# aws/sagemaker-xgboost-container

Hardware: NVIDIA H100
Metric: boosting rounds/sec (higher is better)
Workload: dtype int64

## Files before the change

### microbench/hist_modes.py

```python
#!/usr/bin/env python
import argparse
import json
import os
import sys

import numpy as np

ROOT = os.path.dirname(os.path.dirname(os.path.abspath(__file__)))
sys.path.insert(0, ROOT)


def main():
    ap = argparse.ArgumentParser()
    ap.add_argument("--rows", type=int, default=50_000_000)
    ap.add_argument("--cols", type=int, default=100)
    ap.add_argument("--repeats", type=int, default=5)
    ap.add_argument("--out", default="")
    a = ap.parse_args()
    import torch
    import bench
    import sagemaker_xgboost_container_b200 as xgb
    be = xgb.get_backend()
    dev = torch.device("cuda", 0)
    ba = argparse.Namespace(rows=a.rows, cols=a.cols, seed=43, objective="reg:squarederror", num_class=0)
    X, y = bench.gen_shard(ba, 0, a.rows, dev)
    d = xgb.DMatrix(X, label=y.cpu().numpy())
    del X
    torch.cuda.empty_cache()
    b = xgb.Booster({"max_bin": 256}, [d])
    rng = np.random.default_rng(1)
    n, F = a.rows, a.cols
    gpair = np.empty((n, 2), np.float32)
    gpair[:, 0] = rng.standard_normal(n, dtype=np.float32)
    gpair[:, 1] = 1.0
    peak = bench.hbm_peak()[0]
    res = []

    def run(label, mode, rows=None):
        m = n if rows is None else len(rows)
        gp = gpair if rows is None else gpair[:m]
        be.build_histogram_ex(b.handle, d.handle, gp, mode=mode, row_ids=rows, repeats=2)
        hist, scales, ms, kernel = be.build_histogram_ex(b.handle, d.handle, gp, mode=mode, row_ids=rows, repeats=a.repeats)
        bytes_ = m * (F + 8 + (0 if rows is None else 4))
        r = {"case": label, "kernel": kernel, "rows": m, "ms": ms, "gbs": bytes_ / ms / 1e6, "frac_of_peak": bytes_ / ms / 1e6 / peak,
             "checksum": int(hist[:, :, 0].sum()), "checksum_h": int(hist[:, :, 1].sum())}
        res.append(r)
        print(json.dumps(r), flush=True)

    run("root TMA G+H", 0)
    run("root TMA G-only", 2)
    run("root gather-kernel", 1)
    run("every 2nd row", 0, np.arange(0, n, 2, dtype=np.uint32))
    run("every 4th row", 0, np.arange(0, n, 4, dtype=np.uint32))
    sub = np.sort(rng.choice(n, size=n // 4, replace=False).astype(np.uint32))
    run("random 25% sorted", 0, sub)
    sub = np.sort(rng.choice(n, size=n // 16, replace=False).astype(np.uint32))
    run("random 6% sorted", 0, sub)
    if a.out:
        json.dump({"rows": n, "cols": F, "peak_gbs": peak, "results": res}, open(a.out, "w"), indent=1)


if __name__ == "__main__":
    main()
```

### sagemaker-xgboost-container_b200/csrc/booster.cu

```cuda
#include "booster.h"
#include <algorithm>
#include <atomic>
#include <cctype>
#include <cmath>
#include <cstring>
#include "comm.h"
#include "rng.h"

namespace b200 {

long long g_kernel_launches = 0;

namespace {
struct DeviceCtx {
  cudaStream_t stream = nullptr; int num_sms = 0; bool ok = false; std::string why;
  DeviceCtx() {
    int count = 0;
    cudaError_t e = cudaGetDeviceCount(&count);
    if (e != cudaSuccess || count == 0) { why = std::string("no CUDA device available (") + cudaGetErrorString(e) + ")"; cudaGetLastError(); return; }
    int dev = 0;
    if (const char* lr = getenv("LOCAL_RANK")) { dev = atoi(lr) % count; }
    if (const char* d = getenv("B200XGB_DEVICE")) { dev = atoi(d) % count; }
    if (cudaSetDevice(dev) != cudaSuccess) { why = "cudaSetDevice failed"; return; }
    if (cudaStreamCreateWithFlags(&stream, cudaStreamNonBlocking) != cudaSuccess) { why = "cudaStreamCreate failed"; return; }
// ... 462 lines not shown
    c.n = dm->n; c.margin.alloc((size_t)dm->n * K); c.trees_applied = -1;
  }
  return c;
}

void Booster::bring_cache_up_to_date(DMatrix* dm, PredCache& c) {
  cudaStream_t s = engine_stream();
  const int K = param_.num_class;
  const int nt = (int)trees_.size();
  if (c.trees_applied < 0) {
    if (!dm->base_margin.empty()) {
      B200_CHECK(dm->base_margin.size() == (size_t)dm->n * K, "base_margin size does not match rows x groups");
      CUDA_OK(cudaMemcpyAsync(c.margin.p, dm->d_base_margin.p, sizeof(float) * dm->n * K, cudaMemcpyDeviceToDevice, s));
    } else launch_fill(c.margin.p, dm->n * K, base_margin(), s);
    c.trees_applied = 0; c.weights.clear();
  }
  if (dart_.on) {
    std::vector<int> ids; std::vector<float> coef;
    for (int t = 0; t < c.trees_applied; ++t)
      if (c.weights[t] != weight_drop_[t]) { ids.push_back(t); coef.push_back(weight_drop_[t] - c.weights[t]); }
    for (int t = c.trees_applied; t < nt; ++t) { ids.push_back(t); coef.push_back(weight_drop_[t]); }
    if (!ids.empty()) dart_margin(dm, ids, coef, {}, c.margin.p, nullptr);
  } else if (c.trees_applied < nt) {
    upload_model();
    PredictArgs pa = predict_args(dm, c.trees_applied, nt);
    pa.margin = c.margin.p;
    launch_predict(pa, s);
  }
  c.trees_applied = nt;
  c.weights.assign(weight_drop_.begin(), weight_drop_.begin() + nt);
}

std::vector<int> Booster::dart_drop_set(int round) const {
  std::vector<int> D;
  const int T = (int)weight_drop_.size();
  const unsigned seed = param_.seed;
  if (T == 0) return D;
  if (dart_.skip_drop > 0.0f && rng_uniform(seed, kDartSkipStream, (uint64_t)round) < dart_.skip_drop) return D;
  const uint64_t tree_stream = kDartTreeStream + (uint64_t)round;
  float sum_w = 0.0f;
  for (float w : weight_drop_) sum_w += w;
  for (int i = 0; i < T; ++i) {
    const float u = rng_uniform(seed, tree_stream, (uint64_t)i);
    const float thr = dart_.sample_type == 1 ? dart_.rate_drop * (float)T * weight_drop_[i] / sum_w : dart_.rate_drop;
    if (u < thr) D.push_back(i);
  }
  if (dart_.one_drop && D.empty()) {
    const double u = (double)rng_uniform(seed, kDartOneStream, (uint64_t)round);
    int pick = std::min(T - 1, (int)(u * (double)T));
    if (dart_.sample_type == 1) {
      double tot = 0.0; for (float w : weight_drop_) tot += (double)w;
      const double target = u * tot; double acc = 0.0; pick = T - 1;
      for (int i = 0; i < T; ++i) { acc += (double)weight_drop_[i]; if (acc > target) { pick = i; break; } }
    }
    D.push_back(pick);
  }
  return D;
}

float* Booster::dart_begin_round(DMatrix* dtrain, PredCache& c, int round) {
  const std::vector<int> D = dart_drop_set(round);
  const int K = param_.num_class;
  const float lr = (float)((double)param_.eta / (double)K);
  float factor = 1.0f; dart_new_weight_ = 1.0f;
  if (!D.empty()) {
    if (dart_.normalize_type == 1) { factor = (float)(1.0 / (1.0 + (double)lr)); dart_new_weight_ = factor; }
    else { const float denom = (float)D.size() + lr; factor = (float)((double)D.size() / (double)denom); dart_new_weight_ = (float)(1.0 / (double)denom); }
  }
  builder_->set_leaf_scale(dart_new_weight_);
  if (D.empty()) return c.margin.p;
  std::vector<float> coef_full, coef_drop;
  for (int j : D) {
    const float w = weight_drop_[j], w2 = w * factor;
    coef_drop.push_back(w); coef_full.push_back(w2 - w);
    weight_drop_[j] = w2; c.weights[j] = w2;
  }
  dart_drop_margin_.ensure((size_t)dtrain->n * K);
  dart_margin(dtrain, D, coef_full, coef_drop, c.margin.p, dart_drop_margin_.p);
  return dart_drop_margin_.p;
}

void Booster::dart_margin(DMatrix* dm, const std::vector<int>& ids, const std::vector<float>& coef_full, const std::vector<float>& coef_drop,
                          float* m_full, float* m_drop) {
  cudaStream_t s = engine_stream();
  upload_model();
  const size_t m = ids.size();
  dart_ids_.ensure(m); dart_coef_.ensure(2 * m);
  CUDA_OK(cudaMemcpyAsync(dart_ids_.p, ids.data(), sizeof(int) * m, cudaMemcpyHostToDevice, s));
  CUDA_OK(cudaMemcpyAsync(dart_coef_.p, coef_full.data(), sizeof(float) * m, cudaMemcpyHostToDevice, s));
  if (m_drop) CUDA_OK(cudaMemcpyAsync(dart_coef_.p + m, coef_drop.data(), sizeof(float) * m, cudaMemcpyHostToDevice, s));
  DartArgs a{}; a.X = dm->X.p; a.n = dm->n; a.F = dm->F; a.nodes = d_nodes.p; a.tree_offset = d_tree_offset.p; a.tree_info = d_tree_info.p;
  a.trees = dart_ids_.p; a.ntrees = (int)m; a.K = param_.num_class; a.coef_full = dart_coef_.p; a.coef_drop = dart_coef_.p + m;
  a.m_full = m_full; a.m_drop = m_drop;
  launch_dart_margin(a, s);
  Comm::get().sync_stream(s);
}

static void check_labels(const DMatrix* dm) {
  B200_CHECK(dm->labels.size() == (size_t)dm->n, "Check failed: preds.size() == info.labels_.size() (" + std::to_string(dm->n) + " vs. " +
             std::to_string(dm->labels.size()) + ") : labels are not correctly provided");
}
static void check_aft_bounds(const DMatrix* dm) {
  B200_CHECK(dm->label_lower.size() == (size_t)dm->n && dm->label_upper.size() == (size_t)dm->n,
             "survival:aft needs label_lower_bound and label_upper_bound with one entry per row (" + std::to_string(dm->n) + " rows, " +
             std::to_string(dm->label_lower.size()) + " lower and " + std::to_string(dm->label_upper.size()) + " upper bounds)");
}
static void check_train_width(const DMatrix* dm) {
  B200_CHECK(dm->F <= kMaxTrainFeatures, "the CUDA hist builder trains on at most " + std::to_string(kMaxTrainFeatures) + " features (the data has " +
             std::to_string(dm->F) + ")");
}

void Booster::update_one_iter(int iter, DMatrix* dtrain) {
  configure();
  (void)iter;
  cudaStream_t s = engine_stream();
  if (param_.objective == kAft) check_aft_bounds(dtrain); else check_labels(dtrain);
  B200_CHECK(param_.objective != kCox || !Comm::get().distributed(), "survival:cox is not supported with more than one GPU (world_size > 1): its risk sets span the rows of every rank");
  if (num_feature_ == 0) num_feature_ = dtrain->F;
  B200_CHECK(num_feature_ == dtrain->F, "Check failed: learner_model_param_.num_feature == p_fmat->Info().num_col_ (" + std::to_string(num_feature_) +
             " vs. " + std::to_string(dtrain->F) + ") : Number of columns does not match number of features in booster.");
  B200_CHECK(dtrain->n > 0 || Comm::get().distributed(), "Empty dataset at worker: 0");
  check_train_width(dtrain);
  dtrain->ensure_binned(param_.max_bin);
  const int K = param_.num_class;
  TreeBuilder& b = builder_for(dtrain);
  if (!labels_checked_) {
    const std::vector<float>& y = dtrain->labels;
    if (param_.objective == kBinaryLogistic || param_.objective == kRegLogistic || param_.objective == kLogitRaw)
      for (float v : y) B200_CHECK(v >= 0.0f && v <= 1.0f, "Check failed: label must be in [0,1] for logistic regression");
    if (param_.objective == kSoftprob || param_.objective == kSoftmax)
      for (float v : y) B200_CHECK(v >= 0.0f && (int)v < K, "SoftmaxMultiClassObj: label must be in [0, num_class).");
    if (param_.objective == kSquaredLogError) for (float v : y) B200_CHECK(v > -1.0f, "Check failed: label must be greater than -1 for rmsle so that log(label + 1) can be valid.");
    if (param_.objective == kPoisson) for (float v : y) B200_CHECK(v >= 0.0f, "PoissonRegression: label must be nonnegative");
    if (param_.objective == kGamma) for (float v : y) B200_CHECK(v > 0.0f, "GammaRegression: label must be positive.");
    if (param_.objective == kTweedie) for (float v : y) B200_CHECK(v >= 0.0f, "TweedieRegression: label must be nonnegative");
    if (param_.objective == kAft)
      for (int64_t i = 0; i < dtrain->n; ++i) {
        const float lo = dtrain->label_lower[i], hi = dtrain->label_upper[i];
        B200_CHECK(lo >= 0.0f, "survival:aft: label_lower_bound must be >= 0 (row " + std::to_string(i) + ": " + std::to_string(lo) + ")");
        B200_CHECK(hi >= lo, "survival:aft: label_upper_bound must be >= label_lower_bound (row " + std::to_string(i) + ": " + std::to_string(lo) + " > " + std::to_string(hi) + ")");
      }
    labels_checked_ = true;
  }
  estimate_base_score(dtrain);
  PredCache& cache = cache_for(dtrain);
  bring_cache_up_to_date(dtrain, cache);

  const int round = layers();
  const int P = param_.num_parallel_tree;
  const bool per_tree_sample = P > 1 && param_.subsample < 1.0f;
  B200_CHECK(!dart_.on || P == 1, "booster=dart with num_parallel_tree > 1 is not implemented on the CUDA hist path");
  if (!per_tree_sample) forest_gpair_.release();
  const float* grad_margin = dart_.on ? dart_begin_round(dtrain, cache, round) : cache.margin.p;
  CUDA_OK(cudaMemsetAsync(b.gs.absmax, 0, 8, s));
  if (per_tree_sample) {
    forest_gpair_.ensure((size_t)b.gp_stride * K);
    launch_objective(dtrain, grad_margin, round, forest_gpair_.p, b.gp_stride, nullptr, 1.0f);
  } else launch_objective(dtrain, grad_margin, round, b.gpair.p, b.gp_stride, b.gs.absmax, param_.subsample);
  if (!per_tree_sample) {
    Comm::get().allreduce_max_u32(b.gs.absmax, 2, s);
    launch_scales(b.gs, grad_bits_for(b.global_n), s);
  }

  for (int k = 0; k < K; ++k)
    for (int j = 0; j < P; ++j) {
      if (per_tree_sample) {
        CUDA_OK(cudaMemsetAsync(b.gs.absmax, 0, 8, s));
        SampleArgs sa{}; sa.src = forest_gpair_.p; sa.dst = b.gpair.p; sa.absmax = b.gs.absmax; sa.gp_stride = b.gp_stride; sa.n = dtrain->n;
        sa.row_offset = (int64_t)Comm::get().rank() << 40; sa.K = K; sa.subsample = param_.subsample; sa.seed = param_.seed;
        sa.stream = j == 0 ? 0x2000ull + (uint64_t)round : kForestRowStream + ((uint64_t)round << 20) + (uint64_t)j;
        launch_sample_gpair(sa, s);
        Comm::get().allreduce_max_u32(b.gs.absmax, 2, s);
        launch_scales(b.gs, grad_bits_for(b.global_n), s);
      }
      grow_one_tree(dtrain, cache, k, iteration_indptr_[round] + k * P + j);
    }
  iteration_indptr_.push_back((int)trees_.size());
}

void Booster::launch_objective(DMatrix* dm, const float* margin, int round, float2* gpair, int64_t gp_stride, unsigned* absmax, float subsample) {
  cudaStream_t s = engine_stream();
  const int64_t row_offset = (int64_t)Comm::get().rank() << 40;
  if (objective_is_survival(param_.objective)) {
    SurvivalGradArgs sa{}; sa.margin = margin; sa.label = dm->d_labels.p; sa.lower = dm->d_label_lower.p; sa.upper = dm->d_label_upper.p;
    sa.weight = dm->weights.empty() ? nullptr : dm->d_weights.p; sa.gpair = gpair; sa.absmax = absmax; sa.n = dm->n; sa.row_offset = row_offset;
    sa.subsample = subsample; sa.seed = param_.seed; sa.iter = (unsigned long long)round; sa.dist = param_.aft_dist; sa.sigma = param_.aft_sigma;
    if (param_.objective == kAft) { launch_aft_gradient(sa, s); return; }
    if (!dm->cox_order.valid) cox_sort(dm->d_labels.p, dm->n, &dm->cox_order, &cox_scratch_, s);
    launch_cox_gradient(sa, dm->cox_order, &cox_scratch_, s);
    return;
  }
  GradArgs ga{}; ga.margin = margin; ga.label = dm->d_labels.p; ga.weight = dm->weights.empty() ? nullptr : dm->d_weights.p;
  ga.gpair = gpair; ga.gp_stride = gp_stride; ga.absmax = absmax; ga.err = builder_->err.p; ga.n = dm->n; ga.row_offset = row_offset; ga.K = param_.num_class;
  ga.objective = param_.objective; ga.scale_pos_weight = param_.scale_pos_weight; ga.subsample = subsample; ga.seed = param_.seed;
  ga.iter = (unsigned long long)round; ga.aux = objective_aux(param_);
  launch_gradient(ga, s);
}

void Booster::debug_gradient(DMatrix* dm, const float* margin, int round, float* out) {
  configure();
  cudaStream_t s = engine_stream();
  if (param_.objective == kAft) check_aft_bounds(dm); else check_labels(dm);
  dm->ensure_binned(param_.max_bin); builder_for(dm);
  const int K = param_.num_class;
  const int64_t n = dm->n;
  DevBuf<float> d_margin; DevBuf<float2> d_gp; d_margin.alloc((size_t)n * K); d_gp.alloc((size_t)n * K);
  if (n) CUDA_OK(cudaMemcpyAsync(d_margin.p, margin, sizeof(float) * n * K, cudaMemcpyHostToDevice, s));
  launch_objective(dm, d_margin.p, round, d_gp.p, n, nullptr, param_.subsample);
  std::vector<float2> h((size_t)n * K);
  if (n) CUDA_OK(cudaMemcpyAsync(h.data(), d_gp.p, sizeof(float2) * h.size(), cudaMemcpyDeviceToHost, s));
  Comm::get().sync_stream(s);
  for (int64_t r = 0; r < n; ++r)
    for (int k = 0; k < K; ++k) { out[(r * K + k) * 2] = h[(size_t)k * n + r].x; out[(r * K + k) * 2 + 1] = h[(size_t)k * n + r].y; }
}

static int lossguide_iters(const TrainParam& p) {
  if (!p.lossguide) return 0;
  if (p.max_leaves > 0) return std::max(1, p.max_leaves - 1);
  return (1 << p.max_depth) - 1;
}

static TrainParamDev to_dev(const TrainParam& p) {
  TrainParamDev d; d.eta = p.eta / (float)p.num_parallel_tree; d.lambda = p.lambda; d.alpha = p.alpha; d.gamma = p.gamma; d.min_child_weight = p.min_child_weight;
  d.max_delta_step = p.max_delta_step; d.max_depth = p.max_depth; d.max_leaves = p.max_leaves; return d;
}

TreeBuilder& Booster::builder_for(DMatrix* dm) {
  builder_->ensure(dm->binned_view(), param_.max_depth, param_.num_class, lossguide_iters(param_), (int)interaction_.size());
  return *builder_;
}

TreeInputs Booster::tree_inputs(const DMatrix& dm, const std::string& mask, int tree_index, float* margin, int k) {
  TreeBuilder& b = *builder_;
  TreeInputs in{};
  in.bm = dm.binned_view(); in.cut_ptrs = dm.d_cut_ptrs.p; in.cut_vals = dm.d_cut_vals.p; in.min_vals = dm.d_min_vals.p;
  in.margin = margin; in.K = param_.num_class; in.k = k;
  in.p = to_dev(param_); in.colsample_bynode = param_.colsample_bynode; in.seed = param_.seed; in.lg_iters = lossguide_iters(param_);
  in.mask = mask.empty() ? nullptr : b.upload_mask(mask, tree_index);
  in.monotone = b.upload_monotone(monotone_, dm.F);
  b.upload_interaction(interaction_, dm.F); in.n_ic = (int)interaction_.size();
  static const bool no_consth = getenv("B200XGB_NO_CONSTH") != nullptr;
  const bool consth = !no_consth && param_.objective == kSquaredError && param_.num_class == 1 && dm.weights.empty() &&
                      param_.subsample >= 1.0f && param_.scale_pos_weight == 1.0f;
  in.root_mode = !consth ? 0 : b.root_h_valid && b.root_h_uid == dm.uid && b.root_h_version == dm.binned_version ? 2 : 1;
  in.world = Comm::get().world();
  return in;
}

void Booster::grow_one_tree(DMatrix* dtrain, PredCache& cache, int k, int tree_index) {
  cudaStream_t s = engine_stream();
  TreeBuilder& b = *builder_;
  std::string mask;
  if (param_.colsample_bytree < 1.0f || param_.colsample_bylevel < 1.0f || param_.colsample_bynode < 1.0f) {
    const std::string tm = colsample_mask(param_.seed, tree_index, dtrain->F, param_.colsample_bytree);
    for (int d = 0; d < param_.max_depth; ++d) mask += subset_mask(tm, param_.colsample_bylevel, param_.seed, 0x300000ull + 64ull * (uint64_t)tree_index + (uint64_t)d);
  }
  const TreeInputs in = tree_inputs(*dtrain, mask, tree_index, cache.margin.p, k);
  b.grow(in);
  if (in.root_mode == 1) { b.root_h_valid = true; b.root_h_uid = dtrain->uid; b.root_h_version = dtrain->binned_version; }

  reserve_nodes((size_t)b.cap_nodes, 64 * (size_t)b.cap_nodes);
  CUDA_OK(cudaMemcpyAsync(d_nodes.p + d_nodes_used, b.packed.p, sizeof(DevNode) * (size_t)b.cap_nodes, cudaMemcpyDeviceToDevice, s));
  if (pending_.size() - (size_t)std::count_if(pending_.begin(), pending_.end(), [](const PendingTree& p) { return p.staging == nullptr; }) >= 512) sync_model();
  const float weight = dart_.on ? dart_new_weight_ : 1.0f;
  append_device_tree(k, d_nodes_used, b.cap_nodes, b.stage_tree(), weight);
  d_nodes_used += (size_t)b.cap_nodes;
  d_trees_uploaded = 0;
  cache.trees_applied = (int)trees_.size();
  cache.weights.push_back(weight);
}

void Booster::boost_one_iter(DMatrix*, const float*, const float*, size_t) {
  throw Error("custom objective (BoostOneIter) is not implemented on the CUDA hist path");
}

int Booster::boosted_rounds() { configure(); return layers(); }

static std::string default_metric(const TrainParam& p) {
  switch (p.objective) {
    case kSquaredError: case kRegLogistic: return "rmse";
    case kBinaryLogistic: case kLogitRaw: return "logloss";
    case kSquaredLogError: return "rmsle";
    case kPseudoHuber: return "mphe";
    case kPoisson: return "poisson-nloglik";
    case kGamma: return "gamma-nloglik";
    case kTweedie: { char buf[64]; snprintf(buf, sizeof buf, "tweedie-nloglik@%g", (double)p.tweedie_variance_power); return buf; }
    case kHinge: return "error";
    case kAft: return "aft-nloglik";
    case kCox: return "cox-nloglik";
    default: return "mlogloss";
  }
}

std::string Booster::eval_one_iter(int iter, const std::vector<DMatrix*>& dms, const std::vector<std::string>& names) {
  configure();
  cudaStream_t s = engine_stream();
  std::vector<std::string> metrics = eval_metrics_;
  if (metrics.empty()) metrics.push_back(default_metric(param_));
  dsum_.ensure(4);
  std::string out = "[" + std::to_string(iter) + "]";
  for (size_t i = 0; i < dms.size(); ++i) {
    DMatrix* dm = dms[i];
    if (param_.objective != kAft) check_labels(dm);
    PredCache& c = cache_for(dm);
    bring_cache_up_to_date(dm, c);
    for (const std::string& mname : metrics) {
      MetricArgs ma{}; ma.margin = c.margin.p; ma.label = dm->d_labels.p; ma.weight = dm->weights.empty() ? nullptr : dm->d_weights.p;
      ma.out = dsum_.p; ma.n = dm->n; ma.K = param_.num_class; ma.threshold = 0.5f;
      ma.is_logistic = (param_.objective == kBinaryLogistic || param_.objective == kRegLogistic) ? 1 : 0;
      ma.transform = objective_transform(param_.objective); ma.aux = 0.0f;
      std::string base = mname;
      if (mname.rfind("tweedie-nloglik@", 0) == 0) { base = "tweedie-nloglik"; ma.aux = std::stof(mname.substr(16)); B200_CHECK(ma.aux >= 1.0f && ma.aux < 2.0f, "tweedie variance power must be in interval [1, 2)"); }
      if (mname.rfind("error@", 0) == 0) { base = "error"; ma.threshold = std::stof(mname.substr(6)); }
      if (base == "auc") {
        B200_CHECK(param_.num_class <= 1, "auc is implemented for binary / regression-style predictions only");
        const int logistic = (param_.objective == kBinaryLogistic || param_.objective == kRegLogistic) ? 1 : 0;
        compute_auc_device(c.margin.p, dm->d_labels.p, dm->weights.empty() ? nullptr : dm->d_weights.p, dm->n, logistic, dsum_.p, s);
        double h3[3];
        CUDA_OK(cudaMemcpyAsync(h3, dsum_.p, 3 * sizeof(double), cudaMemcpyDeviceToHost, s));
        Comm::get().sync_stream(s);
        double pair[2] = {h3[0], h3[1] * h3[2]};
        if (Comm::get().distributed()) {
          CUDA_OK(cudaMemcpyAsync(dsum_.p, pair, 2 * sizeof(double), cudaMemcpyHostToDevice, s));
          Comm::get().allreduce_sum_f64(dsum_.p, 2, s);
          CUDA_OK(cudaMemcpyAsync(pair, dsum_.p, 2 * sizeof(double), cudaMemcpyDeviceToHost, s));
          Comm::get().sync_stream(s);
        }
        B200_CHECK(pair[1] > 0.0, "Check failed: !auc_error AUC: the dataset only contains pos or neg samples");
        char buf[64]; snprintf(buf, sizeof buf, "%.17g", pair[0] / pair[1]);
        out += "\t" + names[i] + "-" + mname + ":" + buf;
        continue;
      }
      if (mname == "aft-nloglik" || mname == "interval-regression-accuracy") {
        check_aft_bounds(dm);
        CUDA_OK(cudaMemsetAsync(dsum_.p, 0, 2 * sizeof(double), s));
        launch_aft_metric(c.margin.p, dm->d_label_lower.p, dm->d_label_upper.p, ma.weight, dm->n, param_.aft_dist, param_.aft_sigma,
                          mname == "aft-nloglik" ? 0 : 1, dsum_.p, s);
      } else if (mname == "cox-nloglik") {
        B200_CHECK(!Comm::get().distributed(), "cox-nloglik is not supported with more than one GPU (world_size > 1)");
        check_labels(dm);
        if (!dm->cox_order.valid) cox_sort(dm->d_labels.p, dm->n, &dm->cox_order, &cox_scratch_, s);
        cox_nloglik(c.margin.p, dm->n, dm->cox_order, &cox_scratch_, dsum_.p, s);
      } else {
        if (param_.objective == kAft) check_labels(dm);
        if (base == "rmse") ma.metric = kMetricRmse; else if (base == "mse") ma.metric = kMetricRmse; else if (base == "mae") ma.metric = kMetricMae;
        else if (base == "logloss") ma.metric = kMetricLogloss; else if (base == "error") ma.metric = kMetricError;
        else if (base == "merror") ma.metric = kMetricMerror; else if (base == "mlogloss") ma.metric = kMetricMlogloss;
        else if (base == "rmsle") ma.metric = kMetricRmsle; else if (base == "mape") ma.metric = kMetricMape;
        else if (base == "mphe") { ma.metric = kMetricMphe; ma.aux = param_.huber_slope; }
        else if (base == "poisson-nloglik") ma.metric = kMetricPoissonNll; else if (base == "gamma-nloglik") ma.metric = kMetricGammaNll;
        else if (base == "gamma-deviance") ma.metric = kMetricGammaDeviance;
        else if (base == "tweedie-nloglik") { ma.metric = kMetricTweedieNll; if (ma.aux == 0.0f) throw Error("tweedie-nloglik needs its variance power: tweedie-nloglik@rho"); }
        else throw Error("Unknown metric function " + mname + " (the CUDA hist path implements rmse, mse, rmsle, mae, mape, mphe, logloss, error, error@t, merror, mlogloss, auc, poisson-nloglik, gamma-nloglik, gamma-deviance, tweedie-nloglik@rho, aft-nloglik, interval-regression-accuracy, cox-nloglik)");
        if (param_.objective == kLogitRaw && (ma.metric == kMetricLogloss || ma.metric == kMetricError)) ma.is_logistic = 1;
        if ((ma.metric == kMetricMerror || ma.metric == kMetricMlogloss)) B200_CHECK(param_.num_class > 1, "Check failed: preds.size() == info.labels_.size() : label and prediction size not match, hint: use merror or mlogloss for multi-class classification");
        CUDA_OK(cudaMemsetAsync(dsum_.p, 0, 2 * sizeof(double), s));
        launch_metric(ma, s);
      }
      Comm::get().allreduce_sum_f64(dsum_.p, 2, s);
      double h[2];
      CUDA_OK(cudaMemcpyAsync(h, dsum_.p, 2 * sizeof(double), cudaMemcpyDeviceToHost, s));
      Comm::get().sync_stream(s);
      double v = h[1] == 0.0 ? h[0] : h[0] / h[1];
      if (mname == "rmse" || mname == "rmsle") v = std::sqrt(v);
      if (mname == "gamma-deviance") v *= 2.0;
      char buf[64]; snprintf(buf, sizeof buf, "%.17g", v);
      out += "\t" + names[i] + "-" + mname + ":" + buf;
    }
  }
  return out;
}

void Booster::predict(DMatrix* dm, int type, bool training, int iter_begin, int iter_end, bool strict_shape,
                      std::vector<float>* out, std::vector<uint64_t>* shape) {
  configure();
  (void)training;
  cudaStream_t s = engine_stream();
  const int K = param_.num_class;
  const int rounds = layers();
  if (iter_end == 0) iter_end = rounds;
  B200_CHECK(iter_begin >= 0 && iter_begin <= iter_end && iter_end <= rounds, "Invalid iteration range: [" + std::to_string(iter_begin) + ", " + std::to_string(iter_end) + ") for a model with " + std::to_string(rounds) + " rounds");
  if (num_feature_ > 0 && !trees_.empty())
    B200_CHECK(dm->F <= num_feature_ || true, "feature count mismatch");
  B200_CHECK(type == 0 || type == 1 || type == 2 || type == 6, "predict type " + std::to_string(type) + " (approximate contributions / interactions) is not implemented on the CUDA path");
  const int tb = iteration_indptr_[iter_begin], te = iteration_indptr_[iter_end];
  if (type == 2) { predict_contribs(dm, tb, te, out, shape); return; }
  upload_model();
  const int64_t n = dm->n;
  PredictArgs pa = predict_args(dm, tb, te);
  if (type == 6) {
    const int nt = te - tb;
    DevBuf<int>& leaf = pred_leaf_; leaf.ensure((size_t)n * std::max(nt, 1));
    pa.margin = nullptr; pa.leaf = leaf.p;
    launch_predict(pa, s);
    std::vector<int> h((size_t)n * nt);
    if (!h.empty()) CUDA_OK(cudaMemcpyAsync(h.data(), leaf.p, sizeof(int) * h.size(), cudaMemcpyDeviceToHost, s));
    Comm::get().sync_stream(s);
// ... 153 lines not shown
```

### sagemaker-xgboost-container_b200/csrc/booster.h

```cpp
#pragma once
#include <map>
#include <memory>
#include <string>
#include <vector>
#include "engine.h"
#include "grow.h"
#include "json.h"
#include "misc.h"
#include "survival.h"
#include "tree.h"

namespace b200 {

class DMatrix {
 public:
  int64_t n = 0; int F = 0;
  bool has_missing = false;
  DevBuf<float> X;
  std::vector<float> labels, weights, base_margin;
  DevBuf<float> d_labels, d_weights, d_base_margin;
  std::vector<float> label_lower, label_upper;
  DevBuf<float> d_label_lower, d_label_upper;
  CoxOrder cox_order;
  std::vector<std::string> feature_names, feature_types;
  bool binned = false; int binned_max_bin = 0;
  HostCuts cuts; DevBuf<int> d_cut_ptrs; DevBuf<float> d_cut_vals, d_min_vals;
  DevBuf<uint8_t> bins, bins_tail, bins_col, bins_gather; int ngroups = 0, tw = 0, ntail = 0, gather_stride = 0;
  uint64_t binned_version = 0;
  uint64_t uid;

  DMatrix();
  static std::unique_ptr<DMatrix> from_dense(const float* data, int64_t nrow, int ncol, float missing);
  static std::unique_ptr<DMatrix> from_device(const float* dptr, int64_t nrow, int ncol, float missing);
  static std::unique_ptr<DMatrix> from_csv_text(const char* text, int64_t len, char delim, int* status);
  static std::unique_ptr<DMatrix> from_libsvm_text(const char* text, int64_t len, int whitespace_mode, float absent, int* status);
  static std::unique_ptr<DMatrix> from_csv_text_labeled(const char* text, int64_t len, char delim, int label_col, int weight_col, int* status);
  static std::unique_ptr<DMatrix> from_columns(const void* const* cols, const int* types, int ncols, int64_t nrow, int label_col, int weight_col);
  static std::unique_ptr<DMatrix> from_csr(const size_t* indptr, const unsigned* indices, const float* data, size_t nindptr, size_t nelem, size_t ncol);
  std::unique_ptr<DMatrix> slice(const int* idx, int64_t len) const;
  void set_float_info(const std::string& field, const float* v, size_t len);
  const std::vector<float>& get_float_info(const std::string& field) const;
  void ensure_binned(int max_bin);
  void set_cuts(const HostCuts& c);
  BinnedMatrix binned_view() const { BinnedMatrix b; b.bins = bins.p; b.bins_tail = tw ? bins_tail.p : nullptr; b.bins_col = bins_col.p; b.n = n; b.F = F;
    b.bins_gather = bins_gather.p ? bins_gather.p : bins.p; b.gather_stride = gather_stride; b.tail_in_gather = bins_gather.p && tw == 8 ? 1 : 0;
    b.ngroups = ngroups; b.tw = tw; b.ntail = ntail; b.has_missing = has_missing; return b; }
  void finish_upload(float missing);
 private:
  void bin_with_cuts();
};

struct HostTree {
  std::vector<int> left, right, parent, split_index, split_bin;
  std::vector<uint8_t> default_left;
  std::vector<float> split_cond, base_weight, loss_chg, sum_hess;
  int num_nodes() const { return (int)left.size(); }
};

struct PredCache {
  DevBuf<float> margin; int trees_applied = 0; int64_t n = 0; uint64_t model_version = 0;
  std::vector<float> weights;
};

struct DartParam { bool on = false; float rate_drop = 0.0f, skip_drop = 0.0f; int one_drop = 0, sample_type = 0, normalize_type = 0; };

bool looks_like_legacy_binary(const char* buf, size_t len);
JPtr legacy_binary_to_doc(const char* buf, size_t len);
std::pair<const char*, size_t> legacy_serialized_model_section(const char* buf, size_t len);

class Booster {
 public:
  Booster();
  ~Booster();
  void set_param(const std::string& k, const std::string& v);
  std::string save_config();
  void load_config(const std::string& json);
  void update_one_iter(int iter, DMatrix* dtrain);
  void boost_one_iter(DMatrix* dtrain, const float* grad, const float* hess, size_t len);
  std::string eval_one_iter(int iter, const std::vector<DMatrix*>& dms, const std::vector<std::string>& names);
  void predict(DMatrix* dm, int type, bool training, int iter_begin, int iter_end, bool strict_shape,
               std::vector<float>* out, std::vector<uint64_t>* shape);
  void predict_contribs(DMatrix* dm, int tree_begin, int tree_end, std::vector<float>* out, std::vector<uint64_t>* shape);
  std::string save_model_buffer(const std::string& format);
  void load_model_buffer(const char* buf, size_t len);
  std::string serialize();
  void unserialize(const char* buf, size_t len);
  std::unique_ptr<Booster> slice(int begin, int end, int step);
  int boosted_rounds();
  int num_features() const { return num_feature_; }
  std::map<std::string, std::string> attrs;
  std::vector<std::string> feature_names, feature_types;

  void sync_model();
  void cached_margin(DMatrix* dm, std::vector<float>* out);
  float debug_predict_kernel_ms(DMatrix* dm, int repeats);
  std::string debug_predict_plan(DMatrix* dm, int iter_begin, int iter_end);
  const std::vector<HostTree>& trees() { sync_model(); return trees_; }
  const std::vector<int>& tree_info() const { return tree_info_; }
  const std::vector<float>& tree_weights() const { return weight_drop_; }
  float base_score() const { return base_score_; }
  int num_class() const { return param_.num_class; }
  const TrainParam& param() { configure(); return param_; }
  void set_profile(bool on);
  void debug_gradient(DMatrix* dm, const float* margin, int round, float* out);
  std::string get_profile();
  void debug_build_root_hist(DMatrix* dm, const float* gpair_host, std::vector<long long>* hist_out, float* scales_out,
                             int repeats, float* ms_out, int mode = 0, const unsigned* row_ids = nullptr, int64_t n_ids = 0);
  std::string debug_eval_root(DMatrix* dm, const long long* hist_fm, long long G, long long H, float max_g, float max_h,
                              float lower, float upper, const unsigned char* feat_mask);

 private:
  PredictArgs predict_args(DMatrix* dm, int tree_begin, int tree_end);
  std::map<std::string, std::string> raw_params_;
  std::vector<std::string> eval_metrics_;
  std::vector<int> monotone_;
  std::vector<std::vector<int>> interaction_;
  bool configured_ = false;
  TrainParam param_;
  std::string objective_name_ = "reg:squarederror";
  bool base_score_set_ = false; float base_score_ = 0.5f; bool base_score_estimated_ = false;
  int num_feature_ = 0;
  std::vector<HostTree> trees_; std::vector<int> tree_info_;
  std::vector<int> iteration_indptr_{0};
  DevBuf<float2> forest_gpair_;
  std::vector<float> weight_drop_;
  DartParam dart_;
  float dart_new_weight_ = 1.0f;
  DevBuf<float> dart_drop_margin_;
  DevBuf<int> dart_ids_; DevBuf<float> dart_coef_;
  std::vector<PendingTree> pending_;
  std::vector<char> on_device_;
  uint64_t model_version_ = 0;
  DevBuf<DevNode> d_nodes; std::vector<int64_t> h_tree_offset; DevBuf<int64_t> d_tree_offset; DevBuf<int> d_tree_info;
  size_t d_nodes_used = 0; int d_trees_uploaded = 0;
  std::map<uint64_t, PredCache> caches_;
  std::unique_ptr<TreeBuilder> builder_ = std::make_unique<TreeBuilder>();
  DevBuf<double> dsum_;
  CoxScratch cox_scratch_;
  bool labels_checked_ = false;
  DevBuf<float> pred_margin_, pred_cls_; DevBuf<int> pred_leaf_;
  bool children_adjacent_ = true;

  void configure();
  int layers() const { return (int)iteration_indptr_.size() - 1; }
  float base_margin() const;
  void estimate_base_score(DMatrix* dtrain);
  void upload_model();
  PredCache& cache_for(DMatrix* dm);
  void bring_cache_up_to_date(DMatrix* dm, PredCache& c);
  void append_device_tree(int class_id, size_t device_offset, int max_nodes, PendingTree pt, float weight);
  std::vector<int> dart_drop_set(int round) const;
  float* dart_begin_round(DMatrix* dtrain, PredCache& c, int round);
  void dart_margin(DMatrix* dm, const std::vector<int>& ids, const std::vector<float>& coef_full, const std::vector<float>& coef_drop,
                   float* m_full, float* m_drop);
  void reserve_nodes(size_t count, size_t slack);
  TreeBuilder& builder_for(DMatrix* dm);
  TreeInputs tree_inputs(const DMatrix& dm, const std::string& mask, int tree_index, float* margin, int k);
  void grow_one_tree(DMatrix* dtrain, PredCache& cache, int k, int tree_index);
  void launch_objective(DMatrix* dm, const float* margin, int round, float2* gpair, int64_t gp_stride, unsigned* absmax, float subsample);
  JPtr model_to_json();
  void model_from_json(const JValue& doc);
  JPtr config_to_json();
  void config_from_json(const JValue& doc);
  void reset_model();
};

std::string colsample_mask(unsigned seed, int tree_index, int F, float frac);
std::string subset_mask(const std::string& parent, float frac, unsigned seed, uint64_t stream);

}
```

### sagemaker-xgboost-container_b200/csrc/grow.cu

```cuda
#include "grow.h"
#include <algorithm>
#include <cmath>
#include <cstdlib>
#include <cstring>
#include "comm.h"

namespace b200 {

__global__ void pack_tree_kernel(TreeArrays t, const int* n_nodes, DevNode* out, int cap) {
  const int nn = *n_nodes;
  for (int i = blockIdx.x * blockDim.x + threadIdx.x; i < cap; i += gridDim.x * blockDim.x) {
    DevNode d;
    if (i < nn) { d.cond = t.split_cond[i]; d.left = t.left[i]; d.right = t.right[i]; d.fidx_dl = (unsigned)t.split_index[i] | ((unsigned)t.default_left[i] << 31); }
    else { d.cond = 0.f; d.left = -1; d.right = -1; d.fidx_dl = 0; }
    out[i] = d;
  }
}
__global__ void snapshot_h_kernel(const GH64* slot, long long* cache, size_t entries) {
  for (size_t e = (size_t)blockIdx.x * blockDim.x + threadIdx.x; e < entries; e += (size_t)gridDim.x * blockDim.x) cache[e] = slot[e].h;
}
__global__ void slot_from_cache_kernel(GH64* slot, const long long* cache, size_t entries) {
  for (size_t e = (size_t)blockIdx.x * blockDim.x + threadIdx.x; e < entries; e += (size_t)gridDim.x * blockDim.x) { GH64 v; v.g = 0; v.h = cache[e]; slot[e] = v; }
}
__global__ void gather_u32_kernel(const unsigned* src, const unsigned* idx, unsigned* dst, int64_t n) {
// ... 15 lines not shown
  auto take = [&](auto*& p, size_t bytes) { p = reinterpret_cast<std::remove_reference_t<decltype(p)>>(base + off); off += (bytes + 255) & ~(size_t)255; };
  take(gs.seg_begin, 4 * N); take(gs.seg_count, 4 * N); take(gs.hist_slot, 4 * N); take(gs.node_sum, 16 * N); take(gs.root_gain, 4 * N); take(gs.weight, 4 * N);
  take(gs.best, sizeof(SplitCand) * N); take(gs.best_group, sizeof(SplitCand) * N * nblocks);
  take(gs.level_nodes, 4 * (size_t)(kMaxDepth + 1) * L); take(gs.level_count, 4 * (kMaxDepth + 2));
  take(gs.build_nid, 4 * L); take(gs.build_sub_nid, 4 * L); take(gs.build_parent_slot, 4 * L); take(gs.build_count, 4); take(gs.build_prefix, 4 * (L + 1));
  take(gs.part_action, 4 * L); take(gs.tile_prefix, 4 * (L + 1));
  take(gs.tile_desc, 8 * ((size_t)max_tiles + 1)); gs.part_ctl = (unsigned*)(gs.tile_desc + max_tiles);
  take(gs.n_leaves, 4); take(gs.scales, 16); take(gs.absmax, 8);
  take(gs.depth, 4 * N); take(gs.open, N); take(gs.n_slots, 4); take(gs.lg_done, 4); take(gs.lower, 4 * N); take(gs.upper, 4 * N);
  return off;
}

void TreeBuilder::ensure(const BinnedMatrix& bm, int max_depth_, int K, int lg_iters_, int n_ic_) {
  const bool tail_pos_ = tail_by_position(bm);
  const int64_t stride_ = (bm.n + 63) & ~(int64_t)63;
  if (n == bm.n && F == bm.F && ngroups == bm.ngroups && tw == bm.tw && tail_pos == tail_pos_ && max_depth == max_depth_ && lg_iters == lg_iters_ &&
      n_ic == n_ic_ && gpair.n >= (size_t)stride_ * K + 512) return;
  if (lg_iters_ == 0) B200_CHECK(max_depth_ >= 1 && max_depth_ <= kMaxDepth, "max_depth must be in [1, 16] for the B200 depth-wise hist builder");
  n = bm.n; F = bm.F; ngroups = bm.ngroups; tw = bm.tw; tail_pos = tail_pos_; max_depth = max_depth_; lg_iters = lg_iters_; n_ic = n_ic_;
  gp_stride = stride_; root_h_valid = false;
  cudaStream_t s = engine_stream();
  if (peer_reduce_active()) {
    peer_reduce_close();
    DevBuf<unsigned> bar; bar.alloc(1); bar.zero(s);
    Comm::get().allreduce_max_u32(bar.p, 1, s);
    Comm::get().sync_stream(s);
  }
  for (auto& tg : graphs) tg.destroy();
  size_t pool_slots; int max_nodes;
  if (lg_iters > 0) {
    max_nodes = 2 * lg_iters + 1; max_level_nodes = 2; region = 0;
    pool_slots = (size_t)lg_iters + kLgFirstFreeSlot;
  } else {
    max_nodes = (1 << (max_depth + 1)) - 1; max_level_nodes = 1 << (max_depth - 1); region = max_level_nodes;
    pool_slots = 2 * (size_t)region;
  }
  cap_nodes = (max_nodes + 15) & ~15;
  slot_stride = hist_slot_entries(ngroups, tw);
  const size_t pool_bytes = pool_slots * slot_stride * sizeof(GH64);
  size_t free_b = 0, total_b = 0; cudaMemGetInfo(&free_b, &total_b);
  B200_CHECK(pool_bytes < free_b / 2 + hist_pool.n * sizeof(GH64), "histogram pool for this max_depth / max_leaves / feature count does not fit in device memory");
  hist_pool.alloc(pool_slots * slot_stride);
  gpair.alloc((size_t)gp_stride * K + 512); gpair.zero(s); err.alloc(1); tree_index_dev.alloc(1);
  if (!leaf_scale.p) { leaf_scale.alloc(1); set_leaf_scale(1.0f); }
  root_h_cache.alloc(slot_stride);
  const bool routed = routes(lg_iters, max_depth);
  for (int i = 0; i < 2; ++i) { const size_t m = i == 0 || !routed ? (size_t)n : 0; ridx[i].alloc(m); gp[i].alloc(m); tl[i].alloc(tail_pos ? m : 0); }
  route_tiles = routed ? (unsigned)((n + kRouteTile - 1) / kRouteTile) : 0u;
  node_of_row.alloc(routed ? (size_t)n : 0);
  route_counts.alloc(routed && max_depth >= 2 ? ((size_t)1 << (max_depth - 2)) * route_tiles : 0);
  max_tiles = (unsigned)((n + kPartTile - 1) / kPartTile) + max_level_nodes + 1;
  scratch.alloc(3 * (size_t)max_level_nodes + 8);
  state_block.alloc(carve(gs, 0)); state_block.zero(s);
  carve(gs, (uintptr_t)state_block.p);
  tree_block.alloc(tree_block_bytes(cap_nodes));
  const TreeBlock tb = tree_block_layout(tree_block.p, cap_nodes);
  gs.n_nodes = tb.n_nodes; ta = tb.t; packed.alloc(cap_nodes);
  ic_path.alloc(n_ic ? (size_t)cap_nodes * F : 0); ic_allowed.alloc(n_ic ? (size_t)cap_nodes * F : 0);
  ic_sets.alloc((size_t)n_ic * F); ic_sets_host.clear();
  hist_configure();
  global_n = n;
  if (Comm::get().distributed()) {
    peer_reduce_setup({{hist_pool.p, hist_pool.n * sizeof(GH64)}, {state_block.p, state_block.n}}, s);
    DevBuf<double> dsum; dsum.alloc(1); double v = (double)n;
    CUDA_OK(cudaMemcpyAsync(dsum.p, &v, sizeof v, cudaMemcpyHostToDevice, s));
    Comm::get().allreduce_sum_f64(dsum.p, 1, s);
    CUDA_OK(cudaMemcpyAsync(&v, dsum.p, sizeof v, cudaMemcpyDeviceToHost, s));
    Comm::get().sync_stream(s);
    global_n = (int64_t)v;
  }
}

void TreeBuilder::set_leaf_scale(float v) {
  cudaStream_t s = engine_stream();
  CUDA_OK(cudaMemcpyAsync(leaf_scale.p, &v, sizeof v, cudaMemcpyHostToDevice, s));
  Comm::get().sync_stream(s);
}

const unsigned char* TreeBuilder::upload_mask(const std::string& mask, int tree_index) {
  cudaStream_t s = engine_stream(); feat_mask.ensure(mask.size());
  CUDA_OK(cudaMemcpyAsync(feat_mask.p, mask.data(), mask.size(), cudaMemcpyHostToDevice, s));
  CUDA_OK(cudaMemcpyAsync(tree_index_dev.p, &tree_index, sizeof(int), cudaMemcpyHostToDevice, s));
  Comm::get().sync_stream(s); return feat_mask.p;
}
template <typename T> static T* upload_changed(DevBuf<T>& d, std::vector<T>& host, const std::vector<T>& v) {
  if (v == host && d.n >= v.size()) return d.p;
  cudaStream_t s = engine_stream(); d.ensure(v.size());
  CUDA_OK(cudaMemcpyAsync(d.p, v.data(), sizeof(T) * v.size(), cudaMemcpyHostToDevice, s));
  Comm::get().sync_stream(s); host = v; return d.p;
}

const int* TreeBuilder::upload_monotone(const std::vector<int>& mono, int F_) {
  if (mono.empty()) return nullptr;
  B200_CHECK((int)mono.size() <= F_, "monotone_constraints has more entries than the data has features");
  std::vector<int> mh(mono); mh.resize((size_t)F_, 0);
  return upload_changed(monotone_dev, monotone_host, mh);
}
void TreeBuilder::upload_interaction(const std::vector<std::vector<int>>& ic, int F_) {
  if (ic.empty()) return;
  std::vector<unsigned char> sets(ic.size() * (size_t)F_, 0);
  for (size_t si = 0; si < ic.size(); ++si)
    for (int f : ic[si]) { B200_CHECK(f < F_, "interaction_constraints names feature " + std::to_string(f) + " but the data has " + std::to_string(F_) + " features"); sets[si * F_ + f] = 1; }
  upload_changed(ic_sets, ic_sets_host, sets);
}
HistArgs TreeBuilder::hist_args(const BinnedMatrix& bm, int k) const {
  HistArgs ha{}; ha.bins = bm.bins; ha.bins_tail = bm.bins_tail; ha.n = bm.n; ha.row_stride = bm.ngroups * kSlots; ha.tw = bm.tw;
  ha.bins_gather = bm.bins_gather; ha.gather_stride = bm.gather_stride;
  ha.tail_in_gather = bm.tail_in_gather;
  ha.gpair = gpair.p + (size_t)k * gp_stride;
  ha.build_count = gs.build_count; ha.build_nid = gs.build_nid; ha.build_prefix = gs.build_prefix; ha.seg_begin = gs.seg_begin;
  ha.hist_slot = gs.hist_slot; ha.scales = gs.scales; ha.hist_pool = hist_pool.p; ha.node_sum = gs.node_sum; ha.ngroups = bm.ngroups;
  ha.accumulate_sum = 1; ha.window_rows = window_rows_for(global_n);
  return ha;
}

EvalArgs TreeBuilder::eval_args(const TreeInputs& in, int level, const unsigned char* feat_mask) const {
  const BinnedMatrix& bm = in.bm;
  EvalArgs ea{}; ea.hist_pool = hist_pool.p; ea.gs = gs; ea.cut_ptrs = in.cut_ptrs; ea.feat_mask = feat_mask; ea.p = in.p; ea.F = bm.F;
  ea.ngroups = bm.ngroups; ea.tw = bm.tw; ea.ntail = bm.ntail; ea.has_missing = bm.has_missing; ea.level = level; ea.max_level_nodes = max_level_nodes;
  ea.colsample_bynode = in.mask ? in.colsample_bynode : 1.0f; ea.seed = in.seed; ea.tree_index = tree_index_dev.p; ea.monotone = in.monotone;
  ea.node_allowed = in.n_ic > 0 ? ic_allowed.p : nullptr;
  return ea;
}
ApplyArgs TreeBuilder::apply_args(const TreeInputs& in, int level, int next_base, int next_half) const {
  const BinnedMatrix& bm = in.bm;
  ApplyArgs aa{}; aa.gs = gs; aa.tree = ta; aa.cut_ptrs = in.cut_ptrs; aa.cut_vals = in.cut_vals; aa.min_vals = in.min_vals;
  aa.p = in.p; aa.scratch = scratch.p; aa.nblocks = bm.ngroups + (bm.tw > 0 ? 1 : 0); aa.level = level; aa.max_level_nodes = max_level_nodes;
  aa.next_base = next_base; aa.next_half = next_half; aa.monotone = in.monotone;
  if (in.n_ic > 0) { aa.node_path = ic_path.p; aa.node_allowed = ic_allowed.p; aa.ic_sets = ic_sets.p; aa.n_ic_sets = in.n_ic; aa.F = bm.F; }
  return aa;
}
template <class Launch> void TreeBuilder::timed(ProfKind kind, Launch launch) {
  if (!profile) { launch(); return; }
  ProfEvent e; e.kind = kind; e.launches = g_kernel_launches;
  CUDA_OK(cudaEventCreate(&e.a)); CUDA_OK(cudaEventCreate(&e.b));
  CUDA_OK(cudaEventRecord(e.a, engine_stream()));
  launch();
  e.launches = g_kernel_launches - e.launches;
  CUDA_OK(cudaEventRecord(e.b, engine_stream()));
  prof_events.push_back(e);
}

constexpr int kRootRows = -1;
void TreeBuilder::enqueue(const TreeInputs& in) {
  cudaStream_t s = engine_stream();
  const BinnedMatrix& bm = in.bm;
  const int k = in.k, D = in.p.max_depth;
  const bool dist = in.world > 1;
  const int num_sms = engine_num_sms();
  launch_init_tree(gs, ta, (unsigned)bm.n, s);
  if (in.root_mode == 2) { slot_from_cache_kernel<<<num_sms, 256, 0, s>>>(hist_pool.p, root_h_cache.p, slot_stride); ++g_kernel_launches; CUDA_OK(cudaGetLastError()); }
  else CUDA_OK(cudaMemsetAsync(hist_pool.p, 0, slot_stride * sizeof(GH64), s));
  const bool g_only = in.root_mode != 0;
  const bool carry_tail = tail_by_position(bm);
  const bool routed = routes(in.lg_iters, D);
  if (profile && routed) {
    prof_part_row_bytes[0] = 3;
    prof_part_row_bytes[1] = 4;
    prof_part_row_bytes[2] = 8 + 4 + (g_only ? 4 : 8) + (carry_tail ? 8 : 0);
  } else if (profile) {
    prof_part_row_bytes[0] = 8 + (carry_tail ? 4 : 0) + 1;
    prof_part_row_bytes[2] = 4 + (g_only ? 4 : 8) + (carry_tail ? 4 : 0);
    prof_part_row_bytes[1] = prof_part_row_bytes[2] + 1;
  }
  HistArgs root = hist_args(bm, k);
  root.g_only = in.root_mode == 2 ? 1 : 0; root.rows_counter = profile ? prof_rows.p : nullptr;
  timed(kProfRootHist, [&] { launch_hist_build(root, num_sms, s); });
  if (in.root_mode == 1) { snapshot_h_kernel<<<num_sms, 256, 0, s>>>(hist_pool.p, root_h_cache.p, slot_stride); ++g_kernel_launches; CUDA_OK(cudaGetLastError()); }
  auto collective = [&](std::function<void()> f) {
    if (!dist) return;
    if (!capturing) { f(); return; }
    end_segment(); capturing->colls.push_back(f);
    CUDA_OK(cudaStreamBeginCapture(s, cudaStreamCaptureModeThreadLocal));
  };
  auto allreduce_hist = [&](GH64* p, size_t cnt) {
    if (!dist) return;
    if (peer_allreduce_i64(reinterpret_cast<long long*>(p), cnt, s)) return;
    collective([p, cnt, s]() { Comm::get().allreduce_sum_i64(p, cnt, s); });
  };
  allreduce_hist(hist_pool.p, slot_stride * 2);
  allreduce_hist(gs.node_sum, 2);
  if (in.n_ic > 0) {
    CUDA_OK(cudaMemsetAsync(ic_path.p, 0, (size_t)bm.F, s));
    CUDA_OK(cudaMemsetAsync(ic_allowed.p, 1, (size_t)bm.F, s));
  }
  auto part_args = [&](int level, int cur, int next) {
    const bool root = cur == kRootRows;
    PartArgs pa{}; pa.gs = gs; pa.tree = ta; pa.bins_col = bm.bins_col; pa.n = bm.n;
    pa.ridx_cur = root ? nullptr : ridx[cur].p; pa.ridx_next = ridx[next].p;
    pa.gp_cur = root ? static_cast<const void*>(gpair.p + (size_t)k * gp_stride) : gp[cur].p; pa.gp_next = gp[next].p;
    pa.gp_cur_stride = root ? 2 : 1; pa.g_only = g_only ? 1 : 0;
    pa.tl_cur = !carry_tail ? nullptr : (root ? reinterpret_cast<const unsigned*>(bm.bins_tail) : tl[cur].p); pa.tl_next = carry_tail ? tl[next].p : nullptr;
    pa.has_missing = bm.has_missing; pa.level = level; pa.max_level_nodes = max_level_nodes; pa.rows_counter = profile ? prof_rows.p + 2 : nullptr;
    return pa;
  };
  auto level_hist_args = [&](int set) {
    HistArgs ha = hist_args(bm, k);
    ha.ridx = ridx[set].p; ha.tail_pos = carry_tail ? tl[set].p : nullptr; ha.accumulate_sum = 0;
    ha.gpair = g_only ? nullptr : gp[set].p; ha.gpos = g_only ? reinterpret_cast<const float*>(gp[set].p) : nullptr;
    ha.rows_counter = profile ? prof_rows.p + 1 : nullptr;
    return ha;
  };
  launch_eval(eval_args(in, 0, in.mask), 1, s);
  for (int it = 0; it < in.lg_iters; ++it) {
    launch_apply_lossguide(apply_args(in, 0, 0, 0), it, s);
    const PartArgs pa = part_args(0, it == 0 ? kRootRows : 0, 1);
    timed(kProfPartition, [&] { launch_partition(pa, max_tiles, s); });
    launch_lg_copy_back(pa, ridx[0].p, gp[0].p, tl[0].p, max_tiles, s);
    launch_zero_build_slots(gs, hist_pool.p, slot_stride, 1, s);
    timed(kProfDeepHist, [&] { launch_hist_build(level_hist_args(0), num_sms, s); });
    if (dist) {
      launch_lg_stage(gs, hist_pool.p, slot_stride, 1, s);
      allreduce_hist(hist_pool.p + (size_t)kLgStageSlot * slot_stride, slot_stride * 2);
      launch_lg_stage(gs, hist_pool.p, slot_stride, 0, s);
    }
    launch_subtract(gs, hist_pool.p, slot_stride, 1, s);
    launch_eval(eval_args(in, 1, nullptr), 2, s);
  }
  for (int L = 0; L < D && in.lg_iters == 0; ++L) {
    const bool final_level = (L == D - 1);
    const int next_base = ((L + 1) & 1) * region, next_half = 1 << L;
    launch_apply(apply_args(in, L, next_base, next_half), s);
    if (final_level) break;
    if (routed) {
      RouteArgs ra{}; ra.gs = gs; ra.tree = ta; ra.bins_col = bm.bins_col; ra.n = bm.n; ra.node_of_row = node_of_row.p;
      ra.tile_counts = route_counts.p; ra.ntiles = route_tiles; ra.has_missing = bm.has_missing; ra.level = L;
      ra.gpair = gpair.p + (size_t)k * gp_stride; ra.g_only = g_only ? 1 : 0;
      ra.tail_row = carry_tail ? reinterpret_cast<const unsigned*>(bm.bins_tail) : nullptr;
      ra.ridx = ridx[0].p; ra.gp = gp[0].p; ra.tl = carry_tail ? tl[0].p : nullptr; ra.rows_counter = profile ? prof_rows.p + 2 : nullptr;
      timed(kProfPartition, [&] { launch_route(ra, s); });
    } else {
      PartArgs pa = part_args(L, L == 0 ? kRootRows : (L & 1) ^ 1, L & 1);
      pa.build_only = L == D - 2 ? 1 : 0;
      timed(kProfPartition, [&] { launch_partition(pa, max_tiles, s); });
    }
    CUDA_OK(cudaMemsetAsync(hist_pool.p + (size_t)next_base * slot_stride, 0, (size_t)next_half * slot_stride * sizeof(GH64), s));
    timed(kProfDeepHist, [&] { launch_hist_build(level_hist_args(routed ? 0 : L & 1), num_sms, s); });
    allreduce_hist(hist_pool.p + (size_t)next_base * slot_stride, (size_t)next_half * slot_stride * 2);
    launch_subtract(gs, hist_pool.p, slot_stride, next_half, s);
    launch_eval(eval_args(in, L + 1, in.mask ? in.mask + (size_t)(L + 1) * bm.F : nullptr), 1 << (L + 1), s);
  }
  const uint8_t* start = routed && D >= 2 ? node_of_row.p : nullptr;
  timed(kProfMargin, [&] { launch_update_margin(ta, gs.n_nodes, bm.bins_col, bm.n, bm.has_missing, start, in.margin, in.K, k, leaf_scale.p, s); });
  if (profile) prof_margin_rows += bm.n;
  pack_tree_kernel<<<(cap_nodes + 255) / 256, 256, 0, s>>>(ta, gs.n_nodes, packed.p, cap_nodes); ++g_kernel_launches;
  CUDA_OK(cudaGetLastError());
}
void TreeBuilder::end_segment() {
  cudaGraph_t graph = nullptr; cudaGraphExec_t exec = nullptr;
  CUDA_OK(cudaStreamEndCapture(engine_stream(), &graph));
  cudaError_t e = cudaGraphInstantiate(&exec, graph, 0);
  cudaGraphDestroy(graph);
  CUDA_OK(e);
  capturing->segs.push_back(exec);
}

void TreeBuilder::grow(const TreeInputs& in) {
  cudaStream_t s = engine_stream();
  static const bool no_graph = getenv("B200XGB_NO_GRAPH") != nullptr;
  if ((int)graphs.size() <= in.k) graphs.resize(in.k + 1);
  TreeGraph& tg = graphs[in.k];
  if (profile || no_graph || (in.world > 1 && !tg.eager_done) || in.root_mode == 1) { tg.eager_done = true; enqueue(in); return; }
  if (tg.segs.empty() || memcmp(&tg.key, &in, sizeof in) != 0) {
    tg.destroy();
    const long long launches_before = g_kernel_launches;
    CUDA_OK(cudaStreamBeginCapture(s, cudaStreamCaptureModeThreadLocal));
    capturing = &tg;
    try { enqueue(in); end_segment(); }
    catch (...) { capturing = nullptr; cudaGraph_t graph = nullptr; cudaStreamEndCapture(s, &graph); if (graph) cudaGraphDestroy(graph); tg.destroy(); throw; }
    capturing = nullptr;
    tg.key = in; tg.launches = g_kernel_launches - launches_before;
    g_kernel_launches = launches_before;
  }
  for (size_t i = 0; i < tg.segs.size(); ++i) {
    CUDA_OK(cudaGraphLaunch(tg.segs[i], s));
    if (i < tg.colls.size()) tg.colls[i]();
  }
  g_kernel_launches += tg.launches;
}
PendingTree TreeBuilder::stage_tree() {
  cudaStream_t s = engine_stream();
  PendingTree pt; pt.cap_nodes = (size_t)cap_nodes; pt.staging = pinned.take(tree_block.n);
  if (!free_events.empty()) { pt.ready = free_events.back(); free_events.pop_back(); }
  else CUDA_OK(cudaEventCreateWithFlags(&pt.ready, cudaEventDisableTiming));
  CUDA_OK(cudaMemcpyAsync(pt.staging, tree_block.p, tree_block.n, cudaMemcpyDeviceToHost, s));
  CUDA_OK(cudaEventRecord(pt.ready, s));
  return pt;
}

void TreeBuilder::debug_build_root_hist(const BinnedMatrix& bm, const float* gpair_host, std::vector<long long>* hist_out, float* scales_out,
                                        int repeats, float* ms_out, int mode, const unsigned* row_ids, int64_t n_ids) {
  cudaStream_t s = engine_stream();
  const int64_t rows = row_ids ? n_ids : bm.n;
  B200_CHECK(rows <= bm.n, "debug_build_root_hist: more row ids than rows");
  CUDA_OK(cudaMemcpyAsync(gpair.p, gpair_host, sizeof(float2) * rows, cudaMemcpyHostToDevice, s));
  if (row_ids) CUDA_OK(cudaMemcpyAsync(ridx[0].p, row_ids, sizeof(unsigned) * rows, cudaMemcpyHostToDevice, s));
  float mg = 0.f, mh = 0.f;
  for (int64_t i = 0; i < rows; ++i) { mg = std::max(mg, std::fabs(gpair_host[2 * i])); mh = std::max(mh, gpair_host[2 * i + 1]); }
  unsigned am[2]; memcpy(&am[0], &mg, 4); memcpy(&am[1], &mh, 4);
  CUDA_OK(cudaMemcpyAsync(gs.absmax, am, 8, cudaMemcpyHostToDevice, s));
  launch_scales(gs, grad_bits_for(global_n), s);
  HistArgs ha = hist_args(bm, 0);
  ha.ridx = row_ids ? ridx[0].p : nullptr;
  ha.force_gather = (mode & 3) == 1 ? 1 : 0; ha.g_only = (mode & 3) == 2 ? 1 : 0;
  if (mode & 8) {
    std::vector<float> gh((size_t)rows);
    for (int64_t i = 0; i < rows; ++i) gh[i] = gpair_host[2 * i];
    float* gpos = reinterpret_cast<float*>(gp[0].p);
    if (rows) CUDA_OK(cudaMemcpyAsync(gpos, gh.data(), sizeof(float) * rows, cudaMemcpyHostToDevice, s));
    Comm::get().sync_stream(s);
    ha.gpos = gpos; ha.gpair = nullptr;
  }
  if ((mode & 4) && row_ids && tail_by_position(bm)) {
    gather_u32_kernel<<<(unsigned)((rows + 255) / 256), 256, 0, s>>>(reinterpret_cast<const unsigned*>(bm.bins_tail), ridx[0].p, tl[0].p, rows); ++g_kernel_launches;
    CUDA_OK(cudaGetLastError());
    ha.tail_pos = tl[0].p;
  }
  root_h_valid = false;
  cudaEvent_t e0, e1; CUDA_OK(cudaEventCreate(&e0)); CUDA_OK(cudaEventCreate(&e1));
  float total = 0.f;
  for (int r = 0; r < std::max(1, repeats); ++r) {
    launch_init_tree(gs, ta, (unsigned)rows, s);
    CUDA_OK(cudaMemsetAsync(hist_pool.p, 0, slot_stride * sizeof(GH64), s));
    CUDA_OK(cudaEventRecord(e0, s));
    launch_hist_build(ha, engine_num_sms(), s);
    CUDA_OK(cudaEventRecord(e1, s));
    CUDA_OK(cudaEventSynchronize(e1));
    float ms = 0; CUDA_OK(cudaEventElapsedTime(&ms, e0, e1)); total += ms;
  }
  if (ms_out) *ms_out = total / std::max(1, repeats);
  hist_out->resize(slot_stride * 2);
  CUDA_OK(cudaMemcpyAsync(hist_out->data(), hist_pool.p, sizeof(GH64) * slot_stride, cudaMemcpyDeviceToHost, s));
  CUDA_OK(cudaMemcpyAsync(scales_out, gs.scales, 4 * sizeof(float), cudaMemcpyDeviceToHost, s));
  Comm::get().sync_stream(s);
  cudaEventDestroy(e0); cudaEventDestroy(e1);
}

std::string TreeBuilder::debug_eval_root(const TreeInputs& in, const long long* hist_fm, long long G, long long H, float max_g, float max_h,
                                         float lower, float upper) {
  cudaStream_t s = engine_stream();
  root_h_valid = false;
  const BinnedMatrix& bm = in.bm;
  const int F_ = bm.F;
  std::vector<GH64> slot(slot_stride, GH64{0, 0});
  const size_t W = (size_t)bm.ngroups * kSlots, tail0 = (size_t)bm.ngroups * kGroupEntries;
  for (int f = 0; f < F_; ++f)
    for (int b = 0; b < kBins; ++b) {
      const size_t e = (size_t)f < W ? ((size_t)(f / kSlots) * kBins + b) * kSlots + f % kSlots : tail0 + (size_t)b * bm.tw + (f - W);
      slot[e].g = hist_fm[((size_t)f * kBins + b) * 2]; slot[e].h = hist_fm[((size_t)f * kBins + b) * 2 + 1];
    }
  launch_init_tree(gs, ta, (unsigned)bm.n, s);
  CUDA_OK(cudaMemcpyAsync(hist_pool.p, slot.data(), sizeof(GH64) * slot_stride, cudaMemcpyHostToDevice, s));
  const GH64 tot{G, H};
  CUDA_OK(cudaMemcpyAsync(gs.node_sum, &tot, sizeof tot, cudaMemcpyHostToDevice, s));
  CUDA_OK(cudaMemcpyAsync(gs.lower, &lower, 4, cudaMemcpyHostToDevice, s));
  CUDA_OK(cudaMemcpyAsync(gs.upper, &upper, 4, cudaMemcpyHostToDevice, s));
  unsigned am[2]; memcpy(&am[0], &max_g, 4); memcpy(&am[1], &max_h, 4);
  CUDA_OK(cudaMemcpyAsync(gs.absmax, am, 8, cudaMemcpyHostToDevice, s));
  launch_scales(gs, grad_bits_for(global_n), s);
  launch_eval(eval_args(in, 0, in.mask), 1, s);
  const ApplyArgs aa = apply_args(in, 0, region, 1);
  if (in.lg_iters > 0) launch_apply_lossguide(aa, 0, s); else launch_apply(aa, s);
  const int nblocks = bm.ngroups + (bm.tw > 0 ? 1 : 0);
  std::vector<unsigned char> sb(state_block.n), tb(tree_block.n);
  CUDA_OK(cudaMemcpyAsync(sb.data(), state_block.p, sb.size(), cudaMemcpyDeviceToHost, s));
  CUDA_OK(cudaMemcpyAsync(tb.data(), tree_block.p, tb.size(), cudaMemcpyDeviceToHost, s));
  Comm::get().sync_stream(s);
  GrowState h; carve(h, (uintptr_t)sb.data());
  auto bits = [](float v) { unsigned u; memcpy(&u, &v, 4); return std::to_string(u); };
  auto cand = [&](const SplitCand& c) {
    return "{\"loss_chg\":" + bits(c.loss_chg) + ",\"feature\":" + std::to_string(c.feature) + ",\"bin\":" + std::to_string(c.bin) + ",\"dleft\":" +
           std::to_string(c.dleft) + ",\"ord\":" + std::to_string(c.ord) + ",\"GL\":" + std::to_string(c.GL) + ",\"HL\":" + std::to_string(c.HL) + "}";
  };
  const TreeBlock t = tree_block_layout(tb.data(), cap_nodes);
  const int nn = *t.n_nodes;
  std::string o = "{\"scales\":[";
  for (int i = 0; i < 4; ++i) o += (i ? "," : "") + bits(h.scales[i]);
  o += "],\"root_gain\":" + bits(h.root_gain[0]) + ",\"weight\":" + bits(h.weight[0]) + ",\"best_group\":[";
  for (int i = 0; i < nblocks; ++i) o += (i ? "," : "") + cand(h.best_group[i]);
  o += "],\"best\":" + cand(h.best[0]) + ",\"n_nodes\":" + std::to_string(nn) + ",\"expanded\":" + (nn == 3 ? "true" : "false") + ",\"tree\":{";
  const char* iname[5] = {"left", "right", "parent", "split_index", "split_bin"};
  const int* iarr[5] = {t.t.left, t.t.right, t.t.parent, t.t.split_index, t.t.split_bin};
  const char* fname[4] = {"split_cond", "base_weight", "loss_chg", "sum_hess"};
  const float* farr[4] = {t.t.split_cond, t.t.base_weight, t.t.loss_chg, t.t.sum_hess};
  for (int a = 0; a < 5; ++a) { o += std::string(a ? "," : "") + "\"" + iname[a] + "\":["; for (int i = 0; i < nn; ++i) o += (i ? "," : "") + std::to_string(iarr[a][i]); o += "]"; }
  for (int a = 0; a < 4; ++a) { o += std::string(",\"") + fname[a] + "\":["; for (int i = 0; i < nn; ++i) o += (i ? "," : "") + bits(farr[a][i]); o += "]"; }
  o += ",\"default_left\":["; for (int i = 0; i < nn; ++i) o += (i ? "," : "") + std::to_string((int)t.t.default_left[i]); o += "]}";
  o += ",\"children\":[";
  for (int c = 1; c < nn && c < 3; ++c)
    o += std::string(c > 1 ? "," : "") + "{\"G\":" + std::to_string(h.node_sum[c].g) + ",\"H\":" + std::to_string(h.node_sum[c].h) + ",\"lower\":" + bits(h.lower[c]) + ",\"upper\":" + bits(h.upper[c]) + "}";
  o += "]}";
  return o;
}

void TreeBuilder::set_profile(bool on) {
  profile = on;
  if (on) { prof_rows.alloc(4); prof_rows.zero(engine_stream()); prof_margin_rows = 0; }
  for (auto& e : prof_events) { cudaEventDestroy(e.a); cudaEventDestroy(e.b); }
  prof_events.clear();
}
std::string TreeBuilder::profile_json() {
  cudaStream_t s = engine_stream();
  Comm::get().sync_stream(s);
  double ms[kProfKinds] = {}; long long launches[kProfKinds] = {};
  for (auto& e : prof_events) { float t = 0; CUDA_OK(cudaEventElapsedTime(&t, e.a, e.b)); ms[e.kind] += t; launches[e.kind] += e.launches; }
  unsigned long long rows[4] = {0, 0, 0, 0};
  if (prof_rows.p) CUDA_OK(cudaMemcpy(rows, prof_rows.p, sizeof rows, cudaMemcpyDeviceToHost));
  char buf[1024];
  snprintf(buf, sizeof buf, "{\"root_hist_ms\":%.6f,\"root_hist_launches\":%lld,\"root_hist_rows\":%llu,\"deep_hist_ms\":%.6f,\"deep_hist_launches\":%lld,\"deep_hist_rows\":%llu,"
           "\"part_ms\":%.6f,\"part_launches\":%lld,\"part_rows\":%llu,\"part_rows_written\":%llu,"
           "\"part_row_bytes_in_root\":%d,\"part_row_bytes_in\":%d,\"part_row_bytes_out\":%d,\"margin_ms\":%.6f,\"margin_launches\":%lld,\"margin_rows\":%lld}",
           ms[kProfRootHist], launches[kProfRootHist], rows[0], ms[kProfDeepHist], launches[kProfDeepHist], rows[1],
           ms[kProfPartition], launches[kProfPartition], rows[2], rows[3], prof_part_row_bytes[0], prof_part_row_bytes[1], prof_part_row_bytes[2],
           ms[kProfMargin], launches[kProfMargin], prof_margin_rows);
  return buf;
}

}
```

### sagemaker-xgboost-container_b200/csrc/grow.h

```cpp
#pragma once
#include <functional>
#include <string>
#include <type_traits>
#include <vector>
#include "engine.h"
#include "misc.h"
#include "tree.h"

namespace b200 {

struct TreeInputs {
  BinnedMatrix bm;
  const int* cut_ptrs; const float* cut_vals; const float* min_vals;
  float* margin;
  const unsigned char* mask;
  const int* monotone;
  TrainParamDev p;
  float colsample_bynode; unsigned seed;
  int lg_iters, n_ic;
  int K, k, world;
  int root_mode;
};
static_assert(std::is_trivially_copyable<TreeInputs>::value, "TreeInputs is compared as bytes");
static_assert(sizeof(BinnedMatrix) == 4 * sizeof(void*) + sizeof(int64_t) + 8 * sizeof(int), "BinnedMatrix has padding bytes");
static_assert(sizeof(TrainParamDev) == 8 * 4, "TrainParamDev has padding bytes");
static_assert(sizeof(TreeInputs) == sizeof(BinnedMatrix) + 6 * sizeof(void*) + sizeof(TrainParamDev) + 8 * 4, "TreeInputs has padding bytes");

inline size_t tree_block_bytes(size_t cap) { return 64 + 9 * 4 * cap + cap; }
struct TreeBlock { int* n_nodes; TreeArrays t; };
inline TreeBlock tree_block_layout(void* base, size_t cap) {
  int* ip = (int*)((unsigned char*)base + 64); float* fp = (float*)(ip + 5 * cap);
  return {(int*)base, {ip, ip + cap, ip + 2 * cap, ip + 3 * cap, ip + 4 * cap, (unsigned char*)(fp + 4 * cap), fp, fp + cap, fp + 2 * cap, fp + 3 * cap}};
}

struct PendingTree {
  void* staging = nullptr; size_t cap_nodes = 0; cudaEvent_t ready = nullptr;
};
struct PinnedPool {
  std::vector<std::pair<char*, size_t>> chunks; size_t cur = 0, off = 0;
  ~PinnedPool() { for (auto& c : chunks) cudaFreeHost(c.first); }
  void* take(size_t bytes);
  void reset() { cur = 0; off = 0; }
};

struct TreeGraph {
  std::vector<cudaGraphExec_t> segs; std::vector<std::function<void()>> colls;
  TreeInputs key{}; long long launches = 0;
  bool eager_done = false;
  TreeGraph() = default; TreeGraph(TreeGraph&&) = default;
  ~TreeGraph() { destroy(); }
  void destroy() { for (auto e : segs) if (e) cudaGraphExecDestroy(e); segs.clear(); colls.clear(); }
};

struct TreeBuilder {
  int64_t n = 0; int F = 0, ngroups = 0, tw = 0, max_depth = 0, cap_nodes = 0, max_level_nodes = 0, region = 0; bool tail_pos = false;
  int lg_iters = 0, n_ic = 0;
  size_t slot_stride = 0;
  int64_t gp_stride = 0;
  unsigned max_tiles = 0;
  int64_t global_n = 0;
  DevBuf<long long> root_h_cache; uint64_t root_h_uid = 0, root_h_version = 0; bool root_h_valid = false;
  GrowState gs{}; TreeArrays ta{};
  DevBuf<unsigned char> state_block;
  DevBuf<unsigned char> tree_block;
  DevBuf<GH64> hist_pool; DevBuf<unsigned> ridx[2], scratch;
  DevBuf<float2> gpair, gp[2]; DevBuf<unsigned> tl[2]; DevBuf<int> err, tree_index_dev; DevBuf<unsigned char> ic_path, ic_allowed, ic_sets;
  DevBuf<uint8_t> node_of_row; DevBuf<unsigned> route_counts; unsigned route_tiles = 0;
  DevBuf<DevNode> packed;
  DevBuf<float> leaf_scale;
  DevBuf<unsigned char> feat_mask; DevBuf<int> monotone_dev;
  std::vector<unsigned char> ic_sets_host;
  std::vector<int> monotone_host;
  PinnedPool pinned; std::vector<cudaEvent_t> free_events;
  std::vector<TreeGraph> graphs;
  TreeGraph* capturing = nullptr;
  enum ProfKind { kProfRootHist, kProfDeepHist, kProfPartition, kProfMargin, kProfKinds };
  struct ProfEvent { cudaEvent_t a, b; int kind; long long launches; };
  bool profile = false; std::vector<ProfEvent> prof_events;
  DevBuf<unsigned long long> prof_rows;
  long long prof_margin_rows = 0;
  int prof_part_row_bytes[3] = {0, 0, 0};

  ~TreeBuilder() { for (auto e : free_events) cudaEventDestroy(e); for (auto& e : prof_events) { cudaEventDestroy(e.a); cudaEventDestroy(e.b); } }
  void ensure(const BinnedMatrix& bm, int max_depth, int K, int lg_iters, int n_ic);
  static bool routes(int lg_iters, int max_depth) { return lg_iters == 0 && max_depth <= kRouteMaxDepth; }
  const unsigned char* upload_mask(const std::string& mask, int tree_index);
  const int* upload_monotone(const std::vector<int>& mono, int F);
  void upload_interaction(const std::vector<std::vector<int>>& sets, int F);
  void set_leaf_scale(float v);
  void grow(const TreeInputs& in);
  PendingTree stage_tree();
  void set_profile(bool on); std::string profile_json();
  void debug_build_root_hist(const BinnedMatrix& bm, const float* gpair_host, std::vector<long long>* hist_out, float* scales_out,
                             int repeats, float* ms_out, int mode, const unsigned* row_ids, int64_t n_ids);
  std::string debug_eval_root(const TreeInputs& in, const long long* hist_fm, long long G, long long H, float max_g, float max_h,
                              float lower, float upper);

 private:
  size_t carve(GrowState& g, uintptr_t base) const;
  void enqueue(const TreeInputs& in);
  void end_segment();
  HistArgs hist_args(const BinnedMatrix& bm, int k) const;
  EvalArgs eval_args(const TreeInputs& in, int level, const unsigned char* feat_mask) const;
  ApplyArgs apply_args(const TreeInputs& in, int level, int next_base, int next_half) const;
  template <class Launch> void timed(ProfKind kind, Launch launch);
};

}
```

### sagemaker-xgboost-container_b200/csrc/hist.cu

```cuda
#include <cuda.h>
#include <cstdlib>
#include <cstring>
#include <map>
#include <mutex>
#include <tuple>
#include <type_traits>
#include "engine.h"
#include "tree.h"

namespace b200 {

constexpr int kSuperRows = 32;
constexpr int kMinRowsPerCta = 4096;
constexpr int kSpillThreshold = 1 << 24;
constexpr int kPlaneBytes = kGroupEntries * 4;
constexpr int kMaxSmem = 232448;
constexpr int kTeamWarps = 4, kTeams = 6, kRootRows = 16 * kTeamWarps;
constexpr int kRootConsumerWarps = kTeamWarps * kTeams;
constexpr int kRootProducerWarps = 3;
constexpr int kRootThreads = (kRootConsumerWarps + kRootProducerWarps) * 32;

template <int K, int N, typename F> __device__ __forceinline__ void static_for(F&& f) {
  if constexpr (K < N) { f(std::integral_constant<int, K>{}); static_for<K + 1, N>(f); }
}
// ... 118 lines not shown
  ww[0] = __funnelshift_r(w0, w0, qb8); ww[1] = __funnelshift_r(w1, w1, qb8); ww[2] = __funnelshift_r(w2, w2, qb8); ww[3] = __funnelshift_r(w3, w3, qb8);
}
template <int GOFF>
__device__ __forceinline__ void accumulate16_pairs_prerotated(const unsigned (&A)[16], const unsigned (&ww)[4], int gq, unsigned hq) {
#pragma unroll
  for (int jw = 0; jw < 4; ++jw) {
#pragma unroll
    for (int jb = 0; jb < 4; ++jb) {
      const unsigned bin = (ww[jw] >> (8 * jb)) & 0xffu;
      const unsigned addr = (bin << 7) + A[4 * jw + jb];
      red_shared_s32_off<GOFF>(addr, gq);
      red_shared_u32_off<GOFF + 32768>(addr, hq);
    }
  }
}

template <bool GONLY, int GOFF>
__device__ __forceinline__ void accumulate16(const LaneConst& lc, const unsigned (&ww)[4], int gq, unsigned hq) {
#pragma unroll
  for (int jw = 0; jw < 4; ++jw) {
#pragma unroll
    for (int jb = 0; jb < 4; ++jb) {
      const unsigned bin = __byte_perm(ww[jw], 0u, lc.S[jb]);
      const unsigned addr = (bin << 7) + lc.A[4 * jw + jb];
      red_shared_s32_off<GOFF>(addr, gq);
      if (!GONLY) red_shared_u32_off<GOFF + 32768>(addr, hq);
    }
  }
}

struct TailConst { unsigned base_g, hplane_bytes, bin_stride, rep_off; int tw; };

template <bool GONLY>
__device__ __forceinline__ void tail_accumulate(const TailConst& tc, int lane, unsigned w0, unsigned w1, int gq, unsigned hq) {
#pragma unroll
  for (int j = 0; j < 8; ++j) {
    if (j < tc.tw) {
      const unsigned slot = (unsigned)(j + lane) & (unsigned)(tc.tw - 1);
      const unsigned bin = __byte_perm(w0, w1, slot) & 0xffu;
      const unsigned addr = tc.base_g + bin * tc.bin_stride + tc.rep_off + slot * 4u;
      red_shared_s32(addr, gq);
      if (!GONLY) red_shared_u32(addr + tc.hplane_bytes, hq);
    }
  }
}

template <int TW, int TREP>
__device__ __forceinline__ void tail_accumulate_ct(unsigned base_rep, int lane, unsigned w0, unsigned w1, int gq, unsigned hq) {
  constexpr unsigned kBinStride = (unsigned)(TW * TREP) * 4u, kHPlane = 256u * kBinStride;
#pragma unroll
  for (int j = 0; j < TW; ++j) {
    const unsigned slot = (unsigned)(j + lane) & (unsigned)(TW - 1);
    const unsigned bin = __byte_perm(w0, w1, slot) & 0xffu;
    const unsigned addr = base_rep + bin * kBinStride + slot * 4u;
    red_shared_s32(addr, gq);
    red_shared_u32(addr + kHPlane, hq);
  }
}

__device__ __forceinline__ void flush_node_sum(GH64* dst, int g, unsigned h, int lane) {
  long long G = g, H = h;
#pragma unroll
  for (int o = 16; o > 0; o >>= 1) { G += __shfl_xor_sync(0xffffffffu, G, o); H += __shfl_xor_sync(0xffffffffu, H, o); }
  if (lane == 0 && (G != 0 || H != 0)) { red_global_s64(&dst->g, G); red_global_s64(&dst->h, H); }
}

template <int PL>
__device__ __forceinline__ void spill_main(int* smem, int ng_here, GH64* out, bool last, int tid, int nthr) {
  const int vecs = ng_here * PL * (kGroupEntries / 4);
  const int start = (int)(((long long)blockIdx.x * vecs) / gridDim.x);
  for (int i = tid; i < vecs; i += nthr) {
    int v = i + start; if (v >= vecs) v -= vecs;
    int4 x = reinterpret_cast<int4*>(smem)[v];
    if ((x.x | x.y | x.z | x.w) == 0) continue;
    const int plane = v >> 11;
    const int e0 = (v & 2047) << 2;
    const bool is_h = PL == 2 && (plane & 1);
    GH64* o = out + (size_t)(plane / PL) * kGroupEntries + e0;
    int vals[4] = {x.x, x.y, x.z, x.w};
    bool any = false;
#pragma unroll
    for (int k = 0; k < 4; ++k) {
      const int val = vals[k];
      const bool sp = last ? (val != 0) : (is_h ? ((unsigned)val >= (unsigned)kSpillThreshold) : (val >= kSpillThreshold || val <= -kSpillThreshold));
      if (sp) {
        red_global_s64(is_h ? &o[k].h : &o[k].g, is_h ? (long long)(unsigned)val : (long long)val);
        vals[k] = 0; any = true;
      }
    }
    if (any) reinterpret_cast<int4*>(smem)[v] = make_int4(vals[0], vals[1], vals[2], vals[3]);
  }
}

template <int PL>
__device__ __forceinline__ void spill_tail(int* tsm, int tw, int trep, GH64* out_tail, bool last, int tid, int nthr) {
  const int per_plane = 256 * tw * trep;
  const int per_bin = tw * trep;
  for (int idx = tid; idx < PL * per_plane; idx += nthr) {
    const int val = tsm[idx];
    if (val == 0) continue;
    const bool is_h = idx >= per_plane;
    const int e = is_h ? idx - per_plane : idx;
    const int bin = e / per_bin, slot = e & (tw - 1);
    const bool sp = last ? true : (is_h ? ((unsigned)val >= (unsigned)kSpillThreshold) : (val >= kSpillThreshold || val <= -kSpillThreshold));
    if (sp) {
      GH64* o = out_tail + bin * tw + slot;
      red_global_s64(is_h ? &o->h : &o->g, is_h ? (long long)(unsigned)val : (long long)val);
      tsm[idx] = 0;
    }
  }
}

struct RootCfg {
  int S;
  int trep;
  int box_groups;
  unsigned tail_off;
  unsigned ring_off;
  unsigned stage_bytes;
  unsigned total;
  int flags;
};

template <bool GONLY, int G>
__device__ __forceinline__ void root_unit(const LaneConst& lc, const unsigned (&ldsoff)[4], unsigned rowaddr, int gq, unsigned hq) {
  constexpr int PL = GONLY ? 1 : 2;
  unsigned ww[4];
#pragma unroll
  for (int j = 0; j < 4; ++j) ww[j] = lds_u32(rowaddr + (unsigned)(G * 32) + ldsoff[j]);
  accumulate16<GONLY, G * PL * kPlaneBytes>(lc, ww, gq, hq);
}

template <bool GONLY>
__global__ void __launch_bounds__(kRootThreads, 1)
hist_root_kernel(const __grid_constant__ CUtensorMap tm, HistArgs a, RootCfg c) {
  constexpr int PL = GONLY ? 1 : 2;
  constexpr int NCW = kRootConsumerWarps, R = kRootRows;
  extern __shared__ __align__(128) unsigned char smem_raw[];
  const int nb = *a.build_count;
  if (nb <= 0) return;
  const unsigned T = a.build_prefix[nb];
  if (T == 0) return;
  const int lane = threadIdx.x & 31, warp = threadIdx.x >> 5;
  const int g0 = blockIdx.y * a.ng_chunk;
  const int ng_here = min(a.ng_chunk, a.ngroups - g0);
  const bool has_tail = a.tw > 0 && blockIdx.y == gridDim.y - 1;
  if (a.rows_counter && blockIdx.x == 0 && blockIdx.y == 0 && threadIdx.x == 0) atomicAdd(a.rows_counter, (unsigned long long)T);

  const unsigned smem_base = (unsigned)__cvta_generic_to_shared(smem_raw);
  const unsigned ring = (smem_base + c.ring_off + 127u) & ~127u;
  const unsigned bars = ring + (unsigned)c.S * c.stage_bytes;
  const unsigned row_bytes = 32u * (unsigned)c.box_groups;
  const unsigned main_tile_bytes = (unsigned)R * row_bytes;
  const unsigned gp_off = main_tile_bytes, tail_tile_off = main_tile_bytes + (unsigned)R * 8u;
  const unsigned ntiles = (T + R - 1) / R;
  const unsigned my_ntiles = ntiles > blockIdx.x ? (ntiles - blockIdx.x + gridDim.x - 1) / gridDim.x : 0u;

  {
    const int main4 = ng_here * PL * kPlaneBytes / 16;
    int4* z = reinterpret_cast<int4*>(smem_raw);
    for (int i = threadIdx.x; i < main4; i += blockDim.x) z[i] = make_int4(0, 0, 0, 0);
    if (has_tail) {
      const int tail4 = PL * 256 * a.tw * c.trep * 4 / 16;
      int4* zt = reinterpret_cast<int4*>(smem_raw + c.tail_off);
      for (int i = threadIdx.x; i < tail4; i += blockDim.x) zt[i] = make_int4(0, 0, 0, 0);
    }
    if (threadIdx.x == 0) {
      for (int s = 0; s < c.S; ++s) { mbar_init(bars + 8u * s, 1); mbar_init(bars + 8u * (c.S + s), kTeamWarps); }
      asm volatile("fence.mbarrier_init.release.cluster;" ::: "memory");
    }
  }
  __syncthreads();

  const int nid = a.build_nid[0];
  const size_t slot_entries = (size_t)a.ngroups * kGroupEntries + (size_t)256 * a.tw;
  GH64* out_slot = a.hist_pool + (size_t)a.hist_slot[nid] * slot_entries;
  GH64* out_main = out_slot + (size_t)g0 * kGroupEntries;
  GH64* out_tail = out_slot + (size_t)a.ngroups * kGroupEntries;

  if (warp >= NCW) {
    if (lane == 0) {
      const unsigned P = (c.flags & 8) ? 1u : (unsigned)kRootProducerWarps, pw = (unsigned)(warp - NCW);
      if (pw < P) {
        const unsigned tx = main_tile_bytes + (unsigned)R * 8u + (has_tail ? (unsigned)R * (unsigned)a.tw : 0u);
        unsigned s = pw % (unsigned)c.S, round = pw / (unsigned)c.S;
        for (unsigned i = pw; i < my_ntiles; i += P) {
          if (round > 0) mbar_wait(bars + 8u * (c.S + s), (round - 1u) & 1u);
          const unsigned full = bars + 8u * s, dst = ring + s * c.stage_bytes;
          const unsigned t = blockIdx.x + i * gridDim.x;
          const unsigned row0 = t * (unsigned)R;
          mbar_expect_tx(full, tx);
          if ((c.flags & 1) && gridDim.y == 1) bulk_load_1d(dst, a.bins + (size_t)row0 * a.row_stride, main_tile_bytes, full);
          else tma_load_2d(dst, &tm, g0 * 32, (int)row0, full);
          bulk_load_1d(dst + gp_off, a.gpair + row0, (unsigned)R * 8u, full);
          if (has_tail) bulk_load_1d(dst + tail_tile_off, a.bins_tail + (size_t)row0 * a.tw, (unsigned)R * (unsigned)a.tw, full);
          const unsigned tp = t + 8u * gridDim.x;
          if (tp < ntiles && !(c.flags & 4)) tma_prefetch_2d(&tm, g0 * 32, (int)(tp * (unsigned)R));
          s += P; if (s >= (unsigned)c.S) { s -= (unsigned)c.S; ++round; }
        }
      }
    }
    return;
  }

  const int team = warp / kTeamWarps, wit = warp % kTeamWarps;
  const float sg = a.scales[0], sh = a.scales[1];
  const LaneConst lc = make_lane_const(lane, smem_base);
  unsigned ldsoff[4];
#pragma unroll
  for (int j = 0; j < 4; ++j) { ldsoff[j] = 16u * (unsigned)(lane & 1) + 4u * (unsigned)((j + lc.qw) & 3); asm volatile("" : "+r"(ldsoff[j])); }
  TailConst tc;
  tc.tw = a.tw; tc.base_g = smem_base + c.tail_off; tc.hplane_bytes = 256u * (unsigned)a.tw * (unsigned)c.trep * 4u;
  tc.bin_stride = (unsigned)a.tw * (unsigned)c.trep * 4u;
  tc.rep_off = has_tail ? (unsigned)((lane / a.tw) % c.trep) * (unsigned)a.tw * 4u : 0u;
  const unsigned rowl = (unsigned)(wit << 4) + (unsigned)(lane >> 1);
  const unsigned tiles_per_window = (unsigned)a.window_rows / R;
  long long accG = 0, accH = 0;
  unsigned i = (unsigned)team, s = (unsigned)team, ph = 0;
  for (unsigned wstart = 0;; wstart += tiles_per_window) {
    const unsigned wend = wstart + tiles_per_window < my_ntiles ? wstart + tiles_per_window : my_ntiles;
    while (i < wend) {
      mbar_wait(bars + 8u * s, ph);
      const unsigned tile = ring + s * c.stage_bytes;
      const unsigned row0 = (blockIdx.x + i * gridDim.x) * (unsigned)R;
      if (!(c.flags & 2)) {
        const uint2 ghb = lds_v2(tile + gp_off + rowl * 8u);
        int gq = 0; unsigned hq = 0;
        if (row0 + rowl < T) { gq = __float2int_rn(__uint_as_float(ghb.x) * sg); hq = (unsigned)__float2int_rn(__uint_as_float(ghb.y) * sh); }
        if ((lane & 1) == 0) { accG += gq; accH += hq; }
        const unsigned rowaddr = tile + rowl * row_bytes;
        root_unit<GONLY, 0>(lc, ldsoff, rowaddr, gq, hq);
        if (ng_here > 1) root_unit<GONLY, 1>(lc, ldsoff, rowaddr, gq, hq);
        if (ng_here > 2) root_unit<GONLY, 2>(lc, ldsoff, rowaddr, gq, hq);
        if (has_tail) {
          const unsigned tu = ((unsigned)wit + i) & (unsigned)(kTeamWarps - 1);
          if (tu < (unsigned)(R >> 5)) {
            const unsigned trow = (tu << 5) + (unsigned)lane;
            unsigned w0, w1 = 0;
            if (a.tw == 4) w0 = lds_u32(tile + tail_tile_off + trow * 4u);
            else { const uint2 ww = lds_v2(tile + tail_tile_off + trow * 8u); w0 = ww.x; w1 = ww.y; }
            const uint2 gt = lds_v2(tile + gp_off + trow * 8u);
            int gqt = 0; unsigned hqt = 0;
            if (row0 + trow < T) { gqt = __float2int_rn(__uint_as_float(gt.x) * sg); hqt = (unsigned)__float2int_rn(__uint_as_float(gt.y) * sh); }
            else { w0 = 0; w1 = 0; }
            tail_accumulate<GONLY>(tc, lane, w0, w1, gqt, hqt);
          }
        }
      }
      __syncwarp();
      if (lane == 0) mbar_arrive(bars + 8u * (c.S + s));
      i += kTeams; s += kTeams;
      if (s >= (unsigned)c.S) { s -= (unsigned)c.S; ph ^= 1u; }
    }
    if (wend == my_ntiles) break;
    named_bar_sync(1, NCW * 32);
    spill_main<PL>(reinterpret_cast<int*>(smem_raw), ng_here, out_main, false, threadIdx.x, NCW * 32);
    if (has_tail) spill_tail<PL>(reinterpret_cast<int*>(smem_raw + c.tail_off), a.tw, c.trep, out_tail, false, threadIdx.x, NCW * 32);
    named_bar_sync(1, NCW * 32);
  }
  named_bar_sync(1, NCW * 32);
  spill_main<PL>(reinterpret_cast<int*>(smem_raw), ng_here, out_main, true, threadIdx.x, NCW * 32);
  if (has_tail) spill_tail<PL>(reinterpret_cast<int*>(smem_raw + c.tail_off), a.tw, c.trep, out_tail, true, threadIdx.x, NCW * 32);
  if (a.accumulate_sum && blockIdx.y == 0) {
#pragma unroll
    for (int o = 16; o > 0; o >>= 1) { accG += __shfl_xor_sync(0xffffffffu, accG, o); accH += __shfl_xor_sync(0xffffffffu, accH, o); }
    if (lane == 0 && (accG != 0 || accH != 0)) { red_global_s64(&a.node_sum[nid].g, accG); red_global_s64(&a.node_sum[nid].h, accH); }
  }
}

template <int TW, bool GPAY> struct Stage { unsigned id; typename std::conditional<GPAY, float, float2>::type gr; unsigned t0; };
template <bool GPAY> struct Stage<8, GPAY> { unsigned id; typename std::conditional<GPAY, float, float2>::type gr; unsigned t0, t1; };

__host__ __device__ constexpr int gather_tail_replicas(int ng) { return ng >= 3 ? 4 : 8; }
__host__ __device__ constexpr int gather_tail_bytes(int ng) { return ng >= 3 ? 32768 : 65536; }

template <int NG, int TW, int NTHREADS, bool GPAY>
__global__ void __launch_bounds__(NTHREADS, NG == 1 ? (TW ? 1 : 3) : 1) hist_gather_kernel(HistArgs a) {
  constexpr bool TAIL = TW != 0;
  constexpr int NWARPS = NTHREADS / 32;
  constexpr int LPR = 2 * NG, RPI = 32 / LPR, U = 2 * NG;
  constexpr int SUP = RPI * U;
  static_assert(kWindowRowsSmall / (SUP * NWARPS) >= 1, "window too small");
  const unsigned iters_per_window = (unsigned)a.window_rows / (SUP * NWARPS);
  extern __shared__ __align__(16) int smem[];
  const int nb = *a.build_count;
  if (nb <= 0) return;
  const unsigned T = a.build_prefix[nb];
  if (T == 0) return;
  if (a.rows_counter && blockIdx.x == 0 && blockIdx.y == 0 && threadIdx.x == 0) atomicAdd(a.rows_counter, (unsigned long long)T);
  const unsigned C = gridDim.x;
  unsigned ceff = (T + kMinRowsPerCta - 1) / kMinRowsPerCta;
  ceff = ceff < 1 ? 1 : (ceff > C ? C : ceff);
  if (blockIdx.x >= ceff) return;
  unsigned chunk = (T + ceff - 1) / ceff;
  chunk = (chunk + SUP - 1) / SUP * SUP;
  unsigned long long r0l = (unsigned long long)blockIdx.x * chunk;
  if (r0l >= T) return;
  unsigned r0 = (unsigned)r0l;
  unsigned r1 = (unsigned long long)r0 + chunk > T ? T : r0 + chunk;
  const int g0 = blockIdx.y * a.ng_chunk;
  const int ng_here = min(min(a.ng_chunk, NG), a.ngroups - g0);
  const bool has_tail = TAIL && a.tw > 0 && blockIdx.y == gridDim.y - 1;
  const float sg = a.scales[0], sh = a.scales[1];
  const unsigned smem_g = (unsigned)__cvta_generic_to_shared(smem);
  const bool aligned = a.ridx != nullptr && a.bins_gather != nullptr;
  constexpr bool kLineTail = NG == 3 && TW == 8;
  const bool tail_line = kLineTail && aligned && a.tail_in_gather;
  const int64_t row_stride = aligned ? (int64_t)a.gather_stride : (int64_t)a.row_stride;
  const int lane = threadIdx.x & 31, warp = threadIdx.x >> 5;
  const int q = lane / LPR, c = lane - q * LPR;
  const bool lane_on = q < RPI && (c >> 1) < ng_here;
  const int rot = q < RPI ? NG * q + (c >> 1) : 15;
  const LaneConst lc = make_lane_const_rot(rot, c & 1, smem_g + (unsigned)((q < RPI ? (c >> 1) : 0) * 2 * kPlaneBytes));
  const int rot_qw = rot >> 2, rot_qb8 = (rot & 3) * 8;
  const uint8_t* gbins = (aligned ? a.bins_gather : a.bins) + (int64_t)g0 * kSlots + c * 16;
  constexpr int TWC = TAIL ? TW : 4;
  constexpr int trep = gather_tail_replicas(NG) < gather_tail_bytes(NG) / (2 * 256 * 4 * TWC) ? gather_tail_replicas(NG) : gather_tail_bytes(NG) / (2 * 256 * 4 * TWC);
  const unsigned tail_base_rep = smem_g + (unsigned)(NG * 2 * kPlaneBytes) + (unsigned)((lane / TWC) % trep) * (unsigned)TWC * 4u;

  {
    const int words4 = (NG * 2 * kPlaneBytes + (TAIL ? 2 * 256 * TWC * trep * 4 : 0)) / 16;
    for (int i = threadIdx.x; i < words4; i += NTHREADS) reinterpret_cast<int4*>(smem)[i] = make_int4(0, 0, 0, 0);
  }
  __syncthreads();

  int b = 0;
  { int lo = 0, hi = nb; while (lo < hi) { int mid = (lo + hi) >> 1; if (a.build_prefix[mid + 1] > r0) hi = mid; else lo = mid + 1; } b = lo; }

  const size_t slot_entries = (size_t)a.ngroups * kGroupEntries + (size_t)256 * a.tw;
  typedef Stage<TW, GPAY> StageT;
  const unsigned hq_one = (unsigned)__float2int_rn(1.0f * sh);
  while (r0 < r1) {
    const unsigned nbeg = a.build_prefix[b], nend_node = a.build_prefix[b + 1];
    const unsigned nend = nend_node < r1 ? nend_node : r1;
    const int nid = a.build_nid[b];
    const unsigned seg = a.seg_begin[nid];
    GH64* out_slot = a.hist_pool + (size_t)a.hist_slot[nid] * slot_entries;
    GH64* out_main = out_slot + (size_t)g0 * kGroupEntries;
    GH64* out_tail = out_slot + (size_t)a.ngroups * kGroupEntries;
    int accG = 0; unsigned accH = 0;
    const unsigned pa = seg + (r0 - nbeg), pb = seg + (nend - nbeg);
    const unsigned nsuper = (pb - pa + SUP - 1) / SUP;
    const unsigned iters = (nsuper + NWARPS - 1) / NWARPS;

    auto load_ids = [&](unsigned st) -> StageT {
      StageT s_; s_.id = 0xffffffffu; s_.gr = {}; s_.t0 = 0u;
      if constexpr (TW == 8) s_.t1 = 0u;
      unsigned p = pa + st * SUP + lane;
      if (lane < SUP && st < nsuper && p < pb) {
        s_.id = a.ridx ? __ldg(a.ridx + p) : p;
        if constexpr (GPAY) s_.gr = __uint_as_float(ldg_nc_u32(a.gpos + p)); else s_.gr = ldg_nc_f2(a.gpair + p);
        if (TAIL && has_tail && !tail_line) {
          if constexpr (TW == 8) { const uint2 v = ldg_nc_v2(a.bins_tail + (int64_t)s_.id * 8); s_.t0 = v.x; s_.t1 = v.y; }
          else if (a.tail_pos) s_.t0 = ldg_nc_u32(a.tail_pos + p);
          else s_.t0 = ldg_nc_u32(a.bins_tail + (int64_t)s_.id * 4);
        }
      }
      return s_;
    };
    auto load_unit = [&](unsigned ids, int k) -> uint4 {
      const unsigned rid = __shfl_sync(0xffffffffu, ids, q < RPI ? k * RPI + q : 0);
      return (lane_on && rid != 0xffffffffu) ? ldg_nc_v4(gbins + (int64_t)rid * row_stride) : make_uint4(0, 0, 0, 0);
    };
    auto load_line_tail = [&](StageT& s_) {
      if constexpr (TAIL) {
        if (tail_line && has_tail && s_.id != 0xffffffffu) {
          const uint8_t* t = a.bins_gather + (int64_t)s_.id * row_stride + a.ngroups * kSlots;
          if constexpr (TW == 8) { const uint2 v = ldg_nc_v2(t); s_.t0 = v.x; s_.t1 = v.y; } else s_.t0 = ldg_nc_u32(t);
        }
      }
    };
    StageT cur = load_ids(warp);
    StageT nxt = load_ids(warp + NWARPS);
    uint4 w[U];
#pragma unroll
    for (int k = 0; k < U; ++k) w[k] = load_unit(cur.id, k);
    load_line_tail(cur);
    for (unsigned it = 0; it < iters; ++it) {
      const unsigned s = warp + it * NWARPS;
      StageT nn = load_ids(s + 2 * NWARPS);
      const bool active = s < nsuper;
      int gq_l; unsigned hq_l;
      if constexpr (GPAY) { gq_l = __float2int_rn(cur.gr * sg); hq_l = cur.id != 0xffffffffu ? hq_one : 0u; }
      else { gq_l = __float2int_rn(cur.gr.x * sg); hq_l = (unsigned)__float2int_rn(cur.gr.y * sh); }
      accG += gq_l; accH += hq_l;
#pragma unroll
      for (int k = 0; k < U; ++k) {
        if (active) {
          int gq = __shfl_sync(0xffffffffu, gq_l, q < RPI ? k * RPI + q : 0);
          unsigned hq = __shfl_sync(0xffffffffu, hq_l, q < RPI ? k * RPI + q : 0);
          if (!lane_on) { gq = 0; hq = 0; }
          unsigned ww[4];
          rotate_words_bytes(rot_qw, rot_qb8, w[k], ww);
          accumulate16_pairs_prerotated<0>(lc.A, ww, gq, hq);
        }
        w[k] = load_unit(nxt.id, k);
      }
      if constexpr (TAIL) { if (active && has_tail) { unsigned t1 = 0; if constexpr (TW == 8) t1 = cur.t1; tail_accumulate_ct<TWC, trep>(tail_base_rep, lane, cur.t0, t1, gq_l, hq_l); } }
      load_line_tail(nxt);
      cur = nxt; nxt = nn;
      if ((it + 1) % iters_per_window == 0 && it + 1 < iters) {
        if (a.accumulate_sum && blockIdx.y == 0) { flush_node_sum(a.node_sum + nid, accG, accH, lane); accG = 0; accH = 0; }
        __syncthreads();
        spill_main<2>(smem, ng_here, out_main, false, threadIdx.x, NTHREADS);
        if (has_tail) spill_tail<2>(smem + NG * 2 * kGroupEntries, TWC, trep, out_tail, false, threadIdx.x, NTHREADS);
        __syncthreads();
      }
    }
    __syncthreads();
    spill_main<2>(smem, ng_here, out_main, true, threadIdx.x, NTHREADS);
    if (has_tail) spill_tail<2>(smem + NG * 2 * kGroupEntries, TWC, trep, out_tail, true, threadIdx.x, NTHREADS);
    __syncthreads();
    if (a.accumulate_sum && blockIdx.y == 0) flush_node_sum(a.node_sum + nid, accG, accH, lane);
    r0 = nend; ++b;
  }
}

static thread_local const char* g_last_kernel = "none";
const char* hist_last_kernel() { return g_last_kernel; }

static int chunks_for(int ngroups) { return (ngroups + 2) / 3; }
static int groups_per_chunk(int ngroups) { const int nc = chunks_for(ngroups); return (ngroups + nc - 1) / nc; }

static bool root_plan(int ngc, int tw, bool gonly, RootCfg* c) {
  const int PL = gonly ? 1 : 2;
  const unsigned main_b = (unsigned)ngc * PL * kPlaneBytes;
  const unsigned avail = kMaxSmem - 128  - 2 * 8 * 16 ;
  const unsigned stage = (unsigned)kRootRows * (32u * ngc + 8u + tw);
  int trep = tw ? 32 / tw : 0;
  unsigned tail_b = (unsigned)PL * 256u * tw * trep * 4u;
  if (tw && main_b + tail_b + kTeams * stage > avail) { trep = 1; tail_b = (unsigned)PL * 256u * tw * 4u; }
  if (main_b + tail_b + kTeams * stage > avail) return false;
  int S = (int)((avail - main_b - tail_b) / stage);
  int smax = 16;
  if (const char* e = getenv("B200XGB_ROOT_S")) smax = atoi(e);
  if (S > smax) S = smax;
  constexpr int kStageQuantum = kTeams % kRootProducerWarps == 0 ? kTeams : kTeams * kRootProducerWarps;
  S -= S % kStageQuantum;
  if (S < kTeams) return false;
  c->S = S; c->trep = trep; c->box_groups = ngc; c->tail_off = main_b; c->ring_off = main_b + tail_b; c->stage_bytes = stage;
  c->total = main_b + tail_b + 128 + (unsigned)S * stage + 2 * 8 * (unsigned)S;
  c->flags = 0;
  if (const char* f = getenv("B200XGB_ROOT_FLAGS")) c->flags = atoi(f);
  return true;
}

typedef CUresult (*EncodeTiledFn)(CUtensorMap*, CUtensorMapDataType, cuuint32_t, void*, const cuuint64_t*, const cuuint64_t*, const cuuint32_t*,
                                  const cuuint32_t*, CUtensorMapInterleave, CUtensorMapSwizzle, CUtensorMapL2promotion, CUtensorMapFloatOOBfill);
static EncodeTiledFn encode_fn() {
  static EncodeTiledFn fn = [] {
    void* p = nullptr; cudaDriverEntryPointQueryResult q;
    if (cudaGetDriverEntryPoint("cuTensorMapEncodeTiled", &p, cudaEnableDefault, &q) != cudaSuccess || q != cudaDriverEntryPointSuccess) { cudaGetLastError(); p = nullptr; }
    return reinterpret_cast<EncodeTiledFn>(p);
  }();
  return fn;
}

static bool get_tensor_map(const uint8_t* bins, int64_t n, int row_stride, int box_groups, int R, CUtensorMap* out) {
  typedef std::tuple<const void*, int64_t, int, int, int> Key;
  static std::map<Key, CUtensorMap> cache; static std::mutex mu;
  std::lock_guard<std::mutex> lk(mu);
  const Key key(bins, n, row_stride, box_groups, R);
  auto it = cache.find(key);
  if (it != cache.end()) { *out = it->second; return true; }
  EncodeTiledFn fn = encode_fn();
  if (!fn) return false;
  CUtensorMap tm;
  const cuuint64_t dims[2] = {(cuuint64_t)row_stride, (cuuint64_t)n};
  const cuuint64_t strides[1] = {(cuuint64_t)row_stride};
  const cuuint32_t box[2] = {(cuuint32_t)(32 * box_groups), (cuuint32_t)R};
  const cuuint32_t estr[2] = {1, 1};
  CUresult r = fn(&tm, CU_TENSOR_MAP_DATA_TYPE_UINT8, 2, const_cast<uint8_t*>(bins), dims, strides, box, estr, CU_TENSOR_MAP_INTERLEAVE_NONE,
                  CU_TENSOR_MAP_SWIZZLE_NONE, CU_TENSOR_MAP_L2_PROMOTION_L2_128B, CU_TENSOR_MAP_FLOAT_OOB_FILL_NONE);
  if (r != CUDA_SUCCESS) return false;
  if (cache.size() > 64) cache.clear();
  cache[key] = tm; *out = tm;
  return true;
}

template <int NG, int TW, int NT> static void set_gather_attr() {
  const int smem = NG * 2 * kPlaneBytes + (TW ? gather_tail_bytes(NG) : 0);
  CUDA_OK(cudaFuncSetAttribute(hist_gather_kernel<NG, TW, NT, false>, cudaFuncAttributeMaxDynamicSharedMemorySize, smem));
  CUDA_OK(cudaFuncSetAttribute(hist_gather_kernel<NG, TW, NT, true>, cudaFuncAttributeMaxDynamicSharedMemorySize, smem));
}

void hist_configure() {
  static bool configured = false;
  if (configured) return;
  set_gather_attr<1, 0, 256>(); set_gather_attr<1, 4, 256>(); set_gather_attr<1, 8, 256>();
  set_gather_attr<2, 0, 768>(); set_gather_attr<2, 4, 768>(); set_gather_attr<2, 8, 768>();
  set_gather_attr<3, 0, 768>(); set_gather_attr<3, 4, 768>(); set_gather_attr<3, 8, 768>();
  CUDA_OK(cudaFuncSetAttribute(hist_root_kernel<false>, cudaFuncAttributeMaxDynamicSharedMemorySize, kMaxSmem));
  CUDA_OK(cudaFuncSetAttribute(hist_root_kernel<true>, cudaFuncAttributeMaxDynamicSharedMemorySize, kMaxSmem));
  configured = true;
}

template <int NG, int NT, bool GPAY>
static void launch_gather_tw(const HistArgs& a, int gx, int nchunks, cudaStream_t stream) {
  const int smem = NG * 2 * kPlaneBytes + (a.tw ? gather_tail_bytes(NG) : 0);
  if (a.tw == 0) hist_gather_kernel<NG, 0, NT, GPAY><<<dim3(gx, nchunks), NT, smem, stream>>>(a);
  else if (a.tw == 4) hist_gather_kernel<NG, 4, NT, GPAY><<<dim3(gx, nchunks), NT, smem, stream>>>(a);
  else hist_gather_kernel<NG, 8, NT, GPAY><<<dim3(gx, nchunks), NT, smem, stream>>>(a);
}
template <int NG, int NT>
static void launch_gather(const HistArgs& a, int gx, int nchunks, cudaStream_t stream) {
  if (a.gpos) launch_gather_tw<NG, NT, true>(a, gx, nchunks, stream); else launch_gather_tw<NG, NT, false>(a, gx, nchunks, stream);
}

void launch_hist_build(const HistArgs& a_in, int num_sms, cudaStream_t stream) {
  HistArgs a = a_in;
  const int nchunks = chunks_for(a.ngroups);
  a.ng_chunk = groups_per_chunk(a.ngroups);
  static const bool no_tma = getenv("B200XGB_NO_TMA") != nullptr;
  if (a.ridx == nullptr && !no_tma && !a.force_gather && a.gpos == nullptr) {
    RootCfg c; CUtensorMap tm;
    const bool gonly = a.g_only != 0;
    if (root_plan(a.ng_chunk, a.tw, gonly, &c) && get_tensor_map(a.bins, a.n, a.row_stride, c.box_groups, kRootRows, &tm)) {
      const int gx = num_sms / nchunks > 0 ? num_sms / nchunks : 1;
      if (gonly) hist_root_kernel<true><<<dim3(gx, nchunks), kRootThreads, c.total, stream>>>(tm, a, c);
      else hist_root_kernel<false><<<dim3(gx, nchunks), kRootThreads, c.total, stream>>>(tm, a, c);
      g_last_kernel = gonly ? "hist_root_kernel<GONLY>" : "hist_root_kernel<GH>";
      ++g_kernel_launches;
      CUDA_OK(cudaGetLastError());
      return;
    }
  }
  B200_CHECK(!a.g_only || a.ridx == nullptr, "hist: G-only accumulation is a root-pass mode");
  B200_CHECK(!a.g_only, "hist: the G-only root pass needs the TMA kernel (tensor-map creation failed or B200XGB_NO_TMA is set)");
  const bool tail = a.tw > 0;
  const int ng = a.ng_chunk;
  if (ng == 1) {
    const int per_sm = tail ? 1 : 3;
    const int gx = (num_sms * per_sm + nchunks - 1) / nchunks;
    launch_gather<1, 256>(a, gx, nchunks, stream);
  } else {
    const int gx = (num_sms + nchunks - 1) / nchunks;
    if (ng == 2) launch_gather<2, 768>(a, gx, nchunks, stream); else launch_gather<3, 768>(a, gx, nchunks, stream);
  }
  g_last_kernel = "hist_gather_kernel";
  ++g_kernel_launches;
  CUDA_OK(cudaGetLastError());
}

}
```

### sagemaker-xgboost-container_b200/csrc/misc.cu

```cuda
#include <algorithm>
#include <cstdlib>
#include <utility>
#include "engine.h"
#include "misc.h"
#include "rng.h"

namespace b200 {

__device__ __forceinline__ float sigmoidf_xgb(float x) {
  const float kEps = 1e-16f;
  x = fminf(-x, 88.7f);
  float denom = expf(x) + 1.0f + kEps;
  return 1.0f / denom;
}

__global__ void __launch_bounds__(256) gradient_kernel(GradArgs a) {
  float mg = 0.f, mh = 0.f;
  for (int64_t r = (int64_t)blockIdx.x * blockDim.x + threadIdx.x; r < a.n; r += (int64_t)gridDim.x * blockDim.x) {
    const float y = a.label[r];
    float w = a.weight ? a.weight[r] : 1.0f;
    bool dropped = false;
    if (a.subsample < 1.0f) dropped = !(rng_uniform(a.seed, 0x2000ull + a.iter, (unsigned long long)(r + a.row_offset)) < a.subsample);
    if (a.objective == kSoftprob || a.objective == kSoftmax) {
      const int K = a.K;
      const float* m = a.margin ? a.margin + r * K : nullptr;
      float wmax = m ? m[0] : 0.f;
      for (int k = 1; k < K; ++k) wmax = fmaxf(wmax, m ? m[k] : 0.f);
      float wsum = 0.f;
      for (int k = 0; k < K; ++k) wsum += expf((m ? m[k] : 0.f) - wmax);
      int label = (int)y;
      if (label < 0 || label >= K) { *a.err = 2; label = 0; }
      for (int k = 0; k < K; ++k) {
        float pk = expf((m ? m[k] : 0.f) - wmax) / wsum;
        float h = fmaxf(2.0f * pk * (1.0f - pk) * w, 1e-16f);
        float g = (label == k ? pk - 1.0f : pk) * w;
        if (dropped) { g = 0.f; h = 0.f; }
        a.gpair[(int64_t)k * a.gp_stride + r] = make_float2(g, h);
        mg = fmaxf(mg, fabsf(g)); mh = fmaxf(mh, h);
      }
    } else {
      const bool reg_loss = a.objective <= kLogitRaw || a.objective == kSquaredLogError || a.objective == kPseudoHuber;
      if (reg_loss && y == 1.0f) w *= a.scale_pos_weight;
      float p = a.margin ? a.margin[r] : 0.f, g, h;
      switch (a.objective) {
        case kSquaredError: g = p - y; h = 1.0f; break;
        case kSquaredLogError: {
          if (!(y > -1.0f)) *a.err = 3;
          p = fmaxf(p, -1.0f + 1e-6f);
          g = (log1pf(p) - log1pf(y)) / (p + 1.0f);
          h = fmaxf((-log1pf(p) + log1pf(y) + 1.0f) / ((p + 1.0f) * (p + 1.0f)), 1e-6f);
          break; }
        case kPseudoHuber: {
          const float z = p - y, s2 = a.aux * a.aux, scale_sqrt = sqrtf(1.0f + z * z / s2);
          g = z / scale_sqrt; h = s2 / ((s2 + z * z) * scale_sqrt);
          break; }
        case kPoisson: {
          if (y < 0.0f) *a.err = 4;
          g = expf(p) - y; h = expf(p + a.aux);
          break; }
        case kGamma: {
          if (!(y > 0.0f)) *a.err = 5;
          const float ep = expf(p);
          g = 1.0f - y / ep; h = y / ep;
          break; }
        case kTweedie: {
          if (y < 0.0f) *a.err = 6;
          const float rho = a.aux, e1 = expf((1.0f - rho) * p), e2 = expf((2.0f - rho) * p);
          g = -y * e1 + e2; h = -y * (1.0f - rho) * e1 + (2.0f - rho) * e2;
          break; }
        case kHinge: {
          const float yy = y * 2.0f - 1.0f;
          if (p * yy < 1.0f) { g = -yy; h = 1.0f; } else { g = 0.0f; h = 1.17549435e-38f; }
          break; }
        default: {
          if (y < 0.0f || y > 1.0f) *a.err = 1;
          p = sigmoidf_xgb(p); g = p - y; h = fmaxf(p * (1.0f - p), 1e-16f);
          break; }
      }
      g *= w; h *= w;
      if (dropped) { g = 0.f; h = 0.f; }
      a.gpair[r] = make_float2(g, h);
      mg = fmaxf(mg, fabsf(g)); mh = fmaxf(mh, h);
    }
  }
#pragma unroll
  for (int o = 16; o > 0; o >>= 1) { mg = fmaxf(mg, __shfl_xor_sync(0xffffffffu, mg, o)); mh = fmaxf(mh, __shfl_xor_sync(0xffffffffu, mh, o)); }
  __shared__ float sg[8], sh[8];
  if ((threadIdx.x & 31) == 0) { sg[threadIdx.x >> 5] = mg; sh[threadIdx.x >> 5] = mh; }
  __syncthreads();
  if (threadIdx.x == 0) {
    for (int w = 1; w < 8; ++w) { mg = fmaxf(mg, sg[w]); mh = fmaxf(mh, sh[w]); }
    if (a.absmax) { atomicMax(a.absmax, __float_as_uint(mg)); atomicMax(a.absmax + 1, __float_as_uint(mh)); }
  }
}

__global__ void __launch_bounds__(256) sample_gpair_kernel(SampleArgs a) {
  float mg = 0.f, mh = 0.f;
  for (int64_t r = (int64_t)blockIdx.x * blockDim.x + threadIdx.x; r < a.n; r += (int64_t)gridDim.x * blockDim.x) {
    const bool keep = rng_uniform(a.seed, a.stream, (unsigned long long)(r + a.row_offset)) < a.subsample;
    for (int k = 0; k < a.K; ++k) {
      const float2 v = keep ? a.src[(int64_t)k * a.gp_stride + r] : make_float2(0.f, 0.f);
      a.dst[(int64_t)k * a.gp_stride + r] = v;
      mg = fmaxf(mg, fabsf(v.x)); mh = fmaxf(mh, v.y);
    }
  }
#pragma unroll
  for (int o = 16; o > 0; o >>= 1) { mg = fmaxf(mg, __shfl_xor_sync(0xffffffffu, mg, o)); mh = fmaxf(mh, __shfl_xor_sync(0xffffffffu, mh, o)); }
  __shared__ float sg[8], sh[8];
  if ((threadIdx.x & 31) == 0) { sg[threadIdx.x >> 5] = mg; sh[threadIdx.x >> 5] = mh; }
  __syncthreads();
  if (threadIdx.x == 0) {
    for (int w = 1; w < 8; ++w) { mg = fmaxf(mg, sg[w]); mh = fmaxf(mh, sh[w]); }
    atomicMax(a.absmax, __float_as_uint(mg)); atomicMax(a.absmax + 1, __float_as_uint(mh));
  }
}

__global__ void __launch_bounds__(256) sum_gpair_kernel(const float2* gp, int64_t n, double* out) {
  double g = 0, h = 0;
  for (int64_t r = (int64_t)blockIdx.x * blockDim.x + threadIdx.x; r < n; r += (int64_t)gridDim.x * blockDim.x) { float2 v = gp[r]; g += v.x; h += v.y; }
#pragma unroll
  for (int o = 16; o > 0; o >>= 1) { g += __shfl_xor_sync(0xffffffffu, g, o); h += __shfl_xor_sync(0xffffffffu, h, o); }
  if ((threadIdx.x & 31) == 0) { atomicAdd(out, g); atomicAdd(out + 1, h); }
}

__device__ __forceinline__ uint8_t bin_of(float v, const float* c, int nc) {
  if (isnan(v)) return (uint8_t)kMissingBin;
  int lo = 0, hi = nc;
  while (lo < hi) { int mid = (lo + hi) >> 1; if (c[mid] > v) hi = mid; else lo = mid + 1; }
  if (lo >= nc) lo = nc - 1;
  return (uint8_t)lo;
}

__global__ void __launch_bounds__(256) bin_kernel(const float* X, int64_t n, int F, int ngroups, int tw, const int* cut_ptrs, const float* cut_vals,
                                                  uint8_t* bins, uint8_t* bins_tail) {
  const int W = ngroups * kSlots + tw;
  const int64_t total = n * W;
  for (int64_t idx = (int64_t)blockIdx.x * blockDim.x + threadIdx.x; idx < total; idx += (int64_t)gridDim.x * blockDim.x) {
    const int c = (int)(idx % W);
    const int64_t r = idx / W;
    uint8_t b = 0;
    if (c < F) b = bin_of(X[r * F + c], cut_vals + cut_ptrs[c], cut_ptrs[c + 1] - cut_ptrs[c]);
    if (c < ngroups * kSlots) bins[r * (ngroups * kSlots) + c] = b;
    else bins_tail[r * tw + (c - ngroups * kSlots)] = b;
  }
}

__global__ void __launch_bounds__(256) pad_rows_kernel(const uint8_t* src, const uint8_t* tail, int tw, int64_t n, int src_stride, uint8_t* dst, int dst_stride) {
  const int cpr = dst_stride / 16, spr = src_stride / 16;
  for (int64_t i = (int64_t)blockIdx.x * blockDim.x + threadIdx.x; i < n * cpr; i += (int64_t)gridDim.x * blockDim.x) {
    const int64_t r = i / cpr; const int c = (int)(i - r * cpr);
    uint4 v = make_uint4(0, 0, 0, 0);
    if (c < spr) v = reinterpret_cast<const uint4*>(src + r * src_stride)[c];
    else if (c == spr && tw > 0) {
      v.x = reinterpret_cast<const unsigned*>(tail + r * tw)[0];
      if (tw == 8) v.y = reinterpret_cast<const unsigned*>(tail + r * tw)[1];
    }
    reinterpret_cast<uint4*>(dst + r * dst_stride)[c] = v;
  }
}
void launch_pad_rows(const uint8_t* src, const uint8_t* tail, int tw, int64_t n, int src_stride, uint8_t* dst, int dst_stride, cudaStream_t s) {
  if (n == 0) return;
  B200_CHECK(tw == 0 || (tw <= dst_stride - src_stride && src_stride % 16 == 0), "pad_rows: the tail does not fit in the row's pad");
  pad_rows_kernel<<<engine_num_sms() * 16, 256, 0, s>>>(src, tail, tw, n, src_stride, dst, dst_stride); ++g_kernel_launches; CUDA_OK(cudaGetLastError());
}

__global__ void __launch_bounds__(256) transpose_bins_kernel(const uint8_t* bins, const uint8_t* bins_tail, int64_t n, int F, int ngroups, int tw, uint8_t* bins_col) {
  __shared__ uint8_t tile[256][kSlots + 1];
  const int g = blockIdx.y;
  const bool is_tail = g == ngroups;
  const int width = is_tail ? tw : kSlots;
  const int64_t r0 = (int64_t)blockIdx.x * 256;
  for (int i = threadIdx.x; i < 256 * width; i += 256) {
    int rr = i / width, s = i % width;
    int64_t r = r0 + rr;
    tile[rr][s] = r < n ? (is_tail ? bins_tail[r * tw + s] : bins[r * (ngroups * kSlots) + g * kSlots + s]) : 0;
  }
  __syncthreads();
  const int64_t r = r0 + threadIdx.x;
  if (r < n) for (int s = 0; s < width; ++s) { int f = g * kSlots + s; if (f < F) bins_col[(int64_t)f * n + r] = tile[threadIdx.x][s]; }
}

__global__ void __launch_bounds__(256) count_nan_kernel(const float* X, int64_t count, float missing, int use_missing, unsigned long long* out) {
  unsigned long long c = 0;
  for (int64_t i = (int64_t)blockIdx.x * blockDim.x + threadIdx.x; i < count; i += (int64_t)gridDim.x * blockDim.x) {
    float v = X[i];
    c += (isnan(v) || (use_missing && v == missing)) ? 1ull : 0ull;
  }
#pragma unroll
  for (int o = 16; o > 0; o >>= 1) c += __shfl_xor_sync(0xffffffffu, c, o);
  if ((threadIdx.x & 31) == 0 && c) atomicAdd(out, c);
}

__global__ void __launch_bounds__(256) replace_missing_kernel(float* X, int64_t count, float missing) {
  for (int64_t i = (int64_t)blockIdx.x * blockDim.x + threadIdx.x; i < count; i += (int64_t)gridDim.x * blockDim.x)
    if (X[i] == missing) X[i] = __int_as_float(0x7fc00000);
}

__global__ void __launch_bounds__(256) predict_kernel(PredictArgs a) {
  const int64_t r = (int64_t)blockIdx.x * blockDim.x + threadIdx.x;
  if (r >= a.n) return;
  const float* x = a.X + r * a.F;
  const int nt = a.tree_end - a.tree_begin;
  float acc = (a.K == 1 && a.margin) ? a.margin[r] : 0.f;
  for (int t = a.tree_begin; t < a.tree_end; ++t) {
    const DevNode* nodes = a.nodes + a.tree_offset[t];
    int nid = 0;
    DevNode nd = nodes[0];
    while (nd.left != -1) {
      const unsigned f = nd.fidx_dl & 0x7fffffffu;
      const float v = f < (unsigned)a.F ? __ldg(x + f) : __int_as_float(0x7fc00000);
      if (isnan(v)) nid = (nd.fidx_dl >> 31) ? nd.left : nd.right;
      else nid = v < nd.cond ? nd.left : nd.right;
      nd = nodes[nid];
    }
    if (a.margin) { if (a.K == 1) acc += nd.cond; else a.margin[r * a.K + a.tree_info[t]] += nd.cond; }
    if (a.leaf) a.leaf[r * nt + (t - a.tree_begin)] = nid;
  }
  if (a.K == 1 && a.margin) a.margin[r] = acc;
}

struct PNode { float cond; unsigned w; };

static_assert(kPredictMaxPitch <= 0x7fff + 1, "the tiled predictor's feature field has 15 bits");

template <bool HAS_NAN, bool LEAF_OUT>
__global__ void __launch_bounds__(1024) predict_tiled_kernel(PredictArgs a, int tree_lo, int tree_hi, int pitch, int rows_per_tile, int64_t num_tiles) {
  extern __shared__ __align__(16) unsigned char psm[];
  const int nt_chunk = tree_hi - tree_lo;
  int* s_toff = reinterpret_cast<int*>(psm);
  PNode* s_nodes = reinterpret_cast<PNode*>(psm + (((size_t)(nt_chunk + 1) * 4 + 15) & ~(size_t)15));
  __shared__ int s_total;
  if (threadIdx.x == 0) {
    int off = 0;
    for (int t = 0; t < nt_chunk; ++t) { s_toff[t] = off; off += (int)(a.tree_offset[tree_lo + t + 1] - a.tree_offset[tree_lo + t]); }
    s_toff[nt_chunk] = off; s_total = off;
  }
  __syncthreads();
  for (int t = 0; t < nt_chunk; ++t) {
    const DevNode* src = a.nodes + a.tree_offset[tree_lo + t];
    const int cnt = s_toff[t + 1] - s_toff[t];
    for (int i = threadIdx.x; i < cnt; i += blockDim.x) {
      const DevNode d = src[i];
      PNode p; p.cond = d.cond;
      p.w = (d.left < 0 ? 0xffffu : (unsigned)d.left) | ((d.fidx_dl & 0x7fffu) << 16) | (d.fidx_dl & 0x80000000u);
      s_nodes[s_toff[t] + i] = p;
    }
  }
  float* s_x = reinterpret_cast<float*>(s_nodes + s_total);
  const int F = a.F, K = a.K, nt_all = a.tree_end - a.tree_begin;
  for (int64_t tile = blockIdx.x; tile < num_tiles; tile += gridDim.x) {
    const int64_t r0 = tile * rows_per_tile;
    const int rows = (int)((a.n - r0 < rows_per_tile) ? a.n - r0 : rows_per_tile);
    __syncthreads();
    const float* src = a.X + r0 * F;
    const int total = rows * F;
    for (int i = threadIdx.x; i < total; i += blockDim.x) { const int r = i / F, f = i - r * F; s_x[r * pitch + f] = __ldg(src + i); }
    __syncthreads();
    for (int rl = threadIdx.x; rl < rows; rl += blockDim.x) {
      const float* x = s_x + rl * pitch;
      const int64_t r = r0 + rl;
      float acc = (!LEAF_OUT && K == 1) ? a.margin[r] : 0.f;
      auto step = [&](const PNode* tn, int& nid, PNode& nd) {
        const float v = x[(nd.w >> 16) & 0x7fffu];
        const int left = (int)(nd.w & 0xffffu);
        bool go_left = v < nd.cond;
        if (HAS_NAN) { if (isnan(v)) go_left = (nd.w >> 31) != 0; }
        nid = go_left ? left : left + 1;
        nd = tn[nid];
      };
      auto emit = [&](int t, int nid, const PNode& nd) {
        if (LEAF_OUT) a.leaf[r * nt_all + (tree_lo - a.tree_begin) + t] = nid;
        else if (K == 1) acc += nd.cond;
        else a.margin[r * K + a.tree_info[tree_lo + t]] += nd.cond;
      };
      int t = 0;
      for (; t + 4 <= nt_chunk; t += 4) {
        const PNode* tn[4]; int nid[4]; PNode nd[4];
#pragma unroll
        for (int j = 0; j < 4; ++j) { tn[j] = s_nodes + s_toff[t + j]; nid[j] = 0; nd[j] = tn[j][0]; }
        bool any = true;
        while (any) {
          any = false;
#pragma unroll
          for (int j = 0; j < 4; ++j) if ((nd[j].w & 0xffffu) != 0xffffu) { step(tn[j], nid[j], nd[j]); any = true; }
        }
#pragma unroll
        for (int j = 0; j < 4; ++j) emit(t + j, nid[j], nd[j]);
      }
      for (; t < nt_chunk; ++t) {
        const PNode* tn = s_nodes + s_toff[t];
        int nid = 0; PNode nd = tn[0];
        while ((nd.w & 0xffffu) != 0xffffu) step(tn, nid, nd);
        emit(t, nid, nd);
      }
      if (!LEAF_OUT && K == 1) a.margin[r] = acc;
    }
  }
}

__global__ void __launch_bounds__(256) transform_kernel(float* m, int64_t n, int K, int objective, float* out_class) {
  const int64_t r = (int64_t)blockIdx.x * blockDim.x + threadIdx.x;
  if (r >= n) return;
  if (objective == kBinaryLogistic || objective == kRegLogistic) m[r] = sigmoidf_xgb(m[r]);
  else if (objective == kPoisson || objective == kGamma || objective == kTweedie || objective == kAft || objective == kCox) m[r] = expf(m[r]);
  else if (objective == kHinge) m[r] = m[r] > 0.0f ? 1.0f : 0.0f;
  else if (objective == kSoftprob || objective == kSoftmax) {
    float* p = m + r * K;
    float wmax = p[0]; int arg = 0;
    for (int k = 1; k < K; ++k) if (p[k] > wmax) { wmax = p[k]; arg = k; }
    if (objective == kSoftmax) { out_class[r] = (float)arg; return; }
    float wsum = 0.f;
    for (int k = 0; k < K; ++k) { p[k] = expf(p[k] - wmax); wsum += p[k]; }
    for (int k = 0; k < K; ++k) p[k] /= wsum;
  }
}

__global__ void __launch_bounds__(256) fill_kernel(float* p, int64_t n, float v) {
  for (int64_t i = (int64_t)blockIdx.x * blockDim.x + threadIdx.x; i < n; i += (int64_t)gridDim.x * blockDim.x) p[i] = v;
}
__global__ void __launch_bounds__(256) add_base_margin_kernel(float* p, const float* bm, int64_t count) {
  for (int64_t i = (int64_t)blockIdx.x * blockDim.x + threadIdx.x; i < count; i += (int64_t)gridDim.x * blockDim.x) p[i] = bm[i];
}

__global__ void __launch_bounds__(256) metric_kernel(MetricArgs a) {
  double s = 0, ws = 0;
  for (int64_t r = (int64_t)blockIdx.x * blockDim.x + threadIdx.x; r < a.n; r += (int64_t)gridDim.x * blockDim.x) {
    const float y = a.label[r];
    const float w = a.weight ? a.weight[r] : 1.0f;
    float loss = 0.f;
    if (a.metric == kMetricMlogloss || a.metric == kMetricMerror) {
      const float* m = a.margin + r * a.K;
      float wmax = m[0]; int arg = 0;
      for (int k = 1; k < a.K; ++k) if (m[k] > wmax) { wmax = m[k]; arg = k; }
      int label = (int)y;
      if (a.metric == kMetricMerror) loss = (arg != label) ? 1.f : 0.f;
      else {
        float wsum = 0.f;
        for (int k = 0; k < a.K; ++k) wsum += expf(m[k] - wmax);
        float p = (label >= 0 && label < a.K) ? expf(m[label] - wmax) / wsum : 0.f;
        const float eps = 1e-16f;
        loss = p > eps ? -logf(p) : -logf(eps);
      }
    } else {
      float p = a.margin[r];
      if (a.is_logistic || a.transform == kTransformSigmoid) p = sigmoidf_xgb(p);
      else if (a.transform == kTransformExp) p = expf(p);
      else if (a.transform == kTransformHinge) p = p > 0.0f ? 1.0f : 0.0f;
      switch (a.metric) {
        case kMetricRmsle: { float d = log1pf(y) - log1pf(p); loss = d * d; break; }
        case kMetricMape: loss = fabsf((y - p) / y); break;
        case kMetricMphe: { const float z = (y - p) / a.aux; loss = a.aux * a.aux * (sqrtf(1.0f + z * z) - 1.0f); break; }
        case kMetricPoissonNll: { const float py = fmaxf(p, 1e-16f); loss = lgammaf(y + 1.0f) + py - logf(py) * y; break; }
        case kMetricGammaNll: { const float py = fmaxf(p, 1e-6f); loss = y / py + logf(py); break; }
        case kMetricGammaDeviance: { const float py = p + 1e-6f, yy = y + 1e-6f; loss = logf(py / yy) + yy / py - 1.0f; break; }
        case kMetricTweedieNll: { const float rho = a.aux, lp = logf(p); loss = -y * expf((1.0f - rho) * lp) / (1.0f - rho) + expf((2.0f - rho) * lp) / (2.0f - rho); break; }
        case kMetricRmse: { float d = p - y; loss = d * d; break; }
        case kMetricMae: loss = fabsf(p - y); break;
        case kMetricLogloss: {
          const float eps = 1e-16f;
          float pneg = 1.0f - p;
          if (p < eps) loss = -y * logf(eps) - (1.0f - y) * logf(1.0f - eps);
          else if (pneg < eps) loss = -y * logf(1.0f - eps) - (1.0f - y) * logf(eps);
          else loss = -y * logf(p) - (1.0f - y) * logf(pneg);
          break; }
        case kMetricError: loss = (p > a.threshold) ? (1.0f - y) : y; break;
        default: break;
      }
    }
    s += (double)(loss * w); ws += (double)w;
  }
#pragma unroll
  for (int o = 16; o > 0; o >>= 1) { s += __shfl_xor_sync(0xffffffffu, s, o); ws += __shfl_xor_sync(0xffffffffu, ws, o); }
  if ((threadIdx.x & 31) == 0) { atomicAdd(a.out, s); atomicAdd(a.out + 1, ws); }
}

static inline int grid_for(int64_t n, int block = 256, int cap = engine_num_sms() * 16) {
  int64_t g = (n + block - 1) / block; if (g < 1) g = 1; if (g > cap) g = cap; return (int)g;
}
void launch_gradient(const GradArgs& a, cudaStream_t s) {
  if (a.n == 0) return;
  gradient_kernel<<<grid_for(a.n, 256, engine_num_sms() * 8), 256, 0, s>>>(a); ++g_kernel_launches; CUDA_OK(cudaGetLastError());
}
void launch_sample_gpair(const SampleArgs& a, cudaStream_t s) {
  if (a.n == 0) return;
  sample_gpair_kernel<<<grid_for(a.n, 256, engine_num_sms() * 8), 256, 0, s>>>(a); ++g_kernel_launches; CUDA_OK(cudaGetLastError());
}
void launch_sum_gpair(const float2* gp, int64_t n, double* out, cudaStream_t s) {
  sum_gpair_kernel<<<grid_for(n), 256, 0, s>>>(gp, n, out); ++g_kernel_launches; CUDA_OK(cudaGetLastError());
}
void launch_bin(const float* X, int64_t n, int F, int ngroups, int tw, const int* cut_ptrs, const float* cut_vals, uint8_t* bins, uint8_t* bins_tail, cudaStream_t s) {
  if (n == 0) return;
  bin_kernel<<<grid_for(n * (ngroups * kSlots + tw), 256, engine_num_sms() * 32), 256, 0, s>>>(X, n, F, ngroups, tw, cut_ptrs, cut_vals, bins, bins_tail); ++g_kernel_launches;
  CUDA_OK(cudaGetLastError());
}
void launch_transpose_bins(const uint8_t* bins, const uint8_t* bins_tail, int64_t n, int F, int ngroups, int tw, uint8_t* bins_col, cudaStream_t s) {
  if (n == 0) return;
  dim3 grid((unsigned)((n + 255) / 256), ngroups + (tw > 0 ? 1 : 0));
  transpose_bins_kernel<<<grid, 256, 0, s>>>(bins, bins_tail, n, F, ngroups, tw, bins_col); ++g_kernel_launches; CUDA_OK(cudaGetLastError());
}
void launch_count_nan(const float* X, int64_t count, float missing, int use_missing, unsigned long long* out, cudaStream_t s) {
  if (count == 0) return;
  count_nan_kernel<<<grid_for(count), 256, 0, s>>>(X, count, missing, use_missing, out); ++g_kernel_launches; CUDA_OK(cudaGetLastError());
}
void launch_replace_missing(float* X, int64_t count, float missing, cudaStream_t s) {
  if (count == 0) return;
  replace_missing_kernel<<<grid_for(count), 256, 0, s>>>(X, count, missing); ++g_kernel_launches; CUDA_OK(cudaGetLastError());
}
PredictPlan plan_for(const PredictArgs& a) {
  static const bool legacy = getenv("B200XGB_PREDICT_LEGACY") != nullptr;
  return plan_predict(a.h_tree_offset, a.tree_begin, a.tree_end, a.F, a.model_F, a.children_adjacent != 0, legacy);
}

void launch_predict(const PredictArgs& a, cudaStream_t s) {
  if (a.n == 0 || a.tree_end <= a.tree_begin) return;
  const PredictPlan plan = plan_for(a);
  if (plan.kernel == PredictKernel::kTiled) {
    static bool attr = false;
    if (!attr) {
      CUDA_OK(cudaFuncSetAttribute(predict_tiled_kernel<false, false>, cudaFuncAttributeMaxDynamicSharedMemorySize, (int)kPredictSmem));
      CUDA_OK(cudaFuncSetAttribute(predict_tiled_kernel<true, false>, cudaFuncAttributeMaxDynamicSharedMemorySize, (int)kPredictSmem));
      CUDA_OK(cudaFuncSetAttribute(predict_tiled_kernel<false, true>, cudaFuncAttributeMaxDynamicSharedMemorySize, (int)kPredictSmem));
      CUDA_OK(cudaFuncSetAttribute(predict_tiled_kernel<true, true>, cudaFuncAttributeMaxDynamicSharedMemorySize, (int)kPredictSmem));
      attr = true;
    }
    const int pitch = plan.pitch;
    for (const PredictChunk& ch : plan.chunks) {
      const int rows = ch.rows, threads = ch.threads;
      const int64_t tiles = (a.n + rows - 1) / rows;
      const int grid = (int)std::min<int64_t>(tiles, engine_num_sms() * (threads == 1024 ? 1 : 2048 / threads));
      if (a.leaf) { if (a.has_nan) predict_tiled_kernel<true, true><<<grid, threads, ch.smem, s>>>(a, ch.tree_lo, ch.tree_hi, pitch, rows, tiles);
                    else predict_tiled_kernel<false, true><<<grid, threads, ch.smem, s>>>(a, ch.tree_lo, ch.tree_hi, pitch, rows, tiles); }
      else { if (a.has_nan) predict_tiled_kernel<true, false><<<grid, threads, ch.smem, s>>>(a, ch.tree_lo, ch.tree_hi, pitch, rows, tiles);
             else predict_tiled_kernel<false, false><<<grid, threads, ch.smem, s>>>(a, ch.tree_lo, ch.tree_hi, pitch, rows, tiles); }
      ++g_kernel_launches; CUDA_OK(cudaGetLastError());
    }
    return;
  }
  predict_kernel<<<(unsigned)((a.n + 255) / 256), 256, 0, s>>>(a); ++g_kernel_launches; CUDA_OK(cudaGetLastError());
}
void launch_transform(float* m, int64_t n, int K, int objective, float* out_class, cudaStream_t s) {
  if (n == 0) return;
  transform_kernel<<<(unsigned)((n + 255) / 256), 256, 0, s>>>(m, n, K, objective, out_class); ++g_kernel_launches; CUDA_OK(cudaGetLastError());
}
void launch_fill(float* p, int64_t n, float v, cudaStream_t s) {
  if (n == 0) return;
  fill_kernel<<<grid_for(n), 256, 0, s>>>(p, n, v); ++g_kernel_launches; CUDA_OK(cudaGetLastError());
}
void launch_metric(const MetricArgs& a, cudaStream_t s) {
  if (a.n == 0) return;
  metric_kernel<<<grid_for(a.n), 256, 0, s>>>(a); ++g_kernel_launches; CUDA_OK(cudaGetLastError());
}

}
```

### sagemaker-xgboost-container_b200/csrc/misc.h

```cpp
#pragma once
#include "engine.h"
#include "predict_plan.h"

namespace b200 {

struct GradArgs {
  const float* margin;
  const float* label; const float* weight;
  float2* gpair;
  int64_t gp_stride;
  unsigned* absmax;
  int* err;
  int64_t n, row_offset;
  int K, objective;
  float scale_pos_weight, subsample;
  unsigned seed; unsigned long long iter;
  float aux;
};

struct DevNode { float cond; int left; int right; unsigned fidx_dl; };

struct PredictArgs {
  const float* X; int64_t n; int F;
  const DevNode* nodes; const int64_t* tree_offset; const int* tree_info;
  int tree_begin, tree_end, K;
  float* margin;
  int* leaf;
  const int64_t* h_tree_offset;
  int has_nan;
  int children_adjacent;
  int model_F;
};

enum Metric : int { kMetricRmse = 0, kMetricMae = 1, kMetricLogloss = 2, kMetricError = 3, kMetricMerror = 4, kMetricMlogloss = 5,
                    kMetricAuc = 6, kMetricMse = 7, kMetricRmsle = 8, kMetricMape = 9, kMetricMphe = 10, kMetricPoissonNll = 11,
                    kMetricGammaNll = 12, kMetricGammaDeviance = 13, kMetricTweedieNll = 14 };

struct MetricArgs {
  const float* margin; const float* label; const float* weight; double* out;
  int64_t n; int K, metric, is_logistic; float threshold;
  int transform;
  float aux;
};

struct ShapNode { float cond; int left; int right; unsigned fidx_dl; float sum_hess; float mean; };
struct ShapArgs {
  const float* X; int64_t n; int F;
  const ShapNode* nodes; const int64_t* tree_offset; const int* tree_info;
  int tree_begin, tree_end, K;
  float* out;
  const float* base_margin_rows;
  float base_margin;
  const float* tree_weight;
};
void launch_shap(const ShapArgs& a, int max_depth, cudaStream_t s);

struct DartArgs {
  const float* X; int64_t n; int F;
  const DevNode* nodes; const int64_t* tree_offset; const int* tree_info;
  const int* trees; int ntrees; int K;
  const float* coef_full;
  const float* coef_drop;
  float* m_full;
  float* m_drop;
};
void launch_dart_margin(const DartArgs& a, cudaStream_t s);

struct SampleArgs {
  const float2* src;
  float2* dst;
  unsigned* absmax;
  int64_t gp_stride, n, row_offset;
  int K; float subsample; unsigned seed; unsigned long long stream;
};

void launch_gradient(const GradArgs& a, cudaStream_t s);
void launch_sample_gpair(const SampleArgs& a, cudaStream_t s);
void launch_sum_gpair(const float2* gp, int64_t n, double* out, cudaStream_t s);
void launch_bin(const float* X, int64_t n, int F, int ngroups, int tw, const int* cut_ptrs, const float* cut_vals, uint8_t* bins, uint8_t* bins_tail, cudaStream_t s);
void launch_transpose_bins(const uint8_t* bins, const uint8_t* bins_tail, int64_t n, int F, int ngroups, int tw, uint8_t* bins_col, cudaStream_t s);
void launch_pad_rows(const uint8_t* src, const uint8_t* tail, int tw, int64_t n, int src_stride, uint8_t* dst, int dst_stride, cudaStream_t s);
void launch_count_nan(const float* X, int64_t count, float missing, int use_missing, unsigned long long* out, cudaStream_t s);
void launch_replace_missing(float* X, int64_t count, float missing, cudaStream_t s);
PredictPlan plan_for(const PredictArgs& a);
void launch_predict(const PredictArgs& a, cudaStream_t s);
void launch_transform(float* m, int64_t n, int K, int objective, float* out_class, cudaStream_t s);
void launch_fill(float* p, int64_t n, float v, cudaStream_t s);
void launch_metric(const MetricArgs& a, cudaStream_t s);
void compute_auc_device(const float* margin, const float* label, const float* weight, int64_t n, int is_logistic, double* out, cudaStream_t s);

struct HostCuts { std::vector<int> ptrs; std::vector<float> vals; std::vector<float> mins; };
void compute_cuts_device(const float* dX, int64_t n, int F, const float* dweights, int max_bin, bool has_missing,
                         HostCuts* out, cudaStream_t s);
struct FeatureSummary { std::vector<float> vals; std::vector<double> weights; };
void compute_summaries_device(const float* dX, int64_t n, int F, const float* dweights, int cap,
                              std::vector<FeatureSummary>* out, cudaStream_t s);
void cuts_from_summaries(const std::vector<FeatureSummary>& sums, int max_bin, bool has_missing, HostCuts* out);
constexpr int kRankSummaryCap = 2048;
void merge_summaries(const std::vector<std::vector<FeatureSummary>>& per_rank, int F, std::vector<FeatureSummary>* merged);
void compute_rank_cuts_device(const float* dX, int F, const float* dweights, const int64_t* row_bounds, int nranges, int max_bin,
                              bool has_missing, HostCuts* out, cudaStream_t s);

}
```

### sagemaker-xgboost-container_b200/csrc/tree.cu

```cuda
#include <algorithm>
#include <type_traits>
#include "engine.h"
#include "rng.h"
#include "tree.h"

namespace b200 {

__device__ __forceinline__ double threshold_l1(double w, double alpha) {
  if (w > +alpha) return w - alpha;
  if (w < -alpha) return w + alpha;
  return 0.0;
}
__device__ __forceinline__ float calc_weight(const TrainParamDev& p, double G, double H) {
  if (H < p.min_child_weight || H <= 0.0) return 0.0f;
  double dw = -threshold_l1(G, p.alpha) / (H + p.lambda);
  if (p.max_delta_step != 0.0f && fabs(dw) > p.max_delta_step) dw = copysign((double)p.max_delta_step, dw);
  return (float)dw;
}
__device__ __forceinline__ float gain_at_weight_f(float g, float h, float lambda, float w) {
  return -__fadd_rn(__fmul_rn(__fmul_rn(2.0f, g), w), __fmul_rn(__fmul_rn(__fadd_rn(h, lambda), w), w));
}
__device__ __forceinline__ float calc_gain_given_weight(const TrainParamDev& p, double G, double H, float w) {
  if (H <= 0.0) return 0.0f;
  if (p.max_delta_step == 0.0f) { double t = threshold_l1(G, p.alpha); return (float)(t * t / (H + p.lambda)); }
// ... 315 lines not shown
__global__ void __launch_bounds__(256) apply_lossguide_kernel(ApplyArgs a, int iter) {
  __shared__ unsigned long long s_key[8];
  GrowState& gs = a.gs;
  const double isg = (double)gs.scales[2], ish = (double)gs.scales[3];
  const int src = iter == 0 ? 0 : 1;
  const int cnt = gs.level_count[src];
  const int* nodes = gs.level_nodes + (size_t)src * a.max_level_nodes;
  if (iter == 0 && threadIdx.x == 0 && cnt > 0) finish_root(a, ish);
  for (int i = threadIdx.x; i < cnt; i += blockDim.x) {
    const int nid = nodes[i];
    gs.open[nid] = best_of_blocks(a, nid).loss_chg > 1e-6f ? 1 : 0;
  }
  __syncthreads();
  const int n0 = *gs.n_nodes;
  unsigned long long key = 0ull;
  for (int nid = threadIdx.x; nid < n0; nid += blockDim.x)
    if (gs.open[nid]) { unsigned long long k = ((unsigned long long)__float_as_uint(gs.best[nid].loss_chg) << 32) | (unsigned long long)(0xffffffffu - (unsigned)nid); key = k > key ? k : key; }
#pragma unroll
  for (int o = 16; o > 0; o >>= 1) { unsigned long long x = __shfl_xor_sync(0xffffffffu, key, o); key = x > key ? x : key; }
  if ((threadIdx.x & 31) == 0) s_key[threadIdx.x >> 5] = key;
  __syncthreads();
  if (threadIdx.x != 0) return;
  for (int w = 1; w < 8; ++w) key = s_key[w] > key ? s_key[w] : key;
  bool stop = *gs.lg_done != 0 || key == 0ull;
  int nid = 0; SplitCand best{}; GH64 tot{};
  if (!stop) {
    nid = (int)(0xffffffffu - (unsigned)(key & 0xffffffffull));
    best = gs.best[nid]; tot = gs.node_sum[nid];
    stop = !split_is_valid(a.p, best, tot, gs.depth[nid]) || (a.p.max_leaves > 0 && *gs.n_leaves == a.p.max_leaves);
  }
  if (stop) {
    *gs.lg_done = 1;
    gs.level_count[0] = 0; gs.level_count[1] = 0; *gs.build_count = 0; gs.part_action[0] = 0; gs.tile_prefix[0] = 0; gs.tile_prefix[1] = 0;
    return;
  }
  gs.open[nid] = 0;
  const int Lc = n0, Rc = n0 + 1, d = gs.depth[nid];
  expand_node(a, nid, best, tot, Lc, Rc, isg, ish);
  gs.depth[Lc] = d + 1; gs.depth[Rc] = d + 1; gs.open[Lc] = 0; gs.open[Rc] = 0;
  *gs.n_nodes = n0 + 2;
  const int leaves = *gs.n_leaves + 1;
  *gs.n_leaves = leaves;
  const bool children_evaluated = !(a.p.max_depth > 0 && d + 1 >= a.p.max_depth) && !(a.p.max_leaves > 0 && leaves >= a.p.max_leaves);
  gs.level_nodes[0] = nid; gs.level_count[0] = 1;
  gs.part_action[0] = children_evaluated ? 1 : 0;
  gs.tile_prefix[0] = 0; gs.tile_prefix[1] = children_evaluated ? (gs.seg_count[nid] + kPartTile - 1) / kPartTile : 0u;
  if (children_evaluated) {
    int* nxt = gs.level_nodes + (size_t)a.max_level_nodes;
    nxt[0] = Lc; nxt[1] = Rc; gs.level_count[1] = 2;
    const int slot = (*gs.n_slots)++;
    plan_child_hists(gs, 0, nid, best, tot, Lc, Rc, slot, gs.hist_slot[nid]);
    *gs.build_count = 1;
  } else { gs.level_count[1] = 0; *gs.build_count = 0; }
}

template <typename Pay>
__global__ void __launch_bounds__(256) lg_copy_back_kernel(PartArgs a, unsigned* ridx_dst, Pay* gp_dst, unsigned* tl_dst) {
  const GrowState& gs = a.gs;
  if (gs.level_count[0] <= 0 || !gs.part_action[0]) return;
  const int nid = gs.level_nodes[0];
  const unsigned b = gs.seg_begin[nid], c = gs.seg_count[nid];
  const Pay* gp_src = static_cast<const Pay*>(a.gp_next);
  for (unsigned p = b + blockIdx.x * blockDim.x + threadIdx.x; p < b + c; p += gridDim.x * blockDim.x) {
    ridx_dst[p] = a.ridx_next[p]; gp_dst[p] = gp_src[p];
    if (a.tl_next) tl_dst[p] = a.tl_next[p];
  }
}

__global__ void __launch_bounds__(256) zero_build_slots_kernel(GrowState gs, GH64* pool, size_t stride) {
  const int r = blockIdx.x;
  if (r >= *gs.build_count) return;
  GH64* h = pool + (size_t)gs.hist_slot[gs.build_nid[r]] * stride;
  GH64 z; z.g = 0; z.h = 0;
  for (size_t e = (size_t)blockIdx.y * blockDim.x + threadIdx.x; e < stride; e += (size_t)gridDim.y * blockDim.x) h[e] = z;
}

__global__ void __launch_bounds__(256) lg_stage_kernel(GrowState gs, GH64* pool, size_t stride, int to_stage) {
  if (*gs.build_count <= 0) return;
  GH64* slot = pool + (size_t)gs.hist_slot[gs.build_nid[0]] * stride;
  GH64* stage = pool + (size_t)kLgStageSlot * stride;
  for (size_t e = (size_t)blockIdx.x * blockDim.x + threadIdx.x; e < stride; e += (size_t)gridDim.x * blockDim.x) {
    if (to_stage) stage[e] = slot[e]; else slot[e] = stage[e];
  }
}

__device__ __forceinline__ int find_node_of_tile(const unsigned* tile_prefix, int cnt, unsigned tile) {
  int lo = 0, hi = cnt;
  while (hi - lo > 1) { int mid = (lo + hi) >> 1; if (tile_prefix[mid] <= tile) lo = mid; else hi = mid; }
  return lo;
}

constexpr unsigned long long kDescAggregate = 1ull << 62;
constexpr unsigned long long kDescPrefix = 2ull << 62;

__device__ __forceinline__ unsigned long long ld_relaxed_u64(const unsigned long long* p) {
  unsigned long long v; asm volatile("ld.relaxed.gpu.global.u64 %0, [%1];" : "=l"(v) : "l"(p) : "memory"); return v;
}
__device__ __forceinline__ void st_relaxed_u64(unsigned long long* p, unsigned long long v) {
  asm volatile("st.relaxed.gpu.global.u64 [%0], %1;" :: "l"(p), "l"(v) : "memory");
}

__device__ unsigned lookback_lefts(const unsigned long long* d, unsigned lt) {
  const int lane = threadIdx.x & 31;
  unsigned acc = 0;
  for (int hi = (int)lt - 1; hi >= 0; hi -= 32) {
    const int j = hi - lane;
    unsigned long long v = 0;
    if (j >= 0) { v = ld_relaxed_u64(d + j); while ((v >> 62) == 0) { __nanosleep(64); v = ld_relaxed_u64(d + j); } }
    const unsigned pref = __ballot_sync(0xffffffffu, (v >> 62) == 2);
    const int last = pref ? __ffs(pref) - 1 : 31;
    unsigned x = lane <= last ? (unsigned)v : 0u;
#pragma unroll
    for (int o = 16; o > 0; o >>= 1) x += __shfl_xor_sync(0xffffffffu, x, o);
    acc += x;
    if (pref) break;
  }
  return acc;
}

template <bool GONLY, bool TL>
__global__ void __launch_bounds__(256, GONLY ? (TL ? 5 : 6) : 4) part_kernel(PartArgs a) {
  typedef typename std::conditional<GONLY, float, float2>::type Pay;
  GrowState& gs = a.gs;
  __shared__ unsigned s_rid[kPartTile];
  __shared__ Pay s_gp[kPartTile];
  __shared__ unsigned s_tl[TL ? kPartTile : 1];
  __shared__ unsigned s_w[8];
  const int cnt = gs.level_count[a.level];
  const unsigned total = cnt > 0 ? gs.tile_prefix[cnt] : 0u;
  if (threadIdx.x == 0) s_w[0] = atomicAdd(gs.part_ctl, 1u);
  __syncthreads();
  const unsigned tile = s_w[0];
  __syncthreads();
  const int i = tile < total ? find_node_of_tile(gs.tile_prefix, cnt, tile) : 0;
  if (tile < total && gs.part_action[i]) {
    const int nid = gs.level_nodes[(size_t)a.level * a.max_level_nodes + i];
    const unsigned t0 = gs.tile_prefix[i], lt = tile - t0;
    const unsigned b = gs.seg_begin[nid], c = gs.seg_count[nid];
    const unsigned p0 = b + lt * kPartTile, p1 = (b + c < p0 + kPartTile) ? b + c : p0 + kPartTile;
    const unsigned nrows = p1 - p0;
    const int f = a.tree.split_index[nid];
    const int sb = a.tree.split_bin[nid], dl = a.tree.default_left[nid];
    const uint8_t* col = a.bins_col + (int64_t)f * a.n;
    const Pay* gp_cur = static_cast<const Pay*>(a.gp_cur);
    Pay* gp_next = static_cast<Pay*>(a.gp_next);
    const unsigned pt = p0 + threadIdx.x * 8;
    unsigned rows[8]; Pay gp[8]; unsigned tl[8]; unsigned char fl[8]; unsigned mine = 0;
#pragma unroll
    for (int j = 0; j < 8; ++j) {
      const unsigned p = pt + j;
      rows[j] = 0; gp[j] = Pay{}; tl[j] = 0u;
      if (p < p1) {
        rows[j] = a.ridx_cur ? a.ridx_cur[p] : p;
        if constexpr (GONLY) gp[j] = static_cast<const float*>(a.gp_cur)[(size_t)p * a.gp_cur_stride];
        else gp[j] = gp_cur[p];
        if constexpr (TL) tl[j] = a.tl_cur[p];
      }
    }
#pragma unroll
    for (int j = 0; j < 8; ++j) {
      if (pt + j < p1) {
        const int byte = col[rows[j]];
        const bool left = (a.has_missing && byte == kMissingBin) ? (dl != 0) : (byte <= sb);
        fl[j] = left ? 1 : 0; mine += fl[j];
      } else fl[j] = 2;
    }
    const int lane = threadIdx.x & 31, warp = threadIdx.x >> 5;
    unsigned x = mine;
#pragma unroll
    for (int o = 1; o < 32; o <<= 1) { unsigned y = __shfl_up_sync(0xffffffffu, x, o); if (lane >= o) x += y; }
    if (lane == 31) s_w[warp] = x;
    __syncthreads();
    unsigned woff = 0, tile_left = 0;
    for (int w = 0; w < 8; ++w) { if (w < warp) woff += s_w[w]; tile_left += s_w[w]; }
    unsigned long long* desc = gs.tile_desc + t0;
    if (threadIdx.x == 0) st_relaxed_u64(desc + lt, (lt == 0 ? kDescPrefix : kDescAggregate) | tile_left);
    unsigned lbefore = woff + x - mine;
#pragma unroll
    for (int j = 0; j < 8; ++j) {
      if (fl[j] == 2) continue;
      const unsigned jj = threadIdx.x * 8 + j;
      const unsigned slot = fl[j] ? lbefore++ : tile_left + (jj - lbefore);
      s_rid[slot] = rows[j]; s_gp[slot] = gp[j]; if constexpr (TL) s_tl[slot] = tl[j];
    }
    unsigned lefts_before = 0;
    if (warp == 0 && lt > 0) {
      lefts_before = lookback_lefts(desc, lt);
      if (lane == 0) st_relaxed_u64(desc + lt, kDescPrefix | (lefts_before + tile_left));
    }
    __syncthreads();
    if (threadIdx.x == 0) s_w[0] = lefts_before;
    __syncthreads();
    lefts_before = s_w[0];
    const unsigned rights_before = lt * kPartTile - lefts_before;
    const int Lc = a.tree.left[nid], Rc = a.tree.right[nid];
    bool write_left = true, write_right = true;
    if (a.build_only) { const bool build_right = gs.node_sum[Rc].h < gs.node_sum[Lc].h; write_left = !build_right; write_right = build_right; }
    const unsigned k0 = write_left ? 0u : tile_left, k1 = write_right ? nrows : tile_left;
    const unsigned dl0 = b + lefts_before, dr0 = b + c - 1 - rights_before + tile_left;
    for (unsigned k = k0 + threadIdx.x; k < k1; k += blockDim.x) {
      const unsigned dest = k < tile_left ? dl0 + k : dr0 - k;
      a.ridx_next[dest] = s_rid[k];
      gp_next[dest] = s_gp[k];
      if constexpr (TL) a.tl_next[dest] = s_tl[k];
    }
    if (threadIdx.x == 0) {
      if (lt == gs.tile_prefix[i + 1] - t0 - 1) {
        const unsigned nl = lefts_before + tile_left;
        gs.seg_begin[Lc] = b; gs.seg_count[Lc] = nl; gs.seg_begin[Rc] = b + nl; gs.seg_count[Rc] = c - nl;
      }
      if (a.rows_counter) { atomicAdd(a.rows_counter, (unsigned long long)nrows); atomicAdd(a.rows_counter + 1, (unsigned long long)(k1 - k0)); }
    }
  }
  __syncthreads();
  if (threadIdx.x == 0) { __threadfence(); s_w[0] = atomicAdd(gs.part_ctl + 1, 1u) == gridDim.x - 1 ? 1u : 0u; }
  __syncthreads();
  if (!s_w[0]) return;
  __threadfence();
  const int nb = *gs.build_count;
  for (int r = threadIdx.x; r < nb; r += blockDim.x) gs.build_prefix[r] = __ldcg(gs.seg_count + gs.build_nid[r]);
  __syncthreads();
  const unsigned tot = nb > 0 ? block_exclusive_scan(gs.build_prefix, gs.build_prefix, nb, s_rid ) : 0u;
  if (threadIdx.x == 0) gs.build_prefix[nb > 0 ? nb : 0] = tot;
}

struct PackedNode { unsigned feat; unsigned short bin_dl; unsigned short left; };
constexpr int kPackedNodesSmem = 2048;
static_assert(sizeof(PackedNode) == 8, "PackedNode is 8 B");
__device__ __forceinline__ PackedNode pack_node(const TreeArrays& t, int i) {
  PackedNode p; p.feat = (unsigned)t.split_index[i]; p.bin_dl = (unsigned short)((t.split_bin[i] + 1) | (t.default_left[i] ? 0x8000 : 0));
  const int l = t.left[i]; p.left = l < 0 ? 0xffff : (unsigned short)l;
  return p;
}
__device__ __forceinline__ bool goes_left(const PackedNode& p, int byte, int has_missing) {
  return (has_missing && byte == kMissingBin) ? ((p.bin_dl & 0x8000) != 0) : (byte < (int)(p.bin_dl & 0x7fff));
}

__device__ __forceinline__ void stage_route_tables(const RouteArgs& a, PackedNode* s_node, unsigned char* s_bidx, int nb) {
  const int nn = *a.gs.n_nodes;
  for (int i = threadIdx.x; i < kRouteMaxNodes; i += blockDim.x) {
    if (s_node) { PackedNode p{0u, 0, 0xffff}; if (i < nn) p = pack_node(a.tree, i); s_node[i] = p; }
    s_bidx[i] = 0xff;
  }
  __syncthreads();
  for (int r = threadIdx.x; r < nb; r += blockDim.x) s_bidx[a.gs.build_nid[r]] = (unsigned char)r;
  __syncthreads();
}

constexpr int kRuns = kRouteTile / 1024;
__global__ void __launch_bounds__(256) route_kernel(RouteArgs a) {
  __shared__ PackedNode s_node[kRouteMaxNodes];
  __shared__ unsigned char s_bidx[kRouteMaxNodes];
  __shared__ unsigned s_cnt[kRouteMaxBuild];
  const int nb = *a.gs.build_count;
  if (a.level > 0 && nb == 0) return;
  const int64_t r0 = (int64_t)blockIdx.x * kRouteTile + threadIdx.x * 4;
  const int lane = threadIdx.x & 31;
  unsigned ids[kRuns], out[kRuns];
#pragma unroll
  for (int j = 0; j < kRuns; ++j) {
    const int64_t r = r0 + j * 1024;
    ids[j] = 0u; out[j] = 0u;
    if (a.level > 0) {
      if (r + 4 <= a.n) ids[j] = *reinterpret_cast<const unsigned*>(a.node_of_row + r);
      else for (int e = 0; e < 4; ++e) if (r + e < a.n) ids[j] |= (unsigned)a.node_of_row[r + e] << (8 * e);
    }
  }
  if (threadIdx.x < kRouteMaxBuild) s_cnt[threadIdx.x] = 0;
  stage_route_tables(a, s_node, s_bidx, nb);
  int byte[4 * kRuns];
#pragma unroll
  for (int q = 0; q < 4 * kRuns; ++q) {
    const int64_t r = r0 + (q >> 2) * 1024 + (q & 3);
    const PackedNode p = s_node[(ids[q >> 2] >> (8 * (q & 3))) & 0xffu];
    byte[q] = (r < a.n && p.left != 0xffff) ? a.bins_col[(int64_t)p.feat * a.n + r] : 0;
  }
#pragma unroll
  for (int q = 0; q < 4 * kRuns; ++q) {
    const int64_t r = r0 + (q >> 2) * 1024 + (q & 3);
    const unsigned id = (ids[q >> 2] >> (8 * (q & 3))) & 0xffu;
    const PackedNode p = s_node[id];
    const unsigned child = p.left == 0xffff ? id : (goes_left(p, byte[q], a.has_missing) ? p.left : p.left + 1u);
    out[q >> 2] |= child << (8 * (q & 3));
    const unsigned c = r < a.n ? s_bidx[child] : 0xffu;
    const unsigned m = __match_any_sync(0xffffffffu, c);
    if (c != 0xffu && lane == __ffs(m) - 1) atomicAdd(&s_cnt[c], (unsigned)__popc(m));
  }
#pragma unroll
  for (int j = 0; j < kRuns; ++j) {
    const int64_t r = r0 + j * 1024;
    if (a.level > 0 && out[j] == ids[j]) continue;
    if (r + 4 <= a.n) *reinterpret_cast<unsigned*>(a.node_of_row + r) = out[j];
    else for (int e = 0; e < 4; ++e) if (r + e < a.n) a.node_of_row[r + e] = (uint8_t)(out[j] >> (8 * e));
  }
  __syncthreads();
  for (int c = threadIdx.x; c < nb; c += blockDim.x) a.tile_counts[(size_t)c * a.ntiles + blockIdx.x] = s_cnt[c];
  if (a.rows_counter && threadIdx.x == 0) {
    const int64_t t0 = (int64_t)blockIdx.x * kRouteTile;
    atomicAdd(a.rows_counter, (unsigned long long)(a.n - t0 < (int64_t)kRouteTile ? a.n - t0 : (int64_t)kRouteTile));
  }
}

__global__ void __launch_bounds__(1024) route_scan_kernel(RouteArgs a) {
  __shared__ unsigned s_run[1024], s_tmp[33];
  const int c = blockIdx.x;
  if (c >= *a.gs.build_count) return;
  unsigned* cnt = a.tile_counts + (size_t)c * a.ntiles;
  const unsigned per = (a.ntiles + blockDim.x - 1) / blockDim.x, t0 = threadIdx.x * per, t1 = min(t0 + per, a.ntiles);
  unsigned sum = 0;
#pragma unroll 8
  for (unsigned t = t0; t < t1; ++t) sum += cnt[t];
  s_run[threadIdx.x] = sum;
  __syncthreads();
  const unsigned tot = block_exclusive_scan(s_run, s_run, (int)blockDim.x, s_tmp);
  unsigned run = s_run[threadIdx.x];
#pragma unroll 8
  for (unsigned t = t0; t < t1; ++t) { const unsigned v = cnt[t]; cnt[t] = run; run += v; }
  if (threadIdx.x == 0) a.gs.seg_count[a.gs.build_nid[c]] = tot;
}

constexpr int kWarpRows = kRouteTile / 8, kWarpSteps = kWarpRows / 32;
template <bool GONLY, bool TL>
__global__ void __launch_bounds__(256, 4) scatter_kernel(RouteArgs a) {
  typedef typename std::conditional<GONLY, float, float2>::type Pay;
  __shared__ unsigned char s_bidx[kRouteMaxNodes];
  __shared__ unsigned s_start[kRouteMaxBuild];
  __shared__ unsigned s_local[kRouteMaxBuild + 1];
  __shared__ unsigned s_dst[kRouteMaxBuild];
  __shared__ unsigned s_wofs[8][kRouteMaxBuild];
  __shared__ unsigned s_rid[kRouteTile];
  __shared__ Pay s_gp[kRouteTile];
  __shared__ unsigned s_tl[TL ? kRouteTile : 1];
  __shared__ unsigned char s_ch[kRouteTile];
  const GrowState& gs = a.gs;
  const int nb = *gs.build_count;
  if (nb == 0) { if (blockIdx.x == 0 && threadIdx.x == 0) gs.build_prefix[0] = 0; return; }
  stage_route_tables(a, nullptr, s_bidx, nb);
  if (threadIdx.x < nb) s_start[threadIdx.x] = gs.seg_count[gs.build_nid[threadIdx.x]];
  __syncthreads();
  if (threadIdx.x == 0) {
    unsigned run = 0;
    for (int c = 0; c < nb; ++c) {
      const unsigned t = s_start[c]; s_start[c] = run;
      if (blockIdx.x == 0) { gs.build_prefix[c] = run; gs.seg_begin[gs.build_nid[c]] = run; }
      run += t;
    }
    if (blockIdx.x == 0) gs.build_prefix[nb] = run;
  }
  const int lane = threadIdx.x & 31, warp = threadIdx.x >> 5;
  const unsigned lanes_below = (1u << lane) - 1u;
  for (unsigned tile = blockIdx.x; tile < a.ntiles; tile += gridDim.x) {
    const int64_t rw = (int64_t)tile * kRouteTile + warp * kWarpRows + lane;
    unsigned ck[kWarpSteps];
#pragma unroll
    for (int it = 0; it < kWarpSteps; ++it) { const int64_t r = rw + it * 32; ck[it] = r < a.n ? a.node_of_row[r] : kRouteMaxNodes - 1; }
    const unsigned toff = threadIdx.x < nb ? a.tile_counts[(size_t)threadIdx.x * a.ntiles + tile] : 0u;
    __syncthreads();
    for (int i = threadIdx.x; i < 8 * kRouteMaxBuild; i += blockDim.x) s_wofs[i / kRouteMaxBuild][i % kRouteMaxBuild] = 0;
    __syncthreads();
#pragma unroll
    for (int it = 0; it < kWarpSteps; ++it) {
      const unsigned c = s_bidx[ck[it]];
      const unsigned m = __match_any_sync(0xffffffffu, c);
      const unsigned before = c != 0xffu ? s_wofs[warp][c] : 0u;
      __syncwarp();
      if (c != 0xffu && lane == __ffs(m) - 1) s_wofs[warp][c] = before + __popc(m);
      __syncwarp();
      ck[it] = c << 16 | (before + __popc(m & lanes_below));
    }
    __syncthreads();
    if (threadIdx.x < nb) {
      unsigned t = 0;
      for (int w = 0; w < 8; ++w) t += s_wofs[w][threadIdx.x];
      s_local[threadIdx.x + 1] = t;
    }
    __syncthreads();
    if (threadIdx.x == 0) { s_local[0] = 0; for (int c = 0; c < nb; ++c) s_local[c + 1] += s_local[c]; }
    __syncthreads();
    if (threadIdx.x < nb) {
      const unsigned c = threadIdx.x;
      unsigned run = s_local[c];
      s_dst[c] = s_start[c] + toff - run;
      for (int w = 0; w < 8; ++w) { const unsigned t = s_wofs[w][c]; s_wofs[w][c] = run; run += t; }
    }
    __syncthreads();
#pragma unroll
    for (int h = 0; h < kWarpSteps; h += 8) {
      Pay pv[8]; unsigned tv[8];
#pragma unroll
      for (int j = 0; j < 8; ++j) {
        const unsigned r = (unsigned)(rw + (h + j) * 32);
        pv[j] = Pay{}; tv[j] = 0u;
        if ((ck[h + j] >> 16) != 0xffu) {
          if constexpr (GONLY) pv[j] = __ldg(reinterpret_cast<const float*>(a.gpair) + (size_t)r * 2); else pv[j] = __ldg(a.gpair + r);
          if constexpr (TL) tv[j] = __ldg(a.tail_row + r);
        }
      }
#pragma unroll
      for (int j = 0; j < 8; ++j) {
        const unsigned c = ck[h + j] >> 16;
        if (c == 0xffu) continue;
        const unsigned k = s_wofs[warp][c] + (ck[h + j] & 0xffffu);
        s_rid[k] = (unsigned)(rw + (h + j) * 32); s_gp[k] = pv[j]; s_ch[k] = (unsigned char)c;
        if constexpr (TL) s_tl[k] = tv[j];
      }
    }
    __syncthreads();
    const unsigned built = s_local[nb];
    for (unsigned k = threadIdx.x; k < built; k += blockDim.x) {
      const unsigned pos = s_dst[s_ch[k]] + k;
      a.ridx[pos] = s_rid[k]; static_cast<Pay*>(a.gp)[pos] = s_gp[k];
      if constexpr (TL) a.tl[pos] = s_tl[k];
    }
    if (a.rows_counter && threadIdx.x == 0) atomicAdd(a.rows_counter + 1, (unsigned long long)built);
  }
}

__global__ void __launch_bounds__(256) update_margin_kernel(TreeArrays t, const int* n_nodes, const uint8_t* bins_col, int64_t n, int has_missing,
                                                            const uint8_t* node_of_row, float* margin, int K, int k, const float* leaf_scale) {
  __shared__ PackedNode s_nodes[kPackedNodesSmem];
  __shared__ float s_leaf[kPackedNodesSmem];
  const int nn = *n_nodes;
  const bool packed = nn <= kPackedNodesSmem && nn < 0xffff;
  if (packed) {
    for (int i = threadIdx.x; i < nn; i += blockDim.x) { s_nodes[i] = pack_node(t, i); s_leaf[i] = t.split_cond[i]; }
    __syncthreads();
  }
  const int64_t base = (int64_t)blockIdx.x * 1024 + threadIdx.x;
  int nid[4]; bool done[4];
#pragma unroll
  for (int j = 0; j < 4; ++j) {
    const int64_t r = base + j * 256;
    nid[j] = (node_of_row != nullptr && r < n) ? (int)node_of_row[r] : 0;
    done[j] = r >= n || (packed ? (s_nodes[nid[j]].left == 0xffff) : (t.left[nid[j]] == -1));
  }
  bool any = !(done[0] && done[1] && done[2] && done[3]);
  while (any) {
    int byte[4];
#pragma unroll
    for (int j = 0; j < 4; ++j) {
      const int f = packed ? (int)s_nodes[nid[j]].feat : t.split_index[nid[j]];
      byte[j] = done[j] ? 0 : bins_col[(int64_t)f * n + base + j * 256];
    }
    any = false;
#pragma unroll
    for (int j = 0; j < 4; ++j) {
      if (done[j]) continue;
      const int nd = nid[j];
      if (packed) {
        const PackedNode p = s_nodes[nd];
        nid[j] = goes_left(p, byte[j], has_missing) ? p.left : p.left + 1;
        done[j] = s_nodes[nid[j]].left == 0xffff;
      } else {
        const bool left = (has_missing && byte[j] == kMissingBin) ? (t.default_left[nd] != 0) : (byte[j] <= t.split_bin[nd]);
        nid[j] = left ? t.left[nd] : t.right[nd];
        done[j] = t.left[nid[j]] == -1;
      }
      any |= !done[j];
    }
  }
  const float sc = *leaf_scale;
#pragma unroll
  for (int j = 0; j < 4; ++j) { const int64_t r = base + j * 256; if (r < n) margin[r * K + k] = __fadd_rn(margin[r * K + k], __fmul_rn(sc, packed ? s_leaf[nid[j]] : t.split_cond[nid[j]])); }
}

__global__ void __launch_bounds__(256) subtract_kernel(GrowState gs, GH64* pool, size_t stride) {
  const int r = blockIdx.x;
  if (r >= *gs.build_count) return;
  const int bld = gs.build_nid[r], sub = gs.build_sub_nid[r];
  const GH64* hb = pool + (size_t)gs.hist_slot[bld] * stride;
  const GH64* hp = pool + (size_t)gs.build_parent_slot[r] * stride;
  GH64* hs = pool + (size_t)gs.hist_slot[sub] * stride;
  for (size_t e = (size_t)blockIdx.y * blockDim.x + threadIdx.x; e < stride; e += (size_t)gridDim.y * blockDim.x) {
    GH64 p = hp[e], b = hb[e]; GH64 o; o.g = p.g - b.g; o.h = p.h - b.h; hs[e] = o;
  }
}

void launch_init_tree(const GrowState& gs, const TreeArrays& t, unsigned n, cudaStream_t s) {
  init_tree_kernel<<<1, 32, 0, s>>>(gs, t, n); ++g_kernel_launches; CUDA_OK(cudaGetLastError());
}
void launch_scales(const GrowState& gs, int grad_bits, cudaStream_t s) { scales_kernel<<<1, 32, 0, s>>>(gs, grad_bits); ++g_kernel_launches; CUDA_OK(cudaGetLastError()); }
void launch_eval(const EvalArgs& a, int max_nodes_level, cudaStream_t s) {
  dim3 grid(max_nodes_level, a.ngroups + (a.tw > 0 ? 1 : 0)); eval_kernel<<<grid, 32 * kEvalSegs, 0, s>>>(a); ++g_kernel_launches; CUDA_OK(cudaGetLastError());
}
void launch_apply_lossguide(const ApplyArgs& a, int iter, cudaStream_t s) { apply_lossguide_kernel<<<1, 256, 0, s>>>(a, iter); ++g_kernel_launches; CUDA_OK(cudaGetLastError()); }
void launch_lg_copy_back(const PartArgs& a, unsigned* ridx_dst, void* gp_dst, unsigned* tl_dst, unsigned max_tiles, cudaStream_t s) {
  const unsigned grid = max_tiles < 1184u ? max_tiles : 1184u;
  if (a.g_only) lg_copy_back_kernel<float><<<grid, 256, 0, s>>>(a, ridx_dst, static_cast<float*>(gp_dst), tl_dst);
  else lg_copy_back_kernel<float2><<<grid, 256, 0, s>>>(a, ridx_dst, static_cast<float2*>(gp_dst), tl_dst);
  ++g_kernel_launches; CUDA_OK(cudaGetLastError());
}
void launch_zero_build_slots(const GrowState& gs, GH64* pool, size_t slot_entries, int max_build, cudaStream_t s) {
  dim3 grid(max_build, (unsigned)((slot_entries + 1023) / 1024)); zero_build_slots_kernel<<<grid, 256, 0, s>>>(gs, pool, slot_entries); ++g_kernel_launches; CUDA_OK(cudaGetLastError());
}
void launch_lg_stage(const GrowState& gs, GH64* pool, size_t slot_entries, int to_stage, cudaStream_t s) {
  lg_stage_kernel<<<(unsigned)((slot_entries + 1023) / 1024), 256, 0, s>>>(gs, pool, slot_entries, to_stage); ++g_kernel_launches; CUDA_OK(cudaGetLastError());
}
void launch_apply(const ApplyArgs& a, cudaStream_t s) { apply_kernel<<<1, 256, 0, s>>>(a); ++g_kernel_launches; CUDA_OK(cudaGetLastError()); }
void launch_partition(const PartArgs& a, unsigned max_tiles, cudaStream_t s) {
  CUDA_OK(cudaMemsetAsync(a.gs.tile_desc, 0, sizeof(unsigned long long) * ((size_t)max_tiles + 1), s));
  const bool tl = a.tl_cur != nullptr;
  if (a.g_only) { if (tl) part_kernel<true, true><<<max_tiles, 256, 0, s>>>(a); else part_kernel<true, false><<<max_tiles, 256, 0, s>>>(a); }
  else { if (tl) part_kernel<false, true><<<max_tiles, 256, 0, s>>>(a); else part_kernel<false, false><<<max_tiles, 256, 0, s>>>(a); }
  ++g_kernel_launches; CUDA_OK(cudaGetLastError());
}
void launch_route(const RouteArgs& a, cudaStream_t s) {
  if (a.ntiles == 0) return;
  route_kernel<<<a.ntiles, 256, 0, s>>>(a); ++g_kernel_launches; CUDA_OK(cudaGetLastError());
  route_scan_kernel<<<1u << a.level, 1024, 0, s>>>(a); ++g_kernel_launches; CUDA_OK(cudaGetLastError());
  const bool tl = a.tail_row != nullptr;
  const unsigned grid = std::min(a.ntiles, 4u * (unsigned)engine_num_sms());
  if (a.g_only) { if (tl) scatter_kernel<true, true><<<grid, 256, 0, s>>>(a); else scatter_kernel<true, false><<<grid, 256, 0, s>>>(a); }
  else { if (tl) scatter_kernel<false, true><<<grid, 256, 0, s>>>(a); else scatter_kernel<false, false><<<grid, 256, 0, s>>>(a); }
  ++g_kernel_launches; CUDA_OK(cudaGetLastError());
}
void launch_update_margin(const TreeArrays& t, const int* n_nodes, const uint8_t* bins_col, int64_t n, int has_missing, const uint8_t* node_of_row,
                          float* margin, int K, int k, const float* leaf_scale, cudaStream_t s) {
  if (n == 0) return;
  update_margin_kernel<<<(unsigned)((n + 1023) / 1024), 256, 0, s>>>(t, n_nodes, bins_col, n, has_missing, node_of_row, margin, K, k, leaf_scale);
  ++g_kernel_launches; CUDA_OK(cudaGetLastError());
}
void launch_subtract(const GrowState& gs, GH64* pool, size_t slot_entries, int max_build, cudaStream_t s) {
  dim3 grid(max_build, (unsigned)((slot_entries + 1023) / 1024)); subtract_kernel<<<grid, 256, 0, s>>>(gs, pool, slot_entries); ++g_kernel_launches; CUDA_OK(cudaGetLastError());
}

}
```

### sagemaker-xgboost-container_b200/csrc/tree.h

```cpp
#pragma once
#include "engine.h"

namespace b200 {

constexpr unsigned kPartTile = 2048;

struct TrainParamDev {
  float eta, lambda, alpha, gamma, min_child_weight, max_delta_step;
  int max_depth, max_leaves;
};

struct EvalArgs {
  const GH64* hist_pool; GrowState gs; const int* cut_ptrs; const unsigned char* feat_mask;
  TrainParamDev p; int F, ngroups, tw, ntail, has_missing, level, max_level_nodes;
  const int* monotone;
  const unsigned char* node_allowed;
  float colsample_bynode; unsigned seed; const int* tree_index;
};

struct ApplyArgs {
  GrowState gs; TreeArrays tree; const int* cut_ptrs; const float* cut_vals; const float* min_vals;
  TrainParamDev p; unsigned* scratch; int nblocks , level, max_level_nodes, next_base, next_half;
  const int* monotone;
  unsigned char* node_path; unsigned char* node_allowed; const unsigned char* ic_sets; int n_ic_sets, F;
};

struct PartArgs {
  GrowState gs; TreeArrays tree; const uint8_t* bins_col; int64_t n; const unsigned* ridx_cur; unsigned* ridx_next;
  const void* gp_cur; void* gp_next; int gp_cur_stride; int g_only;
  const unsigned* tl_cur; unsigned* tl_next;
  int has_missing, level, max_level_nodes;
  int build_only;
  unsigned long long* rows_counter;
};

constexpr int kRouteMaxDepth = 7;
constexpr unsigned kRouteTile = 2048;
constexpr int kRouteMaxNodes = 256;
constexpr int kRouteMaxBuild = 1 << (kRouteMaxDepth - 2);
struct RouteArgs {
  GrowState gs; TreeArrays tree; const uint8_t* bins_col; int64_t n;
  uint8_t* node_of_row;
  unsigned* tile_counts;
  unsigned ntiles; int has_missing, level;
  const float2* gpair; int g_only; const unsigned* tail_row;
  unsigned* ridx; void* gp; unsigned* tl;
  unsigned long long* rows_counter;
};

struct HistArgs {
  const uint8_t* bins;
  const uint8_t* bins_tail;
  const unsigned* tail_pos;
  int64_t n;
  int row_stride;
  const uint8_t* bins_gather;
  int gather_stride;
  int tail_in_gather;
  int tw;
  const float2* gpair;
  const float* gpos;
  const unsigned* ridx;
  const int* build_count;
  const int* build_nid;
  const unsigned* build_prefix;
  const unsigned* seg_begin;
  const int* hist_slot;
  const float* scales;
  GH64* hist_pool;
  GH64* node_sum;
  int ngroups;
  int ng_chunk;
  int accumulate_sum;
  int g_only;
  int window_rows;
  int force_gather;
  unsigned long long* rows_counter;
};

constexpr int kLgRootSlot = 0, kLgStageSlot = 1, kLgFirstFreeSlot = 2;
void launch_apply_lossguide(const ApplyArgs& a, int iter, cudaStream_t s);
void launch_lg_copy_back(const PartArgs& a, unsigned* ridx_dst, void* gp_dst, unsigned* tl_dst, unsigned max_tiles, cudaStream_t s);
void launch_zero_build_slots(const GrowState& gs, GH64* pool, size_t slot_entries, int max_build, cudaStream_t s);
void launch_lg_stage(const GrowState& gs, GH64* pool, size_t slot_entries, int to_stage, cudaStream_t s);
void launch_hist_build(const HistArgs& a, int num_sms, cudaStream_t stream);
void hist_configure();
const char* hist_last_kernel();
void launch_init_tree(const GrowState& gs, const TreeArrays& t, unsigned n, cudaStream_t s);
void launch_scales(const GrowState& gs, int grad_bits, cudaStream_t s);
void launch_eval(const EvalArgs& a, int max_nodes_level, cudaStream_t s);
void launch_apply(const ApplyArgs& a, cudaStream_t s);
void launch_partition(const PartArgs& a, unsigned max_tiles, cudaStream_t s);
void launch_route(const RouteArgs& a, cudaStream_t s);
void launch_update_margin(const TreeArrays& t, const int* n_nodes, const uint8_t* bins_col, int64_t n, int has_missing, const uint8_t* node_of_row,
                          float* margin, int K, int k, const float* leaf_scale, cudaStream_t s);
void launch_subtract(const GrowState& gs, GH64* pool, size_t slot_entries, int max_build, cudaStream_t s);

}
```

Measured before the change: 99.07.

## Store gradients as dense g-only array for constant-hessian squared-error rounds

When the objective has a constant hessian (squared error, single output, no weights, no subsampling), the gradient kernel writes only g as a dense float array instead of (g,h) float2 pairs. The root histogram TMA kernel, partition and route kernels then read 4 bytes per row instead of 8 (or a strided float), and the hessian is synthesized as a constant. This reduces gradient write and read bandwidth across the objective, root histogram and partition stages. It adds checks that forbid the layout for other objectives and per-tree sampling.

```diff
diff --git a/microbench/hist_modes.py b/microbench/hist_modes.py
--- a/microbench/hist_modes.py
+++ b/microbench/hist_modes.py
@@ -41,7 +41,7 @@
         gp = gpair if rows is None else gpair[:m]
         be.build_histogram_ex(b.handle, d.handle, gp, mode=mode, row_ids=rows, repeats=2)
         hist, scales, ms, kernel = be.build_histogram_ex(b.handle, d.handle, gp, mode=mode, row_ids=rows, repeats=a.repeats)
-        bytes_ = m * (F + 8 + (0 if rows is None else 4))
+        bytes_ = m * (F + (4 if mode == 2 else 8) + (0 if rows is None else 4))
         r = {"case": label, "kernel": kernel, "rows": m, "ms": ms, "gbs": bytes_ / ms / 1e6, "frac_of_peak": bytes_ / ms / 1e6 / peak,
              "checksum": int(hist[:, :, 0].sum()), "checksum_h": int(hist[:, :, 1].sum())}
         res.append(r)
diff --git a/sagemaker-xgboost-container_b200/csrc/booster.cu b/sagemaker-xgboost-container_b200/csrc/booster.cu
--- a/sagemaker-xgboost-container_b200/csrc/booster.cu
+++ b/sagemaker-xgboost-container_b200/csrc/booster.cu
@@ -638,11 +638,13 @@
   B200_CHECK(!dart_.on || P == 1, "booster=dart with num_parallel_tree > 1 is not implemented on the CUDA hist path");
   if (!per_tree_sample) forest_gpair_.release();
   const float* grad_margin = dart_.on ? dart_begin_round(dtrain, cache, round) : cache.margin.p;
+  const bool dense_g = constant_hessian(*dtrain);
+  B200_CHECK(!(dense_g && per_tree_sample), "per-tree row sampling of a constant-hessian round");
   CUDA_OK(cudaMemsetAsync(b.gs.absmax, 0, 8, s));
   if (per_tree_sample) {
     forest_gpair_.ensure((size_t)b.gp_stride * K);
-    launch_objective(dtrain, grad_margin, round, forest_gpair_.p, b.gp_stride, nullptr, 1.0f);
-  } else launch_objective(dtrain, grad_margin, round, b.gpair.p, b.gp_stride, b.gs.absmax, param_.subsample);
+    launch_objective(dtrain, grad_margin, round, forest_gpair_.p, b.gp_stride, nullptr, 1.0f, false);
+  } else launch_objective(dtrain, grad_margin, round, b.gpair.p, b.gp_stride, b.gs.absmax, param_.subsample, dense_g);
   if (!per_tree_sample) {
     Comm::get().allreduce_max_u32(b.gs.absmax, 2, s);
     launch_scales(b.gs, grad_bits_for(b.global_n), s);
@@ -664,10 +666,12 @@
   iteration_indptr_.push_back((int)trees_.size());
 }
 
-void Booster::launch_objective(DMatrix* dm, const float* margin, int round, float2* gpair, int64_t gp_stride, unsigned* absmax, float subsample) {
+void Booster::launch_objective(DMatrix* dm, const float* margin, int round, float2* gpair, int64_t gp_stride, unsigned* absmax, float subsample,
+                               bool dense_g) {
   cudaStream_t s = engine_stream();
   const int64_t row_offset = (int64_t)Comm::get().rank() << 40;
   if (objective_is_survival(param_.objective)) {
+    B200_CHECK(!dense_g, "the survival objectives write (g,h) pairs");
     SurvivalGradArgs sa{}; sa.margin = margin; sa.label = dm->d_labels.p; sa.lower = dm->d_label_lower.p; sa.upper = dm->d_label_upper.p;
     sa.weight = dm->weights.empty() ? nullptr : dm->d_weights.p; sa.gpair = gpair; sa.absmax = absmax; sa.n = dm->n; sa.row_offset = row_offset;
     sa.subsample = subsample; sa.seed = param_.seed; sa.iter = (unsigned long long)round; sa.dist = param_.aft_dist; sa.sigma = param_.aft_sigma;
@@ -679,7 +683,7 @@
   GradArgs ga{}; ga.margin = margin; ga.label = dm->d_labels.p; ga.weight = dm->weights.empty() ? nullptr : dm->d_weights.p;
   ga.gpair = gpair; ga.gp_stride = gp_stride; ga.absmax = absmax; ga.err = builder_->err.p; ga.n = dm->n; ga.row_offset = row_offset; ga.K = param_.num_class;
   ga.objective = param_.objective; ga.scale_pos_weight = param_.scale_pos_weight; ga.subsample = subsample; ga.seed = param_.seed;
-  ga.iter = (unsigned long long)round; ga.aux = objective_aux(param_);
+  ga.iter = (unsigned long long)round; ga.aux = objective_aux(param_); ga.dense_g = dense_g ? 1 : 0;
   launch_gradient(ga, s);
 }
 
@@ -692,7 +696,7 @@
   const int64_t n = dm->n;
   DevBuf<float> d_margin; DevBuf<float2> d_gp; d_margin.alloc((size_t)n * K); d_gp.alloc((size_t)n * K);
   if (n) CUDA_OK(cudaMemcpyAsync(d_margin.p, margin, sizeof(float) * n * K, cudaMemcpyHostToDevice, s));
-  launch_objective(dm, d_margin.p, round, d_gp.p, n, nullptr, param_.subsample);
+  launch_objective(dm, d_margin.p, round, d_gp.p, n, nullptr, param_.subsample, false);
   std::vector<float2> h((size_t)n * K);
   if (n) CUDA_OK(cudaMemcpyAsync(h.data(), d_gp.p, sizeof(float2) * h.size(), cudaMemcpyDeviceToHost, s));
   Comm::get().sync_stream(s);
@@ -714,6 +718,12 @@
 TreeBuilder& Booster::builder_for(DMatrix* dm) {
   builder_->ensure(dm->binned_view(), param_.max_depth, param_.num_class, lossguide_iters(param_), (int)interaction_.size());
   return *builder_;
+}
+
+bool Booster::constant_hessian(const DMatrix& dm) const {
+  static const bool no_consth = getenv("B200XGB_NO_CONSTH") != nullptr;
+  return !no_consth && param_.objective == kSquaredError && param_.num_class == 1 && dm.weights.empty() &&
+         param_.subsample >= 1.0f && param_.scale_pos_weight == 1.0f;
 }
 
 TreeInputs Booster::tree_inputs(const DMatrix& dm, const std::string& mask, int tree_index, float* margin, int k) {
@@ -725,10 +735,7 @@
   in.mask = mask.empty() ? nullptr : b.upload_mask(mask, tree_index);
   in.monotone = b.upload_monotone(monotone_, dm.F);
   b.upload_interaction(interaction_, dm.F); in.n_ic = (int)interaction_.size();
-  static const bool no_consth = getenv("B200XGB_NO_CONSTH") != nullptr;
-  const bool consth = !no_consth && param_.objective == kSquaredError && param_.num_class == 1 && dm.weights.empty() &&
-                      param_.subsample >= 1.0f && param_.scale_pos_weight == 1.0f;
-  in.root_mode = !consth ? 0 : b.root_h_valid && b.root_h_uid == dm.uid && b.root_h_version == dm.binned_version ? 2 : 1;
+  in.root_mode = !constant_hessian(dm) ? 0 : b.root_h_valid && b.root_h_uid == dm.uid && b.root_h_version == dm.binned_version ? 2 : 1;
   in.world = Comm::get().world();
   return in;
 }
diff --git a/sagemaker-xgboost-container_b200/csrc/booster.h b/sagemaker-xgboost-container_b200/csrc/booster.h
--- a/sagemaker-xgboost-container_b200/csrc/booster.h
+++ b/sagemaker-xgboost-container_b200/csrc/booster.h
@@ -157,7 +157,8 @@
   TreeBuilder& builder_for(DMatrix* dm);
   TreeInputs tree_inputs(const DMatrix& dm, const std::string& mask, int tree_index, float* margin, int k);
   void grow_one_tree(DMatrix* dtrain, PredCache& cache, int k, int tree_index);
-  void launch_objective(DMatrix* dm, const float* margin, int round, float2* gpair, int64_t gp_stride, unsigned* absmax, float subsample);
+  bool constant_hessian(const DMatrix& dm) const;
+  void launch_objective(DMatrix* dm, const float* margin, int round, float2* gpair, int64_t gp_stride, unsigned* absmax, float subsample, bool dense_g);
   JPtr model_to_json();
   void model_from_json(const JValue& doc);
   JPtr config_to_json();
diff --git a/sagemaker-xgboost-container_b200/csrc/grow.cu b/sagemaker-xgboost-container_b200/csrc/grow.cu
--- a/sagemaker-xgboost-container_b200/csrc/grow.cu
+++ b/sagemaker-xgboost-container_b200/csrc/grow.cu
@@ -191,18 +191,20 @@
   if (in.root_mode == 2) { slot_from_cache_kernel<<<num_sms, 256, 0, s>>>(hist_pool.p, root_h_cache.p, slot_stride); ++g_kernel_launches; CUDA_OK(cudaGetLastError()); }
   else CUDA_OK(cudaMemsetAsync(hist_pool.p, 0, slot_stride * sizeof(GH64), s));
   const bool g_only = in.root_mode != 0;
+  const int pay = g_only ? 4 : 8;
   const bool carry_tail = tail_by_position(bm);
   const bool routed = routes(in.lg_iters, D);
   if (profile && routed) {
     prof_part_row_bytes[0] = 3;
     prof_part_row_bytes[1] = 4;
-    prof_part_row_bytes[2] = 8 + 4 + (g_only ? 4 : 8) + (carry_tail ? 8 : 0);
+    prof_part_row_bytes[2] = pay + 4 + pay + (carry_tail ? 8 : 0);
   } else if (profile) {
-    prof_part_row_bytes[0] = 8 + (carry_tail ? 4 : 0) + 1;
-    prof_part_row_bytes[2] = 4 + (g_only ? 4 : 8) + (carry_tail ? 4 : 0);
+    prof_part_row_bytes[0] = pay + (carry_tail ? 4 : 0) + 1;
+    prof_part_row_bytes[2] = 4 + pay + (carry_tail ? 4 : 0);
     prof_part_row_bytes[1] = prof_part_row_bytes[2] + 1;
   }
   HistArgs root = hist_args(bm, k);
+  if (g_only) { root.gpair = nullptr; root.gpos = g_dense(); }
   root.g_only = in.root_mode == 2 ? 1 : 0; root.rows_counter = profile ? prof_rows.p : nullptr;
   timed(kProfRootHist, [&] { launch_hist_build(root, num_sms, s); });
   if (in.root_mode == 1) { snapshot_h_kernel<<<num_sms, 256, 0, s>>>(hist_pool.p, root_h_cache.p, slot_stride); ++g_kernel_launches; CUDA_OK(cudaGetLastError()); }
@@ -227,8 +229,8 @@
     const bool root = cur == kRootRows;
     PartArgs pa{}; pa.gs = gs; pa.tree = ta; pa.bins_col = bm.bins_col; pa.n = bm.n;
     pa.ridx_cur = root ? nullptr : ridx[cur].p; pa.ridx_next = ridx[next].p;
-    pa.gp_cur = root ? static_cast<const void*>(gpair.p + (size_t)k * gp_stride) : gp[cur].p; pa.gp_next = gp[next].p;
-    pa.gp_cur_stride = root ? 2 : 1; pa.g_only = g_only ? 1 : 0;
+    const void* root_gp = g_only ? static_cast<const void*>(g_dense()) : static_cast<const void*>(gpair.p + (size_t)k * gp_stride);
+    pa.gp_cur = root ? root_gp : gp[cur].p; pa.gp_next = gp[next].p; pa.g_only = g_only ? 1 : 0;
     pa.tl_cur = !carry_tail ? nullptr : (root ? reinterpret_cast<const unsigned*>(bm.bins_tail) : tl[cur].p); pa.tl_next = carry_tail ? tl[next].p : nullptr;
     pa.has_missing = bm.has_missing; pa.level = level; pa.max_level_nodes = max_level_nodes; pa.rows_counter = profile ? prof_rows.p + 2 : nullptr;
     return pa;
@@ -264,7 +266,8 @@
     if (routed) {
       RouteArgs ra{}; ra.gs = gs; ra.tree = ta; ra.bins_col = bm.bins_col; ra.n = bm.n; ra.node_of_row = node_of_row.p;
       ra.tile_counts = route_counts.p; ra.ntiles = route_tiles; ra.has_missing = bm.has_missing; ra.level = L;
-      ra.gpair = gpair.p + (size_t)k * gp_stride; ra.g_only = g_only ? 1 : 0;
+      if (g_only) ra.g = g_dense(); else ra.gpair = gpair.p + (size_t)k * gp_stride;
+      ra.g_only = g_only ? 1 : 0;
       ra.tail_row = carry_tail ? reinterpret_cast<const unsigned*>(bm.bins_tail) : nullptr;
       ra.ridx = ridx[0].p; ra.gp = gp[0].p; ra.tl = carry_tail ? tl[0].p : nullptr; ra.rows_counter = profile ? prof_rows.p + 2 : nullptr;
       timed(kProfPartition, [&] { launch_route(ra, s); });
@@ -342,10 +345,10 @@
   HistArgs ha = hist_args(bm, 0);
   ha.ridx = row_ids ? ridx[0].p : nullptr;
   ha.force_gather = (mode & 3) == 1 ? 1 : 0; ha.g_only = (mode & 3) == 2 ? 1 : 0;
-  if (mode & 8) {
+  if ((mode & 8) || ha.g_only) {
     std::vector<float> gh((size_t)rows);
     for (int64_t i = 0; i < rows; ++i) gh[i] = gpair_host[2 * i];
-    float* gpos = reinterpret_cast<float*>(gp[0].p);
+    float* gpos = row_ids ? reinterpret_cast<float*>(gp[0].p) : g_dense();
     if (rows) CUDA_OK(cudaMemcpyAsync(gpos, gh.data(), sizeof(float) * rows, cudaMemcpyHostToDevice, s));
     Comm::get().sync_stream(s);
     ha.gpos = gpos; ha.gpair = nullptr;
diff --git a/sagemaker-xgboost-container_b200/csrc/grow.h b/sagemaker-xgboost-container_b200/csrc/grow.h
--- a/sagemaker-xgboost-container_b200/csrc/grow.h
+++ b/sagemaker-xgboost-container_b200/csrc/grow.h
@@ -101,6 +101,7 @@
   void enqueue(const TreeInputs& in);
   void end_segment();
   HistArgs hist_args(const BinnedMatrix& bm, int k) const;
+  float* g_dense() const { return reinterpret_cast<float*>(gpair.p); }
   EvalArgs eval_args(const TreeInputs& in, int level, const unsigned char* feat_mask) const;
   ApplyArgs apply_args(const TreeInputs& in, int level, int next_base, int next_half) const;
   template <class Launch> void timed(ProfKind kind, Launch launch);
diff --git a/sagemaker-xgboost-container_b200/csrc/hist.cu b/sagemaker-xgboost-container_b200/csrc/hist.cu
--- a/sagemaker-xgboost-container_b200/csrc/hist.cu
+++ b/sagemaker-xgboost-container_b200/csrc/hist.cu
@@ -294,7 +294,8 @@
   const unsigned bars = ring + (unsigned)c.S * c.stage_bytes;
   const unsigned row_bytes = 32u * (unsigned)c.box_groups;
   const unsigned main_tile_bytes = (unsigned)R * row_bytes;
-  const unsigned gp_off = main_tile_bytes, tail_tile_off = main_tile_bytes + (unsigned)R * 8u;
+  constexpr unsigned kGradBytes = GONLY ? 4u : 8u;
+  const unsigned gp_off = main_tile_bytes, tail_tile_off = main_tile_bytes + (unsigned)R * kGradBytes;
   const unsigned ntiles = (T + R - 1) / R;
   const unsigned my_ntiles = ntiles > blockIdx.x ? (ntiles - blockIdx.x + gridDim.x - 1) / gridDim.x : 0u;
 
@@ -324,7 +325,7 @@
     if (lane == 0) {
       const unsigned P = (c.flags & 8) ? 1u : (unsigned)kRootProducerWarps, pw = (unsigned)(warp - NCW);
       if (pw < P) {
-        const unsigned tx = main_tile_bytes + (unsigned)R * 8u + (has_tail ? (unsigned)R * (unsigned)a.tw : 0u);
+        const unsigned tx = main_tile_bytes + (unsigned)R * kGradBytes + (has_tail ? (unsigned)R * (unsigned)a.tw : 0u);
         unsigned s = pw % (unsigned)c.S, round = pw / (unsigned)c.S;
         for (unsigned i = pw; i < my_ntiles; i += P) {
           if (round > 0) mbar_wait(bars + 8u * (c.S + s), (round - 1u) & 1u);
@@ -334,7 +335,8 @@
           mbar_expect_tx(full, tx);
           if ((c.flags & 1) && gridDim.y == 1) bulk_load_1d(dst, a.bins + (size_t)row0 * a.row_stride, main_tile_bytes, full);
           else tma_load_2d(dst, &tm, g0 * 32, (int)row0, full);
-          bulk_load_1d(dst + gp_off, a.gpair + row0, (unsigned)R * 8u, full);
+          if (GONLY) bulk_load_1d(dst + gp_off, a.gpos + row0, (unsigned)R * 4u, full);
+          else bulk_load_1d(dst + gp_off, a.gpair + row0, (unsigned)R * 8u, full);
           if (has_tail) bulk_load_1d(dst + tail_tile_off, a.bins_tail + (size_t)row0 * a.tw, (unsigned)R * (unsigned)a.tw, full);
           const unsigned tp = t + 8u * gridDim.x;
           if (tp < ntiles && !(c.flags & 4)) tma_prefetch_2d(&tm, g0 * 32, (int)(tp * (unsigned)R));
@@ -357,6 +359,17 @@
   tc.rep_off = has_tail ? (unsigned)((lane / a.tw) % c.trep) * (unsigned)a.tw * 4u : 0u;
   const unsigned rowl = (unsigned)(wit << 4) + (unsigned)(lane >> 1);
   const unsigned tiles_per_window = (unsigned)a.window_rows / R;
+  const unsigned hq_one = (unsigned)__float2int_rn(1.0f * sh);
+  auto quant = [&](unsigned tile, unsigned row, bool valid, int& gq, unsigned& hq) {
+    gq = 0; hq = 0;
+    if constexpr (GONLY) {
+      const float g = __uint_as_float(lds_u32(tile + gp_off + row * 4u));
+      if (valid) { gq = __float2int_rn(g * sg); hq = hq_one; }
+    } else {
+      const uint2 gh = lds_v2(tile + gp_off + row * 8u);
+      if (valid) { gq = __float2int_rn(__uint_as_float(gh.x) * sg); hq = (unsigned)__float2int_rn(__uint_as_float(gh.y) * sh); }
+    }
+  };
   long long accG = 0, accH = 0;
   unsigned i = (unsigned)team, s = (unsigned)team, ph = 0;
   for (unsigned wstart = 0;; wstart += tiles_per_window) {
@@ -366,9 +379,8 @@
       const unsigned tile = ring + s * c.stage_bytes;
       const unsigned row0 = (blockIdx.x + i * gridDim.x) * (unsigned)R;
       if (!(c.flags & 2)) {
-        const uint2 ghb = lds_v2(tile + gp_off + rowl * 8u);
-        int gq = 0; unsigned hq = 0;
-        if (row0 + rowl < T) { gq = __float2int_rn(__uint_as_float(ghb.x) * sg); hq = (unsigned)__float2int_rn(__uint_as_float(ghb.y) * sh); }
+        int gq; unsigned hq;
+        quant(tile, rowl, row0 + rowl < T, gq, hq);
         if ((lane & 1) == 0) { accG += gq; accH += hq; }
         const unsigned rowaddr = tile + rowl * row_bytes;
         root_unit<GONLY, 0>(lc, ldsoff, rowaddr, gq, hq);
@@ -381,10 +393,9 @@
             unsigned w0, w1 = 0;
             if (a.tw == 4) w0 = lds_u32(tile + tail_tile_off + trow * 4u);
             else { const uint2 ww = lds_v2(tile + tail_tile_off + trow * 8u); w0 = ww.x; w1 = ww.y; }
-            const uint2 gt = lds_v2(tile + gp_off + trow * 8u);
-            int gqt = 0; unsigned hqt = 0;
-            if (row0 + trow < T) { gqt = __float2int_rn(__uint_as_float(gt.x) * sg); hqt = (unsigned)__float2int_rn(__uint_as_float(gt.y) * sh); }
-            else { w0 = 0; w1 = 0; }
+            int gqt; unsigned hqt;
+            quant(tile, trow, row0 + trow < T, gqt, hqt);
+            if (row0 + trow >= T) { w0 = 0; w1 = 0; }
             tail_accumulate<GONLY>(tc, lane, w0, w1, gqt, hqt);
           }
         }
@@ -568,7 +579,7 @@
   const int PL = gonly ? 1 : 2;
   const unsigned main_b = (unsigned)ngc * PL * kPlaneBytes;
   const unsigned avail = kMaxSmem - 128  - 2 * 8 * 16 ;
-  const unsigned stage = (unsigned)kRootRows * (32u * ngc + 8u + tw);
+  const unsigned stage = (unsigned)kRootRows * (32u * ngc + (gonly ? 4u : 8u) + tw);
   int trep = tw ? 32 / tw : 0;
   unsigned tail_b = (unsigned)PL * 256u * tw * trep * 4u;
   if (tw && main_b + tail_b + kTeams * stage > avail) { trep = 1; tail_b = (unsigned)PL * 256u * tw * 4u; }
@@ -654,9 +665,10 @@
   const int nchunks = chunks_for(a.ngroups);
   a.ng_chunk = groups_per_chunk(a.ngroups);
   static const bool no_tma = getenv("B200XGB_NO_TMA") != nullptr;
-  if (a.ridx == nullptr && !no_tma && !a.force_gather && a.gpos == nullptr) {
+  const bool gonly = a.g_only != 0;
+  B200_CHECK(!gonly || a.gpos != nullptr, "hist: the G-only root pass reads the dense g (gpos)");
+  if (a.ridx == nullptr && !no_tma && !a.force_gather && (a.gpos == nullptr || gonly)) {
     RootCfg c; CUtensorMap tm;
-    const bool gonly = a.g_only != 0;
     if (root_plan(a.ng_chunk, a.tw, gonly, &c) && get_tensor_map(a.bins, a.n, a.row_stride, c.box_groups, kRootRows, &tm)) {
       const int gx = num_sms / nchunks > 0 ? num_sms / nchunks : 1;
       if (gonly) hist_root_kernel<true><<<dim3(gx, nchunks), kRootThreads, c.total, stream>>>(tm, a, c);
diff --git a/sagemaker-xgboost-container_b200/csrc/misc.cu b/sagemaker-xgboost-container_b200/csrc/misc.cu
--- a/sagemaker-xgboost-container_b200/csrc/misc.cu
+++ b/sagemaker-xgboost-container_b200/csrc/misc.cu
@@ -79,7 +79,7 @@
       }
       g *= w; h *= w;
       if (dropped) { g = 0.f; h = 0.f; }
-      a.gpair[r] = make_float2(g, h);
+      if (a.dense_g) reinterpret_cast<float*>(a.gpair)[r] = g; else a.gpair[r] = make_float2(g, h);
       mg = fmaxf(mg, fabsf(g)); mh = fmaxf(mh, h);
     }
   }
@@ -378,6 +378,8 @@
   int64_t g = (n + block - 1) / block; if (g < 1) g = 1; if (g > cap) g = cap; return (int)g;
 }
 void launch_gradient(const GradArgs& a, cudaStream_t s) {
+  B200_CHECK(!a.dense_g || (a.K == 1 && a.objective == kSquaredError && a.weight == nullptr && a.subsample >= 1.0f),
+             "gradient: the dense g layout is for constant-hessian objectives only");
   if (a.n == 0) return;
   gradient_kernel<<<grid_for(a.n, 256, engine_num_sms() * 8), 256, 0, s>>>(a); ++g_kernel_launches; CUDA_OK(cudaGetLastError());
 }
diff --git a/sagemaker-xgboost-container_b200/csrc/misc.h b/sagemaker-xgboost-container_b200/csrc/misc.h
--- a/sagemaker-xgboost-container_b200/csrc/misc.h
+++ b/sagemaker-xgboost-container_b200/csrc/misc.h
@@ -9,6 +9,7 @@
   const float* label; const float* weight;
   float2* gpair;
   int64_t gp_stride;
+  int dense_g;
   unsigned* absmax;
   int* err;
   int64_t n, row_offset;
diff --git a/sagemaker-xgboost-container_b200/csrc/tree.cu b/sagemaker-xgboost-container_b200/csrc/tree.cu
--- a/sagemaker-xgboost-container_b200/csrc/tree.cu
+++ b/sagemaker-xgboost-container_b200/csrc/tree.cu
@@ -491,8 +491,7 @@
       rows[j] = 0; gp[j] = Pay{}; tl[j] = 0u;
       if (p < p1) {
         rows[j] = a.ridx_cur ? a.ridx_cur[p] : p;
-        if constexpr (GONLY) gp[j] = static_cast<const float*>(a.gp_cur)[(size_t)p * a.gp_cur_stride];
-        else gp[j] = gp_cur[p];
+        gp[j] = gp_cur[p];
         if constexpr (TL) tl[j] = a.tl_cur[p];
       }
     }
@@ -731,7 +730,7 @@
         const unsigned r = (unsigned)(rw + (h + j) * 32);
         pv[j] = Pay{}; tv[j] = 0u;
         if ((ck[h + j] >> 16) != 0xffu) {
-          if constexpr (GONLY) pv[j] = __ldg(reinterpret_cast<const float*>(a.gpair) + (size_t)r * 2); else pv[j] = __ldg(a.gpair + r);
+          if constexpr (GONLY) pv[j] = __ldg(a.g + r); else pv[j] = __ldg(a.gpair + r);
           if constexpr (TL) tv[j] = __ldg(a.tail_row + r);
         }
       }
diff --git a/sagemaker-xgboost-container_b200/csrc/tree.h b/sagemaker-xgboost-container_b200/csrc/tree.h
--- a/sagemaker-xgboost-container_b200/csrc/tree.h
+++ b/sagemaker-xgboost-container_b200/csrc/tree.h
@@ -27,7 +27,7 @@
 
 struct PartArgs {
   GrowState gs; TreeArrays tree; const uint8_t* bins_col; int64_t n; const unsigned* ridx_cur; unsigned* ridx_next;
-  const void* gp_cur; void* gp_next; int gp_cur_stride; int g_only;
+  const void* gp_cur; void* gp_next; int g_only;
   const unsigned* tl_cur; unsigned* tl_next;
   int has_missing, level, max_level_nodes;
   int build_only;
@@ -43,7 +43,7 @@
   uint8_t* node_of_row;
   unsigned* tile_counts;
   unsigned ntiles; int has_missing, level;
-  const float2* gpair; int g_only; const unsigned* tail_row;
+  const float* g; const float2* gpair; int g_only; const unsigned* tail_row;
   unsigned* ridx; void* gp; unsigned* tl;
   unsigned long long* rows_counter;
 };
```

New measurement: 102.1 (median of 6 runs). +3.0%, better.
